# FKGSOFTWARE/TERRA-GAN

Hardware: AMD Instinct MI355X
Metric: DSM tiles/sec train-step (G+D) at 256x256 bs=16 (higher is better)
Workload: dtype f32; 1 GPU; BASELINE configs[1]: 256x256 1-ch DSM tiles, batch 16 per GPU, fp32, PConv-UNet G + PatchGAN D + L1/VGG-perceptual/TV/boundary(0.5) losses + 2x Adam; global_batch=16, tile=256, parallelism=single-gpu, launch=eager, vgg_weights=deterministic stand-in (ImageNet weights not fetchable offline; same FLOPs), vgg_trunk=forward Winograd F(2x2,3x3), dgrads F(4x4,3x3) (DESIGN 2b)

## Files before the change

### include/terragan_hip.h

```cpp
#ifndef TERRAGAN_HIP_H
#define TERRAGAN_HIP_H

#include <stddef.h>
#include <stdint.h>

#ifdef __cplusplus
extern "C" {
#endif

typedef void* tg_stream_t;

enum { TG_OK = 0, TG_ERR_ARG = -1, TG_ERR_LAUNCH = -2, TG_ERR_WS = -3 };
enum { TG_ACT_NONE = 0, TG_ACT_RELU = 1, TG_ACT_LEAKY = 2 };
enum { TG_PREC_F32 = 0, TG_PREC_BF16 = 1, TG_PREC_F32_WINO4 = 2 };

typedef struct TgConv {
    int32_t B, H, W, Cin;
    int32_t Ho, Wo, Cout;
    int32_t k, stride, pad;
    int32_t precision;
} TgConv;

int tg_version(void);
const char* tg_last_error(void);


size_t tg_conv_fwd_ws_bytes(const TgConv* g);
int tg_conv_fwd(const TgConv* g, const float* x, const float* in_mask, const float* w,
                const float* bias, const float* ratio, int act, float slope, float* y,
                float* ws, size_t ws_bytes, tg_stream_t stream);

size_t tg_conv_dgrad_ws_bytes(const TgConv* g);
int tg_conv_dgrad(const TgConv* g, const float* dy, const float* w, const float* in_mask,
                  float* dx, int accumulate, float* ws, size_t ws_bytes, tg_stream_t stream);
int tg_conv_dgrad_gated(const TgConv* g, const float* dy, const float* w, const float* in_mask,
                        const float* x_act, int act, float slope, float* dx, float* ws,
                        size_t ws_bytes, tg_stream_t stream);

enum { TG_WPREP_FWD = 0, TG_WPREP_DGRAD = 1 };
size_t tg_conv_wprep_bytes(const TgConv* g, int mode);
int tg_conv_wprep(const TgConv* g, int mode, const float* w, float* wprep, tg_stream_t stream);
size_t tg_conv_wprep_item_bytes(void);
int tg_conv_wprep_item(const TgConv* g, int mode, const float* w, float* wprep, void* item_out);
int tg_conv_wprep_run(const void* items_dev, int n, tg_stream_t stream);
int tg_conv_fwd_p(const TgConv* g, const float* x, const float* in_mask, const float* w, const float* wprep,
                  const float* bias, const float* ratio, int act, float slope, float* y, float* ws,
                  size_t ws_bytes, tg_stream_t stream);
int tg_conv_fwd_pool(const TgConv* g, const float* x, const float* in_mask, const float* w, const float* wprep,
                     const float* bias, const float* ratio, int act, float slope, float* y, float* pool_y, float* ws,
                     size_t ws_bytes, tg_stream_t stream);
int tg_conv_pool_code_supported(const TgConv* g);
int tg_conv_fwd_pool_code(const TgConv* g, const float* x, const float* w, const float* wprep, const float* bias,
                          float* pool_y, unsigned char* code, float* ws, size_t ws_bytes, tg_stream_t stream);
int tg_maxpool2_bwd_code(const float* dout, const unsigned char* code, int B, int Ho, int Wo, int C, float* dx,
                         tg_stream_t stream);
typedef struct TgSparseMap {
    const uint32_t* bits;
    const int32_t* list;
    const int32_t* count;
    int32_t nb, tiles_y, tiles_x, _pad;
} TgSparseMap;
size_t tg_vgg_sparse_map_bytes(int nb, int H, int W, const char* plan);
int tg_vgg_sparse_map(const float* x, int nb, int H, int W, const char* plan, void* buf, size_t buf_bytes, int* ticket,
                      TgSparseMap* maps, tg_stream_t stream);
int tg_conv_fwd_sparse(const TgConv* g, const float* x, const float* w, const float* wprep, const float* bias, int act,
                       float slope, float* y, float* pool_y, unsigned char* code, const TgSparseMap* sp, float* ws,
                       size_t ws_bytes, tg_stream_t stream);
typedef struct TgBnAct {
    const float *mean, *rstd, *gamma, *beta;
    int32_t act;
    float slope;
} TgBnAct;
int tg_conv_bnin_supported(const TgConv* g, int wgrad);
int tg_conv_fwd_bnin(const TgConv* g, const float* x, const TgBnAct* bn, const float* w, const float* bias, int act,
                     float slope, float* y, float* ws, size_t ws_bytes, tg_stream_t stream);
int tg_conv_wgrad_bnin(const TgConv* g, const float* x, const TgBnAct* bn, const float* dy, float* dw, float* db, float* ws,
                       size_t ws_bytes, tg_stream_t stream);
int tg_conv_dgrad_p(const TgConv* g, const float* dy, const float* w, const float* wprep, const float* in_mask,
                    const float* x_act, int act, float slope, float* dx, int accumulate, float* ws,
                    size_t ws_bytes, tg_stream_t stream);
int tg_relu_gate_pack(const float* a, int64_t rows, int C, uint32_t* bits, tg_stream_t stream);
int tg_conv_dgrad_gbits(const TgConv* g, const float* dy, const float* w, const float* wprep, const float* in_mask,
                        const uint32_t* gate_bits, float* dx, int accumulate, float* ws, size_t ws_bytes, tg_stream_t stream);

int tg_set_cu_reserve(int cus);
int tg_set_work_stealing(int mode);

size_t tg_conv_wgrad_ws_bytes(const TgConv* g);
int tg_conv_wgrad(const TgConv* g, const float* x, const float* in_mask, const float* dy,
                  float* dw, float* db, float* ws, size_t ws_bytes, tg_stream_t stream);

int tg_fold_cin(const float* w3, int cout, int taps, int cin, float* w1, tg_stream_t stream);


int tg_mask_update(const float* mask, int B, int H, int W, int k, int stride, int pad, int Ho,
                   int Wo, float* mask_out, float* ratio, tg_stream_t stream);
int tg_mask_up_merge(const float* up_mask, const float* skip_mask, int B, int h, int w, int H,
                     int W, float* out, tg_stream_t stream);

#define TG_MASK_PYRAMID_MAX 24
typedef struct TgMaskOp {
    int kind, H, W, Ho, Wo, k, stride, pad;
    const float* in;
    const float* in2;
    float* out;
    float* out2;
} TgMaskOp;
typedef struct TgMaskPyramid {
    int nops, _pad;
    TgMaskOp op[TG_MASK_PYRAMID_MAX];
} TgMaskPyramid;
int tg_mask_pyramid(const TgMaskPyramid* pm, int B, tg_stream_t stream);


size_t tg_bn_ws_bytes(int64_t rows, int C);
int tg_bn_stats(const float* y, int64_t rows, int C, float eps, float momentum, float* save_mean,
                float* save_rstd, float* running_mean, float* running_var,
// ... 191 lines not shown
```

### terra-gan_amd/csrc/igemm.hip

```cpp
#include <atomic>
#include <stdlib.h>
#include <string.h>

#include <mutex>
#include <vector>

#include "common.h"

struct ProfRec {
    hipEvent_t a, b;
    int kind;
    double flops, bytes;
    int M, N, K, C, splits, cfg;
    char tag[32];
};
static std::mutex g_prof_mu;
static bool g_prof_on = false;
static std::vector<ProfRec> g_prof;
static thread_local char g_prof_tag[32] = "";

struct ProfScope {
    bool on = false;
    ProfRec r{};
    hipStream_t s;
// ... 948 lines not shown
    p.splits = cdiv(p.nchunks, q.chunks_per_split);
    if (p.bf16) {
        if (n64) *rc = launch_pgemm_cfg<16, 16, 4, 1, 2, 2, 12, true>(p, q, flops, bytes, Mtot, s);
        else *rc = launch_pgemm_cfg<8, 16, 2, 2, 2, 2, 7, true>(p, q, flops, bytes, Mtot, s);
    } else {
        if (n64) *rc = launch_pgemm_cfg<16, 16, 4, 1, 2, 2, 12, false>(p, q, flops, bytes, Mtot, s);
        else *rc = launch_pgemm_cfg<8, 16, 2, 2, 2, 2, 7, false>(p, q, flops, bytes, Mtot, s);
    }
    return true;
}

#include "wino.inc"
#include "wino44.inc"
#include "wino16.inc"

static int launch_wino(IGemmParams& p, size_t ws_floats_avail, hipStream_t s) {
    const WinoPlan pl = wino_plan(p, ws_floats_avail);
    p.splits = pl.splits;
    p.Ktot = 9 * p.C;
    TgWprepItem it = {};
    it.kind = p.bf16 ? 5 : 1; it.N = p.N; it.K = p.C; it.w = p.w_raw; it.out = p.wino_u; it.ww = pl.ww;
    int rc = TG_OK;
    const auto transform = [&]() -> int {
        if (p.bf16) {
            hipLaunchKernelGGL(wino_weights16_kernel, dim3(ew_grid((int64_t)p.N * (p.C / 2), 256)), dim3(256), 0, s, p.w_raw,
                               reinterpret_cast<__bf16*>(p.wino_u), p.N, p.C, pl.ww);
            TG_CHECK_LAUNCH("wino_weights16_kernel");
        } else {
            hipLaunchKernelGGL(wino_weights_kernel, dim3(ew_grid((int64_t)p.N * p.C, 256)), dim3(256), 0, s, p.w_raw, p.wino_u, p.N,
                               p.C, pl.ww);
            TG_CHECK_LAUNCH("wino_weights_kernel");
        }
        return TG_OK;
    };
    if (wino_prep(p, it, transform, &rc)) return rc;
    if (pl.pool) p.pool_done = 1;
    TG_REQUIRE(pl.pool || !(p.pool_code || p.pool_only), "tg_conv_fwd_pool_code: this launch cannot write the pool from its output transform");
    TG_REQUIRE(!p.pool_code || p.act == TG_ACT_RELU, "tg_conv_fwd_pool_code: needs a ReLU output");
    if (pl.gbits) p.gate_bits_done = 1;
    WinoProf pf = {p.bf16 ? 3 : 0, p.bf16 ? 4016 : 4064, p.M, 2.0 * p.M * (double)p.N * p.Ktot * g_alg_scale, 0.0};
    pf.bytes = 4.0 * ((double)p.B * p.IH * p.IW * p.C + (double)p.M + (double)p.N * p.Ktot + (double)p.M * p.N +
                      (p.amask ? (double)p.B * p.IH * p.IW : 0.0) + (pl.pool ? 0.25 * (double)p.M * p.N : 0.0)) -
               (p.pool_only ? (4.0 - 0.25) * (double)p.M * p.N : 0.0);
    if (p.bf16) {
        typedef void (*W16Kern)(const IGemmParams, const WinoGeom, const __bf16*);
        static const W16Kern kerns[8] = {wino16_kernel<false, false>, wino16_kernel<false, true>, wino16_kernel<true, false>,
                                         wino16_kernel<true, true>, wino16_pipe_kernel<false>, wino16_pipe_kernel<true>,
                                         wino16_pipe_kernel<false, true>, wino16_pipe_kernel<true, false, true>};
        static LdsOptIn opts[8];
        const int ki = pl.kernel(false);
        return wino_launch(kerns[ki], opts[ki], pl.pipe ? W16_PIPE_LDS_BYTES : W16_LDS_BYTES, "wino16_kernel", p, pl.q, pf, true, s);
    }
    typedef void (*WinoKern)(const IGemmParams, const WinoGeom, const float*);
    static const WinoKern kerns[18] = {wino_kernel<false, false, false>, wino_kernel<false, true, false>, wino_kernel<true, false, false>,
                                       wino_kernel<true, true, false>, wino_pipe_kernel<false, false>, wino_pipe_kernel<true, false>,
                                       wino_pipe_kernel<false, false, true>, wino_pipe_kernel<true, false, false, true>,
                                       wino_kernel<false, false, true>, wino_kernel<false, true, true>, wino_kernel<true, false, true>,
                                       wino_kernel<true, true, true>, wino_pipe_kernel<false, true>, wino_pipe_kernel<true, true>,
                                       wino_pipe_kernel<false, true, true>, wino_pipe_kernel<true, true, false, true>,
                                       wino_pipe_kernel<false, false, false, false, true>, wino_pipe_kernel<false, false, true, false, true>};
    static LdsOptIn opts[18];
    WinoGeom q = pl.q;
    q.qctr = wino_queue_block(s, p.splits, q.total_work);
    if (pl.sparse && !q.qctr) {
        const TgSparseMap* sm = p.sparse;
        q.sp_bits = sm->bits; q.sp_list = sm->list; q.sp_count = sm->count;
        q.sp_nb = sm->nb; q.sp_tiles = sm->nb * q.tiles_y * q.tiles_x;
    }
    const int ki = pl.kernel(q.qctr != nullptr);
    return wino_launch(kerns[ki], opts[ki], (size_t)WINO_LDS_FLOATS * sizeof(float), "wino_kernel", p, q, pf, true, s);
}

static int pick_bn(int N) { return N >= 128 && N % 128 == 0 ? 128 : (N > 32 ? 64 : 32); }

static void plan_splits(IGemmParams& p, size_t ws_floats_avail) {
    const int bn = pick_bn(p.N);
    const long tiles = (long)cdiv(p.M, 128) * cdiv(p.N, bn);
    int splits = 1;
    if (p.T >= 8) {
        int smax = p.T / 4 < 64 ? p.T / 4 : 64;
        while (smax > 1 && (size_t)smax * p.M * p.N > ws_floats_avail) --smax;
        splits = choose_splits(tiles, smax, 512);
    }
    p.steps_per_split = cdiv(p.T > 0 ? p.T : 1, splits);
    p.splits = p.T > 0 ? cdiv(p.T, p.steps_per_split) : 1;
}

static int launch_igemm(IGemmParams& p, hipStream_t s, size_t ws_floats_avail = 0) {
    if (p.M <= 0 || p.N <= 0) return TG_OK;
    TG_REQUIRE(!p.pool_only, "tg_conv_fwd_pool_code: this launch cannot write the pool from its output transform");
    if (smallconv_fwd_applies(p)) {
        p.splits = 1;
        p.Ktot = p.TH * p.TW * p.C;
        const double by = 4.0 * ((double)p.B * p.IH * p.IW * p.C + (double)p.M * p.N + (double)p.N * p.Ktot);
        ProfScope ps(s, 2, 2.0 * p.M * (double)p.N * p.Ktot, by, p.M, p.N, p.Ktot, p.C, 1, 2000);
        return smallconv_fwd_launch(p, s);
    }
    {
        int rc = TG_OK;
        if (try_pgemm(&p, 1, ws_floats_avail, s, &rc)) return rc;
    }
    const bool scalar = (p.C % 4) != 0;
    p.Ktot = p.TH * p.TW * p.C;
    p.nchunks = cdiv(p.C, 32);
    p.T = scalar ? cdiv(p.Ktot, 32) : p.TH * p.TW * p.nchunks;
    const int bn = pick_bn(p.N);
    if (scalar) {
        if (bn == 128) return launch_igemm_cfg<2, 2, 2, 2, true>(p, s);
        if (bn == 64) return launch_igemm_cfg<2, 2, 2, 1, true>(p, s);
        return launch_igemm_cfg<4, 1, 1, 1, true>(p, s);
    }
    if (p.bf16) {
        if (bn == 128) return launch_igemm_cfg<2, 2, 2, 2, false, true>(p, s);
        if (bn == 64) return launch_igemm_cfg<2, 2, 2, 1, false, true>(p, s);
    }
    if (bn == 128) return launch_igemm_cfg<2, 2, 2, 2, false>(p, s);
    if (bn == 64) return launch_igemm_cfg<2, 2, 2, 1, false>(p, s);
    return launch_igemm_cfg<4, 1, 1, 1, false>(p, s);
}

template <int WAVES_M, int WAVES_N, int WM, int WN, bool BF16>
static int launch_igemm_multi_cfg(const IGemmMulti& pm, int ncls, hipStream_t s) {
// ... 424 lines not shown
        return smallconv_wgrad_applies(p) && smallconv_bnin_wgrad_ok(p) ? 1 : 0;
    }
    return smallconv_bnin_fwd_ok(conv_fwd_params(g)) ? 1 : 0;
}
extern "C" int tg_conv_fwd_bnin(const TgConv* g, const float* x, const TgBnAct* bn, const float* w, const float* bias, int act,
                                float slope, float* y, float* ws, size_t ws_bytes, tg_stream_t stream) {
    TG_REQUIRE(bn && bn->mean && bn->rstd && bn->gamma && bn->beta, "tg_conv_fwd_bnin: null pointer");
    TG_REQUIRE(tg_conv_bnin_supported(g, 0), "tg_conv_fwd_bnin: geometry not supported (ask tg_conv_bnin_supported first)");
    const BnIn b = bnin_of(bn);
    FwdExtras e;
    e.in_bn = &b;
    return conv_fwd_impl(g, x, nullptr, w, nullptr, 0, bias, nullptr, act, slope, y, ws, ws_bytes, stream, nullptr, &e);
}
extern "C" int tg_conv_fwd(const TgConv* g, const float* x, const float* in_mask, const float* w, const float* bias,
                           const float* ratio, int act, float slope, float* y, float* ws, size_t ws_bytes,
                           tg_stream_t stream) {
    return conv_fwd_impl(g, x, in_mask, w, nullptr, 0, bias, ratio, act, slope, y, ws, ws_bytes, stream);
}
extern "C" int tg_conv_fwd_p(const TgConv* g, const float* x, const float* in_mask, const float* w, const float* wprep,
                             const float* bias, const float* ratio, int act, float slope, float* y, float* ws, size_t ws_bytes,
                             tg_stream_t stream) {
    return conv_fwd_impl(g, x, in_mask, w, const_cast<float*>(wprep), wprep ? 1 : 0, bias, ratio, act, slope, y, ws, ws_bytes,
                         stream);
}

__global__ __launch_bounds__(256) void transpose_w_kernel(const float* __restrict__ w, float* __restrict__ wt,
                                                          int cout, int taps, int cin) {
    const size_t total = (size_t)cout * taps * cin;
    for (size_t idx = (size_t)blockIdx.x * 256 + threadIdx.x; idx < total; idx += (size_t)gridDim.x * 256) {
        int co = (int)(idx % cout);
        size_t r = idx / cout;
        int t = (int)(r % taps);
        int ci = (int)(r / taps);
        wt[idx] = w[((size_t)co * taps + t) * cin + ci];
    }
}

static size_t dgrad_wt_floats(const TgConv* g) {
    size_t wt = align_up((size_t)g->Cout * g->k * g->k * g->Cin, 64);
    size_t uf = conv_wino_floats(g);
    return wt > uf ? wt : uf;
}
extern "C" size_t tg_conv_dgrad_ws_bytes(const TgConv* g) {
    if (!g) return 0;
    if (s2d_ok(g)) {
        const TgConv g2 = s2d_geom(g);
        return (s2d_x_floats(g) + s2d_w_floats(g)) * sizeof(float) + tg_conv_dgrad_ws_bytes(&g2);
    }
    return (dgrad_wt_floats(g) + splitk_room_floats((size_t)g->B * g->H * g->W * g->Cin)) * sizeof(float);
}

static int conv_dgrad_impl(const TgConv* g, const float* dy, const float* w, float* wprep, int prep, const float* in_mask, float* dx,
                           int accumulate, const float* gate, int gate_act, float gate_slope, float* ws, size_t ws_bytes,
                           tg_stream_t stream, const uint32_t* gate_bits = nullptr, int* gate_bits_done = nullptr);
extern "C" int tg_conv_dgrad(const TgConv* g, const float* dy, const float* w, const float* in_mask, float* dx,
                             int accumulate, float* ws, size_t ws_bytes, tg_stream_t stream) {
    return conv_dgrad_impl(g, dy, w, nullptr, 0, in_mask, dx, accumulate, nullptr, 0, 0.f, ws, ws_bytes, stream);
}
extern "C" int tg_conv_dgrad_gated(const TgConv* g, const float* dy, const float* w, const float* in_mask, const float* x_act,
                                   int act, float slope, float* dx, float* ws, size_t ws_bytes, tg_stream_t stream) {
    TG_REQUIRE(x_act != nullptr && (act == TG_ACT_RELU || act == TG_ACT_LEAKY), "tg_conv_dgrad_gated: needs x_act and a ReLU/LeakyReLU");
    return conv_dgrad_impl(g, dy, w, nullptr, 0, in_mask, dx, 0, x_act, act, slope, ws, ws_bytes, stream);
}
extern "C" int tg_conv_dgrad_p(const TgConv* g, const float* dy, const float* w, const float* wprep, const float* in_mask,
                               const float* x_act, int act, float slope, float* dx, int accumulate, float* ws, size_t ws_bytes,
                               tg_stream_t stream) {
    TG_REQUIRE(x_act == nullptr || ((act == TG_ACT_RELU || act == TG_ACT_LEAKY) && !accumulate),
               "tg_conv_dgrad_p: a gated dgrad needs a ReLU/LeakyReLU and accumulate == 0");
    const bool usable = wprep != nullptr && !(x_act != nullptr && g && s2d_ok(g));
    return conv_dgrad_impl(g, dy, w, usable ? const_cast<float*>(wprep) : nullptr, usable ? 1 : 0, in_mask, dx, accumulate, x_act,
                           act, slope, ws, ws_bytes, stream);
}
extern "C" int tg_conv_dgrad_gbits(const TgConv* g, const float* dy, const float* w, const float* wprep, const float* in_mask,
                                   const uint32_t* gate_bits, float* dx, int accumulate, float* ws, size_t ws_bytes, tg_stream_t stream) {
    int rc = check_conv(g, "tg_conv_dgrad_gbits");
    if (rc) return rc;
    TG_REQUIRE(dy && w && gate_bits && dx && ws, "tg_conv_dgrad_gbits: null pointer");
    TG_REQUIRE(!accumulate, "tg_conv_dgrad_gbits: a gated dgrad does not accumulate");
    TG_REQUIRE(g->Cin % 32 == 0, "tg_conv_dgrad_gbits: needs Cin %% 32 == 0 (one gate word per 32 channels), got %d", g->Cin);
    TG_REQUIRE((reinterpret_cast<uintptr_t>(gate_bits) & 15) == 0, "tg_conv_dgrad_gbits: pointers must be 16-byte aligned");
    const bool usable = wprep != nullptr && !s2d_ok(g);
    int done = 0;
    rc = conv_dgrad_impl(g, dy, w, usable ? const_cast<float*>(wprep) : nullptr, usable ? 1 : 0, in_mask, dx, 0, nullptr, TG_ACT_NONE, 0.f,
                         ws, ws_bytes, stream, gate_bits, &done);
    if (rc || done) return rc;
    return gate_bits_apply_launch(dx, gate_bits, (int64_t)g->B * g->H * g->W, g->Cin, (hipStream_t)stream);
}
extern "C" int tg_conv_wprep(const TgConv* g, int mode, const float* w, float* wprep, tg_stream_t stream) {
    TG_REQUIRE(g && w && wprep, "tg_conv_wprep: null pointer");
    TG_REQUIRE(mode == TG_WPREP_FWD || mode == TG_WPREP_DGRAD, "tg_conv_wprep: bad mode %d", mode);
    TG_REQUIRE(tg_conv_wprep_bytes(g, mode) > 0, "tg_conv_wprep: this (geometry, mode) runs on the raw weights");
    if (mode == TG_WPREP_FWD)
        return conv_fwd_impl(g, nullptr, nullptr, w, wprep, -1, nullptr, nullptr, 0, 0.f, nullptr, nullptr, 0, stream);
    return conv_dgrad_impl(g, nullptr, w, wprep, -1, nullptr, nullptr, 0, nullptr, 0, 0.f, nullptr, 0, stream);
}
extern "C" size_t tg_conv_wprep_item_bytes(void) { return sizeof(TgWprepItem); }
extern "C" int tg_conv_wprep_item(const TgConv* g, int mode, const float* w, float* wprep, void* item_out) {
    if (!g || !w || !wprep || !item_out || (mode != TG_WPREP_FWD && mode != TG_WPREP_DGRAD)) return 0;
    if (tg_conv_wprep_bytes(g, mode) == 0) return 0;
    TgWprepItem it = {};
    g_wprep_capture = &it;
    g_wprep_captured = 0;
    int rc = mode == TG_WPREP_FWD ? conv_fwd_impl(g, nullptr, nullptr, w, wprep, -1, nullptr, nullptr, 0, 0.f, nullptr, nullptr, 0, nullptr)
                                  : conv_dgrad_impl(g, nullptr, w, wprep, -1, nullptr, nullptr, 0, nullptr, 0, 0.f, nullptr, 0, nullptr);
    g_wprep_capture = nullptr;
    if (rc != TG_OK || g_wprep_captured != 1) return 0;
    memcpy(item_out, &it, sizeof(it));
    return 1;
}
extern "C" int tg_conv_wprep_run(const void* items_dev, int n, tg_stream_t stream) {
    TG_REQUIRE(items_dev && n > 0, "tg_conv_wprep_run: bad arguments");
    hipLaunchKernelGGL(wprep_multi_kernel, dim3(2048, n), dim3(256), 0, (hipStream_t)stream, static_cast<const TgWprepItem*>(items_dev));
    TG_CHECK_LAUNCH("wprep_multi_kernel");
    return TG_OK;
}
static int conv_dgrad_impl(const TgConv* g, const float* dy, const float* w, float* wprep, int prep, const float* in_mask, float* dx,
                           int accumulate, const float* gate, int gate_act, float gate_slope, float* ws, size_t ws_bytes,
                           tg_stream_t stream, const uint32_t* gate_bits, int* gate_bits_done) {
    int rc = check_conv(g, "tg_conv_dgrad");
    if (rc) return rc;
    TG_REQUIRE(w && (prep < 0 || (dy && dx && ws)), "tg_conv_dgrad: null pointer");
    TG_REQUIRE(aligned16(dy) && aligned16(w) && aligned16(dx) && aligned16(ws) && aligned16(wprep),
               "tg_conv_dgrad: pointers must be 16-byte aligned");
    TG_REQUIRE(prep == 0 || wprep != nullptr, "tg_conv_dgrad: prepared weights expected");
    if (s2d_ok(g) && gate == nullptr && gate_bits == nullptr && (prep < 0 || ws_bytes >= tg_conv_dgrad_ws_bytes(g))) {
        hipStream_t s2 = (hipStream_t)stream;
        const TgConv g2 = s2d_geom(g);
        float* dx2 = ws;
        float* w2 = prep ? wprep : ws + s2d_x_floats(g);
        float* wsr = ws ? ws + s2d_x_floats(g) + s2d_w_floats(g) : nullptr;
        if (prep < 0 && g_wprep_capture) {
            const int rc2 = conv_dgrad_impl(&g2, nullptr, w2, wprep + s2d_w_floats(g), -1, nullptr, nullptr, 0, nullptr, 0, 0.f, nullptr, 0, stream);
            if (rc2 == TG_OK && g_wprep_captured == 1 && g_wprep_capture->kind == 1) {
                g_wprep_capture->kind = 4; g_wprep_capture->w = w; g_wprep_capture->taps = g->Cin;
            } else {
                g_wprep_captured = -1;
            }
            return rc2;
        }
        if (prep <= 0) {
            hipLaunchKernelGGL(w5x5_s2d_kernel, dim3(ew_grid((int64_t)g->Cout * 36 * g->Cin, 256)), dim3(256), 0, s2, w, w2, g->Cout, g->Cin, 1);
            TG_CHECK_LAUNCH("w5x5_s2d_kernel");
        }
        {
            AlgScale sc(25.0 / 36.0);
            rc = conv_dgrad_impl(&g2, dy, w2, prep ? wprep + s2d_w_floats(g) : nullptr, prep, nullptr, dx2, 0, nullptr, 0, 0.f, wsr,
                                 ws ? ws_bytes - (s2d_x_floats(g) + s2d_w_floats(g)) * sizeof(float) : 0, stream);
        }
        if (rc || prep < 0) return rc;
        hipLaunchKernelGGL(d2s_kernel, dim3(ew_grid((int64_t)g->B * g->H * g->W * (g->Cin / 4), 256)), dim3(256), 0, s2, dx2, in_mask, dx,
                           g->B, g->H, g->W, g->Cin, accumulate);
        TG_CHECK_LAUNCH("d2s_kernel");
        return TG_OK;
    }
    TG_REQUIRE(!(s2d_ok(g) && gate == nullptr && gate_bits == nullptr && prep > 0),
               "tg_conv_dgrad: workspace too small for the prepared 5x5 stride-2 path");
    const int taps = g->k * g->k;
    const size_t wt_floats = prep ? 0 : dgrad_wt_floats(g);
    TG_REQUIRE(prep < 0 || ws_bytes >= wt_floats * sizeof(float), "tg_conv_dgrad: workspace too small (%zu < %zu)", ws_bytes,
               wt_floats * sizeof(float));
    hipStream_t s = (hipStream_t)stream;
    float* wt = prep ? wprep : ws;
    float* ws2 = ws ? ws + wt_floats : nullptr;
    const size_t ws2_avail = ws ? ws_bytes / sizeof(float) - wt_floats : 0;
    const size_t room = splitk_room_floats((size_t)g->B * g->H * g->W * g->Cin);
    const size_t ws2_floats = min_floats(ws2_avail, room);
    if (wino_dgrad_geom_ok(g)) {
        IGemmParams p = conv_dgrad_s1_params(g);
        p.src = dy; p.rowscale = in_mask; p.dst = dx; p.ws = ws2;
        p.act = TG_ACT_NONE; p.accumulate = accumulate;
        p.gate = gate; p.gate_act = gate_act; p.gate_slope = gate_slope;
        p.w_raw = w; p.w_sn = 1; p.w_sk = (long)taps * g->Cin; p.w_stap = g->Cin;
        p.wino_u = wt;
        p.wino_ready = prep;
        p.gate_bits = gate_bits;
        rc = launch_wino_s1(p, ws, dgrad_wt_floats(g), ws2_avail, room, s, "tg_conv_dgrad");
        if (gate_bits_done) *gate_bits_done = p.gate_bits_done;
        return rc;
    }
    if (wino22_dgrad_geom_ok(g)) {
        IGemmParams p = {};
        p.src = dy; p.rowscale = in_mask; p.dst = dx; p.ws = ws2;
        p.act = TG_ACT_NONE; p.accumulate = accumulate;
        p.gate = gate; p.gate_act = gate_act; p.gate_slope = gate_slope;
        p.w_raw = w;
        p.wino_u = wt;
        p.wino_ready = prep;
        return launch_wino22(g, p, 1, ws2_floats, s);
    }
    if (prep < 0 && g_wprep_capture) {
        TgWprepItem it = {};
        it.kind = 2; it.N = g->Cout; it.K = g->Cin; it.taps = taps; it.w = w; it.out = wt;
        *g_wprep_capture = it;
        g_wprep_captured = 1;
        return TG_OK;
    }
    if (prep <= 0) {
        hipLaunchKernelGGL(transpose_w_kernel, dim3(ew_grid((int64_t)g->Cout * taps * g->Cin, 256)), dim3(256), 0, s, w, wt,
                           g->Cout, taps, g->Cin);
        TG_CHECK_LAUNCH("transpose_w_kernel");
    }
    if (prep < 0) return TG_OK;

    const int st = g->stride;
    IGemmParams cls[4];
    int ncls = 0;
    const bool mergeable = st * st <= 4;
    for (int py = 0; py < st; ++py) {
        for (int px = 0; px < st; ++px) {
            IGemmParams p = {};
            p.src = dy; p.amask = nullptr; p.wmat = wt; p.bias = nullptr; p.rowscale = in_mask; p.dst = dx; p.ws = ws2;
            p.B = g->B; p.IH = g->Ho; p.IW = g->Wo; p.C = g->Cout;
            p.OH = (g->H - py + st - 1) / st; p.OW = (g->W - px + st - 1) / st;
            if (p.OH <= 0 || p.OW <= 0) continue;
            p.N = g->Cin; p.M = g->B * p.OH * p.OW;
            p.DH = g->H; p.DW = g->W; p.ds = st; p.dy0 = py; p.dx0 = px;
            p.ky0 = (py + g->pad) % st; p.kx0 = (px + g->pad) % st;
            p.TH = p.ky0 < g->k ? (g->k - p.ky0 + st - 1) / st : 0;
            p.TW = p.kx0 < g->k ? (g->k - p.kx0 + st - 1) / st : 0;
            p.ss = 1; p.tstep = -1;
            p.sy0 = (py + g->pad - p.ky0) / st; p.sx0 = (px + g->pad - p.kx0) / st;
            p.KW = g->k; p.kstep = st;
            p.Kfull = taps * g->Cout;
            p.act = TG_ACT_NONE; p.slope = 0.f; p.accumulate = accumulate;
            p.gate = gate; p.gate_act = gate_act; p.gate_slope = gate_slope;
            p.bf16 = g->precision == TG_PREC_BF16;
            p.Ktot = p.TH * p.TW * p.C; p.nchunks = cdiv(p.C, 32);
            p.T = (p.C % 4) ? cdiv(p.Ktot, 32) : p.TH * p.TW * p.nchunks;
// ... 702 lines not shown
```

### terra-gan_amd/csrc/pointwise.hip

```cpp
#include <math.h>
#include <string.h>

#include "common.h"

static thread_local char g_err[512] = "";
void tg_set_error(const char* fmt, ...) {
    va_list ap;
    va_start(ap, fmt);
    vsnprintf(g_err, sizeof(g_err), fmt, ap);
    va_end(ap);
}
extern "C" const char* tg_last_error(void) { return g_err; }
extern "C" int tg_version(void) { return 100; }

static size_t align_up(size_t v, size_t a) { return (v + a - 1) / a * a; }
static inline hipStream_t S(tg_stream_t s) { return (hipStream_t)s; }

constexpr int CR_MAXPASS = 4;

struct ColGeom {
    int cpp;
    int rlanes;
    int npass;
    int grid;
// ... 262 lines not shown
    } else {
        for (int ky = 0; ky < k; ++ky) {
            const int iy = oy * stride - pad + ky;
            if (iy < 0 || iy >= H) continue;
            for (int kx = 0; kx < k; ++kx) {
                const int ix = ox * stride - pad + kx;
                if (ix < 0 || ix >= W) continue;
                s += mask[((int64_t)b * H + iy) * W + ix];
            }
        }
    }
    const float on = s > 0.f ? 1.f : 0.f;
    const int64_t o = ((int64_t)b * Ho + oy) * Wo + ox;
    mask_out[o] = on;
    ratio[o] = (1.0f / (s + 1e-8f)) * (float)(k * k) * on;
}
__global__ __launch_bounds__(1024) void mask_pyramid_kernel(const TgMaskPyramid pm) {
    const int b = blockIdx.x;
    for (int i = 0; i < pm.nops; ++i) {
        const TgMaskOp op = pm.op[i];
        if (op.kind == 0) {
            for (int idx = threadIdx.x; idx < op.Ho * op.Wo; idx += 1024)
                mask_update_one(op.in, op.H, op.W, op.k, op.stride, op.pad, op.Ho, op.Wo, b, idx, op.out, op.out2);
        } else {
            const int offy = floordiv2(op.Ho - 2 * op.H), offx = floordiv2(op.Wo - 2 * op.W);
            for (int idx = threadIdx.x; idx < op.Ho * op.Wo; idx += 1024) {
                const int X = idx % op.Wo, Y = idx / op.Wo;
                const int yu = Y - offy, xu = X - offx;
                float v = 0.f;
                if (yu >= 0 && yu < 2 * op.H && xu >= 0 && xu < 2 * op.W) v = op.in[((int64_t)b * op.H + (yu >> 1)) * op.W + (xu >> 1)];
                const int64_t o = ((int64_t)b * op.Ho + Y) * op.Wo + X;
                op.out[o] = fmaxf(v, op.in2[o]);
            }
        }
        __syncthreads();
    }
}
extern "C" int tg_mask_pyramid(const TgMaskPyramid* pm, int B, tg_stream_t stream) {
    TG_REQUIRE(pm && B > 0 && pm->nops >= 1 && pm->nops <= TG_MASK_PYRAMID_MAX, "tg_mask_pyramid: bad arguments");
    for (int i = 0; i < pm->nops; ++i) {
        const TgMaskOp& op = pm->op[i];
        TG_REQUIRE(op.in && op.out && (op.kind == 0 ? op.out2 != nullptr : op.in2 != nullptr), "tg_mask_pyramid: op %d: null pointer", i);
        TG_REQUIRE(op.H > 0 && op.W > 0 && op.Ho > 0 && op.Wo > 0, "tg_mask_pyramid: op %d: bad dims", i);
        if (op.kind == 0)
            TG_REQUIRE(op.k > 0 && op.stride > 0 && op.pad >= 0 && op.Ho == (op.H + 2 * op.pad - op.k) / op.stride + 1 &&
                       op.Wo == (op.W + 2 * op.pad - op.k) / op.stride + 1, "tg_mask_pyramid: op %d: Ho/Wo inconsistent", i);
    }
    hipLaunchKernelGGL(mask_pyramid_kernel, dim3(B), dim3(1024), 0, S(stream), *pm);
    TG_CHECK_LAUNCH("mask_pyramid_kernel");
    return TG_OK;
}

constexpr int VSM_MAX_OPS = 24, VSM_MAX_CONV = 16, VSM_LDS_WORDS = 4096;
struct VggMapArgs {
    const uint32_t* x;
    int nb, H, W, nops, nconv;
    char ops[VSM_MAX_OPS];
    int tiles_y[VSM_MAX_CONV], tiles_x[VSM_MAX_CONV];
    int32_t* count[VSM_MAX_CONV];
    uint32_t* bits[VSM_MAX_CONV];
    int32_t* list[VSM_MAX_CONV];
    unsigned char* flags[VSM_MAX_CONV];
    uint64_t* d0;
    int rows_per_slice;
    int* ticket;
};
__device__ __forceinline__ uint32_t vsm_even_bits(uint64_t v) {
    v &= 0x5555555555555555ull;
    v = (v | (v >> 1)) & 0x3333333333333333ull;
    v = (v | (v >> 2)) & 0x0f0f0f0f0f0f0f0full;
    v = (v | (v >> 4)) & 0x00ff00ff00ff00ffull;
    v = (v | (v >> 8)) & 0x0000ffff0000ffffull;
    v = (v | (v >> 16)) & 0x00000000ffffffffull;
    return (uint32_t)v;
}
__device__ __forceinline__ uint64_t vsm_row_mask(int W, int w, int WW) {
    return (w == WW - 1 && (W & 63)) ? (1ull << (W & 63)) - 1 : ~0ull;
}
__device__ __forceinline__ bool vsm_last_arrival(int* ctr, int n, int* s_last) {
    __builtin_amdgcn_s_waitcnt(0);
    __syncthreads();
    if (threadIdx.x == 0) {
        __threadfence();
        const bool last = atomicAdd(ctr, 1) == n - 1;
        if (last) __threadfence();
        *s_last = last;
    }
    __syncthreads();
    return *s_last;
}
__global__ __launch_bounds__(1024) void vgg_sparse_map_kernel(const VggMapArgs a) {
    extern __shared__ uint64_t vsm[];
    __shared__ int scan[1024];
    __shared__ int s_last;
    const int tid = threadIdx.x, lane = tid & 63, wave = tid >> 6, b = blockIdx.y;
    int H = a.H, W = a.W, WW = (W + 63) >> 6;
    uint64_t* cur = vsm;
    uint64_t* nxt = vsm + H * WW;
    uint64_t* d0 = a.d0 + (size_t)b * H * WW;
    {
        const uint32_t* xp = a.x + (size_t)b * H * W;
        const uint32_t* tp = a.x + ((size_t)a.nb + b) * H * W;
        const int ubeg = blockIdx.x * a.rows_per_slice * WW, uend = min(H, (blockIdx.x + 1) * a.rows_per_slice) * WW;
        for (int u0 = ubeg + wave; u0 < uend; u0 += 16 * 8) {
            uint32_t pv[8], tv[8];
#pragma unroll
            for (int k = 0; k < 8; ++k) {
                const int u = u0 + 16 * k, y = u / WW, px = (u - y * WW) * 64 + lane;
                pv[k] = tv[k] = 0;
                if (u < uend && px < W) { pv[k] = xp[(size_t)y * W + px]; tv[k] = tp[(size_t)y * W + px]; }
            }
#pragma unroll
            for (int k = 0; k < 8; ++k) {
                const uint64_t m = __ballot(pv[k] != tv[k]);
                if (lane == 0 && u0 + 16 * k < uend) d0[u0 + 16 * k] = m;
            }
        }
    }
    if (!vsm_last_arrival(a.ticket + b, (int)gridDim.x, &s_last)) return;
    for (int u = tid; u < H * WW; u += 1024) cur[u] = d0[u];
    if (tid == 0) __hip_atomic_store(a.ticket + b, 0, __ATOMIC_RELAXED, __HIP_MEMORY_SCOPE_AGENT);
    __syncthreads();
    int ci = 0;
    for (int o = 0; o < a.nops; ++o) {
        if (a.ops[o] == 'C') {
            for (int u = tid; u < H * WW; u += 1024) {
                const int y = u / WW, w = u - y * WW;
                uint64_t r = 0;
                for (int dy = -1; dy <= 1; ++dy) {
                    const int yy = y + dy;
                    if (yy < 0 || yy >= H) continue;
                    const uint64_t* row = cur + yy * WW;
                    const uint64_t v = row[w];
                    r |= v | (v << 1) | (v >> 1);
                    if (w > 0) r |= row[w - 1] >> 63;
                    if (w + 1 < WW) r |= row[w + 1] << 63;
                }
                nxt[u] = r & vsm_row_mask(W, w, WW);
            }
            __syncthreads();
            uint64_t* t = cur; cur = nxt; nxt = t;
            const int ty_n = a.tiles_y[ci], tx_n = a.tiles_x[ci], tiles = ty_n * tx_n;
            for (int t2 = tid; t2 < tiles; t2 += 1024) {
                const int ty = t2 / tx_n, tx = t2 - ty * tx_n;
                const int w = (16 * tx) >> 6, sh = (16 * tx) & 63;
                uint64_t any = 0;
                for (int y = 16 * ty; y < min(16 * ty + 16, H); ++y) any |= (cur[y * WW + w] >> sh) & 0xffffull;
                a.flags[ci][(size_t)b * tiles + t2] = any ? 1 : 0;
            }
            ++ci;
        } else {
            const int H2 = H >> 1, W2 = W >> 1, WW2 = (W2 + 63) >> 6;
            for (int u = tid; u < H2 * WW2; u += 1024) {
                const int y = u / WW2, w = u - y * WW2;
                const uint64_t* r0 = cur + (2 * y) * WW;
                const uint64_t* r1 = r0 + WW;
                const uint64_t s0 = r0[2 * w] | r1[2 * w];
                const uint64_t s1 = 2 * w + 1 < WW ? r0[2 * w + 1] | r1[2 * w + 1] : 0;
                const uint64_t v = (uint64_t)vsm_even_bits(s0 | (s0 >> 1)) | ((uint64_t)vsm_even_bits(s1 | (s1 >> 1)) << 32);
                nxt[u] = v & vsm_row_mask(W2, w, WW2);
            }
            H = H2; W = W2; WW = WW2;
            __syncthreads();
            uint64_t* t = cur; cur = nxt; nxt = t;
        }
        __syncthreads();
    }
    if (!vsm_last_arrival(a.ticket + a.nb, a.nb, &s_last)) return;
    for (int c = 0; c < a.nconv; ++c) {
        const int n = a.nb * a.tiles_y[c] * a.tiles_x[c], nw = (n + 31) >> 5;
        int carry = 0;
        for (int w0 = 0; w0 < nw; w0 += 1024) {
            const int w = w0 + tid;
            uint32_t word = 0;
            if (w < nw) {
                const uint4* fp = reinterpret_cast<const uint4*>(a.flags[c] + 32 * (size_t)w);
                const uint4 f0 = fp[0], f1 = fp[1];
                const uint32_t fw[8] = {f0.x, f0.y, f0.z, f0.w, f1.x, f1.y, f1.z, f1.w};
#pragma unroll
                for (int i = 0; i < 8; ++i)
#pragma unroll
                    for (int j = 0; j < 4; ++j) word |= ((fw[i] >> (8 * j)) & 1u) << (4 * i + j);
                if (32 * w + 32 > n) word &= (1u << (n - 32 * w)) - 1u;
                a.bits[c][w] = word;
            }
            const int pc = __popc(word);
            scan[tid] = pc;
            __syncthreads();
            for (int d = 1; d < 1024; d <<= 1) {
                const int v = tid >= d ? scan[tid - d] : 0;
                __syncthreads();
                scan[tid] += v;
                __syncthreads();
            }
            int pos = carry + scan[tid] - pc;
            for (uint32_t m = word; m; m &= m - 1) a.list[c][pos++] = 32 * w + __ffs(m) - 1;
            carry += scan[1023];
            __syncthreads();
        }
        if (tid == 0) *a.count[c] = carry;
    }
    if (tid == 0) __hip_atomic_store(a.ticket + a.nb, 0, __ATOMIC_RELAXED, __HIP_MEMORY_SCOPE_AGENT);
}

struct VsmLayout {
    int nconv, nops, H, W;
    size_t d0;
    int tiles_y[VSM_MAX_CONV], tiles_x[VSM_MAX_CONV];
    size_t count[VSM_MAX_CONV], bits[VSM_MAX_CONV], list[VSM_MAX_CONV], flags[VSM_MAX_CONV];
    size_t bytes;
};
static bool vsm_layout(int nb, int H, int W, const char* plan, VsmLayout& L) {
    if (nb <= 0 || H <= 0 || W <= 0 || !plan) return false;
    if ((size_t)H * ((W + 63) / 64) > VSM_LDS_WORDS) return false;
    L = VsmLayout{};
    L.H = H; L.W = W;
    L.d0 = 0;
    size_t off = align_up((size_t)nb * H * ((W + 63) / 64) * sizeof(uint64_t), 16);
    int h = H, w = W;
    for (const char* c = plan; *c; ++c) {
        if (L.nops == VSM_MAX_OPS) return false;
        ++L.nops;
        if (*c == 'M') {
            h >>= 1; w >>= 1;
            if (h <= 0 || w <= 0) return false;
        } else if (*c == 'C') {
            if (L.nconv == VSM_MAX_CONV) return false;
            const int i = L.nconv++;
            L.tiles_y[i] = cdiv(h, 16); L.tiles_x[i] = cdiv(w, 16);
            const size_t n = (size_t)nb * L.tiles_y[i] * L.tiles_x[i];
            if (n > ((size_t)1 << 30)) return false;
            L.count[i] = off; off += 16;
            L.bits[i] = off; off += align_up((n + 31) / 32, 4) * 4;
            L.list[i] = off; off += align_up(n, 4) * 4;
            L.flags[i] = off; off += align_up(n, 32);
        } else {
            return false;
        }
    }
    L.bytes = off;
    return L.nconv > 0;
}
extern "C" size_t tg_vgg_sparse_map_bytes(int nb, int H, int W, const char* plan) {
    VsmLayout L;
    return vsm_layout(nb, H, W, plan, L) ? L.bytes : 0;
}
extern "C" int tg_vgg_sparse_map(const float* x, int nb, int H, int W, const char* plan, void* buf, size_t buf_bytes, int* ticket,
                                 TgSparseMap* maps, tg_stream_t stream) {
    VsmLayout L;
    TG_REQUIRE(x && buf && ticket && maps, "tg_vgg_sparse_map: null pointer");
    TG_REQUIRE(vsm_layout(nb, H, W, plan, L), "tg_vgg_sparse_map: geometry not supported (tg_vgg_sparse_map_bytes is 0)");
    TG_REQUIRE(buf_bytes >= L.bytes && (reinterpret_cast<uintptr_t>(buf) & 15) == 0, "tg_vgg_sparse_map: buffer too small or unaligned");
    VggMapArgs a = {};
    a.x = reinterpret_cast<const uint32_t*>(x);
    a.nb = nb; a.H = H; a.W = W; a.nops = L.nops; a.nconv = L.nconv; a.ticket = ticket;
    for (int i = 0; i < L.nops; ++i) a.ops[i] = plan[i];
    char* base = static_cast<char*>(buf);
    a.d0 = reinterpret_cast<uint64_t*>(base + L.d0);
    const int slices = cdiv(H, 8) < cdiv(256, nb) ? cdiv(H, 8) : cdiv(256, nb);
    a.rows_per_slice = cdiv(H, slices);
    for (int i = 0; i < L.nconv; ++i) {
        a.tiles_y[i] = L.tiles_y[i]; a.tiles_x[i] = L.tiles_x[i];
        a.count[i] = reinterpret_cast<int32_t*>(base + L.count[i]);
        a.bits[i] = reinterpret_cast<uint32_t*>(base + L.bits[i]);
        a.list[i] = reinterpret_cast<int32_t*>(base + L.list[i]);
        a.flags[i] = reinterpret_cast<unsigned char*>(base + L.flags[i]);
        maps[i] = TgSparseMap{a.bits[i], a.list[i], a.count[i], nb, L.tiles_y[i], L.tiles_x[i], 0};
    }
    const size_t lds = 2 * (size_t)H * ((W + 63) / 64) * sizeof(uint64_t);
    static bool opted[64] = {};
    int dev = 0;
    (void)hipGetDevice(&dev);
    if (dev < 0 || dev >= 64 || !opted[dev]) {
        if (hipFuncSetAttribute(reinterpret_cast<const void*>(vgg_sparse_map_kernel), hipFuncAttributeMaxDynamicSharedMemorySize,
                                (int)(2 * VSM_LDS_WORDS * sizeof(uint64_t))) != hipSuccess) {
            tg_set_error("tg_vgg_sparse_map: LDS opt-in failed");
            return TG_ERR_LAUNCH;
        }
        if (dev >= 0 && dev < 64) opted[dev] = true;
    }
    hipLaunchKernelGGL(vgg_sparse_map_kernel, dim3(cdiv(H, a.rows_per_slice), nb), dim3(1024), lds, S(stream), a);
    TG_CHECK_LAUNCH("vgg_sparse_map_kernel");
    return TG_OK;
}

struct BnStatF {
    const float* y;
    int C;
    __device__ BnStatF group(int g, int64_t rows_g) const { return BnStatF{y + (size_t)g * rows_g * C, C}; }
    __device__ void operator()(int64_t r, int c, float (&q)[2]) const {
        float d = y[r * C + c] - y[c];
        q[0] += d;
        q[1] += d * d;
    }
    __device__ void quad(int64_t r, int c0, float (&q)[2][4]) const {
        const f32x4 v = *reinterpret_cast<const f32x4*>(y + r * C + c0);
        const f32x4 sh = *reinterpret_cast<const f32x4*>(y + c0);
#pragma unroll
        for (int e = 0; e < 4; ++e) {
            float d = v[e] - sh[e];
            q[0][e] += d;
            q[1][e] += d * d;
        }
    }
};
__global__ __launch_bounds__(256) void bn_finalize_kernel(const float* __restrict__ partial, int nblocks, int C,
                                                          const float* __restrict__ y, int64_t rows, float eps,
                                                          float momentum, float* __restrict__ mean_out,
                                                          float* __restrict__ rstd_out, float* __restrict__ rm,
                                                          float* __restrict__ rv, int64_t* __restrict__ nbt) {
    if (blockIdx.x == 0 && threadIdx.x == 0 && nbt) *nbt += 1;
    double q[2];
    int c;
    if (!final_reduce<2>(partial, nblocks, C, q, &c)) return;
    const double n = (double)rows;
    const double md = q[0] / n;
    double var = q[1] / n - md * md;
    if (var < 0.0) var = 0.0;
    const double mean = (double)y[c] + md;
    mean_out[c] = (float)mean;
    rstd_out[c] = (float)(1.0 / sqrt(var + (double)eps));
    if (rm) rm[c] = (float)((1.0 - (double)momentum) * (double)rm[c] + (double)momentum * mean);
    if (rv) rv[c] = (float)((1.0 - (double)momentum) * (double)rv[c] + (double)momentum * var * (n / (n - 1.0)));
}
extern "C" size_t tg_bn_ws_bytes(int64_t rows, int C) {
    if (rows <= 0 || C <= 0) return 0;
    ColGeom g = col_geom(rows, C);
    int grid = g.grid;
    if (C % 4 == 0) {
        ColGeom4 g4 = col_geom4(rows, C);
        if (g4.grid > grid) grid = g4.grid;
    }
    return align_up((size_t)grid * 5 * C, 64) * sizeof(float);
}
extern "C" int tg_bn_stats(const float* y, int64_t rows, int C, float eps, float momentum, float* save_mean,
                           float* save_rstd, float* running_mean, float* running_var, int64_t* num_batches_tracked,
// ... 1796 lines not shown
```

### terra-gan_amd/csrc/wino.inc

```
#pragma once
#include <utility>

struct WinoGeom {
    int tiles_x, tiles_y, total_work, chunks_per_split, nt;
    int sy_min, sx_min;
    int interleave;
    int* qctr;
    const uint32_t* sp_bits;
    const int* sp_list;
    const int* sp_count;
    int sp_tiles, sp_nb;
};
struct WinoWeights {
    long sn, sk, stap;
    int kyu[3], kxv[3];
    int k_fast;
};
typedef unsigned int u32x4 __attribute__((ext_vector_type(4)));
constexpr int WINO_BN = 64;
constexpr int WINO_V = 16 * 64 * 8;
constexpr int WINO_U = 16 * WINO_BN * 8;
constexpr int WINO_PPIX = 18 * 18;
constexpr int WINO_P = WINO_PPIX * 8;
constexpr int WINO_LDS_FLOATS = 2 * WINO_V + 2 * WINO_U + WINO_P;
constexpr int WINO_THREADS = 512;

__device__ __forceinline__ void wino_barrier() { asm volatile("s_waitcnt lgkmcnt(0)\n\ts_barrier" ::: "memory"); }

template <class F, int... T>
__device__ __forceinline__ void wino_static_for(std::integer_sequence<int, T...>, F&& f) {
    (f(std::integral_constant<int, T>{}), ...);
}

__device__ __forceinline__ void wino_distribute(int total, int interleave, int& item, int& item_end, int& step) {
    const int G = gridDim.x;
    if (interleave) {
        const int xcd = blockIdx.x & 7, slot = blockIdx.x >> 3, nslots = (G - xcd + 7) >> 3;
        const int ch_q = total >> 3, ch_r = total & 7;
        const int chunk0 = xcd < ch_r ? xcd * (ch_q + 1) : ch_r * (ch_q + 1) + (xcd - ch_r) * ch_q;
        item = chunk0 + slot;
        item_end = chunk0 + ch_q + (xcd < ch_r ? 1 : 0);
        step = nslots;
    } else {
        const int rblk = xcd_remap(blockIdx.x, G);
        const int per = total / G, rem = total % G;
        item = rblk * per + min(rblk, rem);
        item_end = item + per + (rblk < rem ? 1 : 0);
        step = 1;
    }
}

constexpr int WQ_Z = 16;
constexpr int WQ_INTS = 8 * WQ_Z + 8;
__device__ __forceinline__ int wq_chunk0(int total, int c) { const int q = total >> 3, r = total & 7; return c < r ? c * (q + 1) : r * (q + 1) + (c - r) * q; }
__device__ __forceinline__ int wq_len(int total, int c) { return (total >> 3) + (c < (total & 7) ? 1 : 0); }
template <bool STEAL>
struct WinoWork {
    int item;
    int item_end, step;
    int* home_ctr;
    int home_c0, home_len;

    __device__ __forceinline__ void init(int total, int interleave, int* ctr, int* slot) {
        if constexpr (!STEAL) {
            wino_distribute(total, interleave, item, item_end, step);
            if (item >= item_end) item = -1;
        } else {
            const int home = blockIdx.x & 7, rank = blockIdx.x >> 3;
            const int nwg = (gridDim.x - home + 7) >> 3;
            const int len = wq_len(total, home), c0 = wq_chunk0(total, home);
            home_ctr = ctr + 8 * blockIdx.z + home;
            home_c0 = c0 + nwg;
            home_len = len - nwg;
            item = rank < len ? c0 + rank : -1;
            step = 0; item_end = 0;
            if (threadIdx.x == 0) {
                int nx = -1;
                if (item >= 0 && home_len > 0) {
                    const int i = atomicAdd(home_ctr, 1);
                    if (i < home_len) nx = home_c0 + i;
                }
                slot[0] = nx;
            }
            __syncthreads();
// ... 344 lines not shown
    wino_barrier();
    constexpr bool gated = GATED;
    f32x4 bq = {0.f, 0.f, 0.f, 0.f};
    if (p.bias && p.splits == 1) bq = *reinterpret_cast<const f32x4*>(p.bias + e_n0 + 32 * nw + 4 * (lane & 7));
    float rsq[2][4] = {{1.f, 1.f, 1.f, 1.f}, {1.f, 1.f, 1.f, 1.f}};
    if (p.rowscale && p.splits == 1) {
#pragma unroll
        for (int j = 0; j < 2; ++j)
#pragma unroll
            for (int t4 = 0; t4 < 4; ++t4) {
                const int t = 32 * mw + (lane >> 3) + 8 * t4;
                const int oy = min(e_oy0 + 2 * (t >> 3) + xh, p.OH - 1), ox = min(e_ox0 + 2 * (t & 7) + j, p.OW - 1);
                rsq[j][t4] = p.rowscale[((size_t)e_b * p.DH + (oy * p.ds + p.dy0)) * p.DW + (ox * p.ds + p.dx0)];
            }
    }
#pragma unroll
    for (int j = 0; j < 2; ++j) {
        f32x4 gq[GATED ? 4 : 1];
        if constexpr (gated) {
#pragma unroll
            for (int t4 = 0; t4 < 4; ++t4) {
                const int t = 32 * mw + (lane >> 3) + 8 * t4;
                const int oy = min(e_oy0 + 2 * (t >> 3) + xh, p.OH - 1), ox = min(e_ox0 + 2 * (t & 7) + j, p.OW - 1);
                const size_t pix = ((size_t)e_b * p.DH + (oy * p.ds + p.dy0)) * p.DW + (ox * p.ds + p.dx0);
                gq[t4] = *reinterpret_cast<const f32x4*>(p.gate + pix * p.N + e_n0 + 32 * nw + 4 * (lane & 7));
            }
        }
        const float* xr = X + ((((xh ^ 1) * 2 + nw) * 2 + mw) * 2 + j) * 1024 + lane;
        f32x16 y;
#pragma unroll
        for (int r = 0; r < 16; ++r) y[r] = own[j][r] + xr[r * 64];
        tile_rows4i(scratch, y, lane, [&](int t4, int rr, int cc, f32x4 v4) {
            const int t = 32 * mw + rr;
            const int oy = e_oy0 + 2 * (t >> 3) + xh, ox = e_ox0 + 2 * (t & 7) + j;
            const int nb = e_n0 + 32 * nw + cc;
            if (oy >= p.OH || ox >= p.OW) return;
            if (p.splits > 1) {
                const size_t m = ((size_t)e_b * p.OH + oy) * p.OW + ox;
                *reinterpret_cast<f32x4*>(p.ws + ((size_t)blockIdx.z * p.M + m) * p.N + nb) = v4;
            } else {
                const size_t pix = ((size_t)e_b * p.DH + (oy * p.ds + p.dy0)) * p.DW + (ox * p.ds + p.dx0);
                *reinterpret_cast<f32x4*>(p.dst + pix * p.N + nb) = epilogue4(p, v4, pix, nb, gated ? &gq[gated ? t4 : 0] : nullptr, &rsq[j][t4], &bq);
            }
        });
    }
    wk.publish(wq_pulled, wq_slot);
    if (!more_items) break;
    wino_barrier();
    wk.advance(wq_next);
    }
    wk.done(q.qctr);
}

template <bool GATED, bool STEAL, bool POOL = false, bool GBITS = false, bool SPARSE = false>
__global__ __launch_bounds__(WINO_THREADS) void wino_pipe_kernel(const IGemmParams p, const WinoGeom q, const float* __restrict__ U) {
    extern __shared__ __attribute__((aligned(16))) float smem[];
    float* Vs = smem;
    float* Us = smem + 2 * WINO_V;
    float* Ps = smem + 2 * WINO_V + 2 * WINO_U;

    const int tid = threadIdx.x, lane = tid & 63, wave = tid >> 6;
    const int mw = wave & 1, nw = (wave >> 1) & 1, xh = wave >> 2;
    __shared__ int wq_slot[2];
    WinoWork<STEAL> wk;
    int total = q.total_work;
    if constexpr (SPARSE) {
        const int cnt = __builtin_amdgcn_readfirstlane(*q.sp_count);
        total = (q.sp_tiles + min(max(cnt, 0), q.sp_tiles)) * q.nt;
    }
    wk.init(total, q.interleave, q.qctr, wq_slot);

    struct Item { int nt, n0, oy0, ox0, b, mirror; uint32_t poff[2]; };
    auto decode_item = [&](int it) {
        Item r;
        r.nt = it % q.nt;
        int tile = it / q.nt;
        r.mirror = 0;
        if constexpr (SPARSE) {
            if (tile < q.sp_tiles) {
                r.mirror = (__builtin_amdgcn_readfirstlane(q.sp_bits[tile >> 5]) >> (tile & 31)) & 1 ? 0 : 1;
                tile += q.sp_tiles;
            } else {
                tile = __builtin_amdgcn_readfirstlane(q.sp_list[tile - q.sp_tiles]);
            }
        }
        const int tx = tile % q.tiles_x;
        tile /= q.tiles_x;
        const int ty = tile % q.tiles_y;
        r.b = tile / q.tiles_y;
        r.n0 = r.nt * WINO_BN; r.oy0 = ty * 16; r.ox0 = tx * 16;
        const int py0 = r.oy0 + q.sy_min, px0 = r.ox0 + q.sx_min;
#pragma unroll
        for (int i = 0; i < 2; ++i) {
            const int pp = (tid + WINO_THREADS * i) >> 1, spy = pp / 18, spx = pp - spy * 18;
            const int iy = py0 + spy, ix = px0 + spx;
            r.poff[i] = 0x80000000u;
            if (pp < WINO_PPIX && iy >= 0 && iy < p.IH && ix >= 0 && ix < p.IW)
                r.poff[i] = ((((uint32_t)r.b * p.IH + iy) * p.IW + ix) * (uint32_t)p.C + 4 * (tid & 1)) * 4u;
        }
        return r;
    };
    const auto srsrc = __builtin_amdgcn_make_buffer_rsrc(const_cast<float*>(p.src), 0, (int)((size_t)p.B * p.IH * p.IW * p.C * 4), 0x00020000);
    const auto ursrc = __builtin_amdgcn_make_buffer_rsrc(const_cast<float*>(U), 0, (int)((size_t)16 * p.N * p.C * 4), 0x00020000);
    const uint32_t u_voff = tid * 16;
    const bool p1_ok = ((tid + WINO_THREADS) >> 1) < WINO_PPIX;
    const int c_begin = blockIdx.z * q.chunks_per_split;
    const int c_end = min(p.C >> 3, c_begin + q.chunks_per_split);
    const size_t ustep = (size_t)q.nt * WINO_U;

    f32x4 ru[4], rp[2];
    auto pload1 = [&](uint32_t voff, int c, int i) { rp[i] = __builtin_bit_cast(f32x4, __builtin_amdgcn_raw_buffer_load_b128(srsrc, voff, c * 32, 0)); };
    auto uload1 = [&](int nt, int c, int j) {
        ru[j] = __builtin_bit_cast(f32x4, __builtin_amdgcn_raw_buffer_load_b128(
            ursrc, u_voff, (int)(((size_t)nt * WINO_U + (size_t)c * ustep) * 4) + 16 * WINO_THREADS * j, 0));
    };
    auto pstore1 = [&](int i) { if (i == 0 || p1_ok) *reinterpret_cast<f32x4*>(Ps + 4 * (tid + WINO_THREADS * i)) = rp[i]; };
    auto ustore1 = [&](int buf, int j) { *reinterpret_cast<f32x4*>(Us + buf * WINO_U + 4 * (tid + WINO_THREADS * j)) = ru[j]; };

    const int t_quad = lane & 1, t_tile = (lane >> 1) + 32 * (wave & 1), t_a = wave >> 1;
    const int t_r0 = t_a == 0 ? 0 : (t_a == 2 ? 2 : 1), t_r1 = t_a == 3 ? 3 : (t_a == 2 ? 1 : 2);
    const float t_s1 = t_a == 1 ? 1.f : -1.f;
    const int t_src0 = ((2 * (t_tile >> 3) + t_r0) * 18 + 2 * (t_tile & 7)) * 8 + 4 * t_quad;
    const int t_src1 = ((2 * (t_tile >> 3) + t_r1) * 18 + 2 * (t_tile & 7)) * 8 + 4 * t_quad;
    const int t_dst = (t_a * 4) * 512 + t_tile * 8 + (((t_quad ^ (t_tile >> 4)) & 1) << 2);
    f32x4 td[2][4], tt[4];
    auto t_read1 = [&](int k) { td[k >> 2][k & 3] = *reinterpret_cast<const f32x4*>(Ps + ((k >> 2) ? t_src1 : t_src0) + (k & 3) * 8); };
    auto t_row1 = [&](int j) { tt[j] = td[0][j] + td[1][j] * t_s1; };
    auto t_col1 = [&](int buf, int k) {
        const f32x4 v = k == 0 ? tt[0] - tt[2] : k == 1 ? tt[1] + tt[2] : k == 2 ? tt[2] - tt[1] : tt[1] - tt[3];
        *reinterpret_cast<f32x4*>(Vs + buf * WINO_V + t_dst + k * 512) = v;
    };

// ... 38 lines not shown
        fa[0] = *reinterpret_cast<const f32x4*>(Vs + cur * WINO_V + a_off);
        fb[0] = *reinterpret_cast<const f32x4*>(Us + cur * WINO_U + b_off);
        auto kstep = [&](uint32_t pv0, uint32_t pv1, int unt, int c2) {
            const int nxt = cur ^ 1;
            const float* Vc = Vs + cur * WINO_V + a_off;
            const float* Uc = Us + cur * WINO_U + b_off;
            const float* Vn = Vs + nxt * WINO_V + a_off;
            const float* Un = Us + nxt * WINO_U + b_off;
            wino_static_for(std::make_integer_sequence<int, 32>{}, [&](auto tc) {
                constexpr int t = decltype(tc)::value;
                constexpr int xi = t >> 2, e = t & 3;
                if constexpr (t < 2) pstore1(t);
                if constexpr (t == 2) pload1(pv0, c2, 0);
                if constexpr (t == 3) pload1(pv1, c2, 1);
                if constexpr (t == 4) wino_barrier();
                if constexpr (t >= 5 && t < 9) { t_read1(t - 5); t_read1(4 + t - 5); }
                if constexpr (t >= 8 && t < 12) { t_row1(t - 8); }
                if constexpr (t >= 14 && t < 18) t_col1(nxt, t - 14);
                if constexpr (t >= 18 && t < 22) ustore1(nxt, t - 18);
                if constexpr (t >= 22 && t < 26) uload1(unt, c2, t - 22);
                if constexpr (t == 26) wino_barrier();
                if constexpr (e == 0 && xi < 7) {
                    fa[(xi + 1) & 1] = *reinterpret_cast<const f32x4*>(Vc + (xi + 1) * 512);
                    fb[(xi + 1) & 1] = *reinterpret_cast<const f32x4*>(Uc + (xi + 1) * 512);
                }
                if constexpr (e == 0 && xi == 7) {
                    fa[0] = *reinterpret_cast<const f32x4*>(Vn);
                    fb[0] = *reinterpret_cast<const f32x4*>(Un);
                }
                __builtin_amdgcn_sched_barrier(0);
                acc[xi] = __builtin_amdgcn_mfma_f32_32x32x2f32(fa[xi & 1][e], fb[xi & 1][e], acc[xi], 0, 0, 0);
                __builtin_amdgcn_sched_barrier(0);
            });
            cur = nxt;
        };
        for (int c = c_begin; c < c_end - 2; ++c) kstep(ci.poff[0], ci.poff[1], ci.nt, c + 2);
        kstep(ni.poff[0], ni.poff[1], ni.nt, c_begin);
        kstep(ni.poff[0], ni.poff[1], ni.nt, c_begin + 1);
        const int wq_pulled = wk.request(wk.next(wq_slot));
        const int fr = cur ^ 1;
        float* X = Vs + fr * WINO_V;
        float* scratch = wave < 7 ? Us + fr * WINO_U + wave * (32 * 36) : Ps;
        const int e_wave = __builtin_amdgcn_readfirstlane(wave);
        const int e_mw = e_wave & 1, e_nw = (e_wave >> 1) & 1, e_xh = e_wave >> 2;
        const int e_row0 = ci.oy0 + 8 * e_mw + e_xh;
        const int e_pitch = p.DW * p.ds;
        const int e_pix0 = (ci.b * p.DH + p.dy0) * p.DW + p.dx0 + ci.ox0 * p.ds;
        const int e_nb0 = ci.n0 + 32 * e_nw;
        const uint32_t e_lane_px = 2 * (lane >> 3) * p.ds;
        const bool e_single = p.splits == 1;
        const float act_neg = p.act == TG_ACT_RELU ? 0.f : (p.act == TG_ACT_LEAKY ? p.slope : 1.f);
        const float gate_neg = p.gate_act == TG_ACT_LEAKY ? p.gate_slope : 0.f;
        const auto drsrc = __builtin_amdgcn_make_buffer_rsrc(p.dst, 0, (int)((size_t)p.B * p.DH * p.DW * p.N * 4), 0x00020000);
        const int e_mdelta = SPARSE ? q.sp_nb * p.DH * p.DW * p.N * 4 : 0;
        f32x4 bq = {0.f, 0.f, 0.f, 0.f};
        if (p.bias && e_single) bq = *reinterpret_cast<const f32x4*>(p.bias + e_nb0 + 4 * (lane & 7));
        f32x4 pmx[POOL ? 4 : 1];
        uint32_t jbits = 0;
        if constexpr (POOL) {
#pragma unroll
            for (int t4 = 0; t4 < 4; ++t4) pmx[t4] = f32x4{0.f, 0.f, 0.f, 0.f};
        }
        float rsq[2][4] = {{1.f, 1.f, 1.f, 1.f}, {1.f, 1.f, 1.f, 1.f}};
        if (p.rowscale && e_single) {
            const auto rrsrc = __builtin_amdgcn_make_buffer_rsrc(const_cast<float*>(p.rowscale), 0, (int)((size_t)p.B * p.DH * p.DW * 4), 0x00020000);
#pragma unroll
            for (int j = 0; j < 2; ++j) {
                const uint32_t voff = ci.ox0 + 2 * (lane >> 3) + j < p.OW ? e_lane_px * 4u : 0x80000000u;
#pragma unroll
                for (int t4 = 0; t4 < 4; ++t4) {
                    const int row = min(e_row0 + 2 * t4, p.OH - 1);
                    rsq[j][t4] = __builtin_bit_cast(float, __builtin_amdgcn_raw_buffer_load_b32(
                        rrsrc, voff, (e_pix0 + row * e_pitch + j * p.ds) * 4, 0));
                }
            }
        }
#pragma unroll
        for (int j = 0; j < 2; ++j) {
            f32x16 own;
            {
                float* xs = X + ((xh * 2 + nw) * 2 + mw) * 1024 + lane;
#pragma unroll
                for (int r = 0; r < 16; ++r) {
                    const float s0 = j == 0 ? acc[0][r] + acc[1][r] + acc[2][r] : acc[1][r] - acc[2][r] - acc[3][r];
                    const float s1 = j == 0 ? acc[4][r] + acc[5][r] + acc[6][r] : acc[5][r] - acc[6][r] - acc[7][r];
                    own[r] = xh == 0 ? s0 + s1 : -s0 - s1;
                    xs[r * 64] = xh == 0 ? s1 : s0;
                }
            }
            const uint32_t e_voff = ci.ox0 + 2 * (lane >> 3) + j < p.OW
                                        ? ((e_lane_px + j * p.ds) * (uint32_t)p.N + 4 * (lane & 7)) * 4u : 0x80000000u;
            f32x4 gq[GATED && !GBITS ? 4 : 1];
            uint32_t gw[GBITS ? 4 : 1];
            if constexpr (GBITS) {
                const int nw32 = p.N >> 5;
                const auto brsrc = __builtin_amdgcn_make_buffer_rsrc(const_cast<uint32_t*>(p.gate_bits), 0, (int)((size_t)p.B * p.DH * p.DW * nw32 * 4), 0x00020000);
                const uint32_t b_voff = ci.ox0 + 2 * (lane >> 3) + j < p.OW ? (e_lane_px + j * p.ds) * (uint32_t)nw32 * 4u : 0x80000000u;
#pragma unroll
                for (int t4 = 0; t4 < 4; ++t4) {
                    const int row = min(e_row0 + 2 * t4, p.OH - 1);
                    gw[t4] = __builtin_amdgcn_raw_buffer_load_b32(brsrc, b_voff, ((e_pix0 + row * e_pitch) * nw32 + (e_nb0 >> 5)) * 4, 0)
                             >> (4 * (lane & 7));
                }
            } else if constexpr (GATED) {
                const auto grsrc = __builtin_amdgcn_make_buffer_rsrc(const_cast<float*>(p.gate), 0, (int)((size_t)p.B * p.DH * p.DW * p.N * 4), 0x00020000);
#pragma unroll
                for (int t4 = 0; t4 < 4; ++t4) {
                    const int row = min(e_row0 + 2 * t4, p.OH - 1);
                    gq[t4] = __builtin_bit_cast(f32x4, __builtin_amdgcn_raw_buffer_load_b128(
                        grsrc, e_voff, ((e_pix0 + row * e_pitch) * p.N + e_nb0) * 4, 0));
                }
            }
            wino_barrier();
            const float* xr = X + (((xh ^ 1) * 2 + nw) * 2 + mw) * 1024 + lane;
            f32x16 y;
#pragma unroll
            for (int r = 0; r < 16; ++r) y[r] = own[r] + xr[r * 64];
            tile_rows4i(scratch, y, lane, [&](int t4, int rr, int cc, f32x4 v4) {
                if (e_single) {
                    const int row = e_row0 + 2 * t4;
                    if (row >= p.OH) return;
                    const int soff = ((e_pix0 + row * e_pitch) * p.N + e_nb0) * 4;
                    f32x4 o = (v4 + bq) * rsq[j][t4];
#pragma unroll
                    for (int e = 0; e < 4; ++e) o[e] = o[e] > 0.f ? o[e] : o[e] * act_neg + 0.f;
                    if constexpr (GBITS) {
#pragma unroll
                        for (int e = 0; e < 4; ++e) o[e] *= (gw[t4] >> e) & 1u ? 1.f : 0.f;
                    } else if constexpr (GATED) {
#pragma unroll
                        for (int e = 0; e < 4; ++e) o[e] *= gq[t4][e] > 0.f ? 1.f : gate_neg;
                    }
                    if (p.accumulate) o += __builtin_bit_cast(f32x4, __builtin_amdgcn_raw_buffer_load_b128(drsrc, e_voff, soff, 0));
                    if constexpr (POOL) {
#pragma unroll
                        for (int e = 0; e < 4; ++e) {
                            const bool gt = j == 1 && o[e] > pmx[t4][e];
                            pmx[t4][e] = (j == 0 || gt) ? o[e] : pmx[t4][e];
                            jbits |= (gt ? 1u : 0u) << (4 * t4 + e);
                        }
                        if (p.pool_only) return;
                    }
                    __builtin_amdgcn_raw_buffer_store_b128(__builtin_bit_cast(u32x4, o), drsrc, e_voff + (uint32_t)soff, 0, 0);
                    if constexpr (SPARSE) {
                        if (ci.mirror)
                            __builtin_amdgcn_raw_buffer_store_b128(__builtin_bit_cast(u32x4, o), drsrc, e_voff + (uint32_t)(soff - e_mdelta), 0, 0);
                    }
                } else {
                    const int t = 32 * mw + rr;
                    const int oy = ci.oy0 + 2 * (t >> 3) + xh, ox = ci.ox0 + 2 * (t & 7) + j;
                    if (oy >= p.OH || ox >= p.OW) return;
                    const size_t m = ((size_t)ci.b * p.OH + oy) * p.OW + ox;
                    *reinterpret_cast<f32x4*>(p.ws + ((size_t)blockIdx.z * p.M + m) * p.N + ci.n0 + 32 * nw + cc) = v4;
                }
            });
            if constexpr (POOL) {
                if (j == 1 && e_xh == 1) {
                    float* ps = X + ((0 * 2 + nw) * 2 + mw) * 1024 + lane;
#pragma unroll
                    for (int t4 = 0; t4 < 4; ++t4)
#pragma unroll
                        for (int e = 0; e < 4; ++e) {
                            const float v = pmx[t4][e];
                            ps[(t4 * 4 + e) * 64] = (p.pool_code && ((jbits >> (4 * t4 + e)) & 1u)) ? -v : v;
                        }
                }
            }
            wino_barrier();
        }
        if constexpr (POOL) {
            if (e_xh == 0 && e_single) {
                const float* pr = X + ((0 * 2 + nw) * 2 + mw) * 1024 + lane;
                const int PH = p.OH >> 1, PW = p.OW >> 1;
                const auto prsrc = __builtin_amdgcn_make_buffer_rsrc(p.pool_dst, 0, (int)((size_t)p.B * PH * PW * p.N * 4), 0x00020000);
                const uint32_t p_voff = (ci.ox0 >> 1) + (lane >> 3) < PW ? ((uint32_t)(lane >> 3) * p.N + 4 * (lane & 7)) * 4u : 0x80000000u;
                const auto crsrc = __builtin_amdgcn_make_buffer_rsrc(p.pool_code ? p.pool_code : reinterpret_cast<unsigned char*>(p.pool_dst), 0,
                                                                     (int)((size_t)p.B * PH * PW * p.N), 0x00020000);
                const uint32_t c_voff = (ci.ox0 >> 1) + (lane >> 3) < PW ? (uint32_t)(lane >> 3) * p.N + 4 * (lane & 7) : 0x80000000u;
#pragma unroll
                for (int t4 = 0; t4 < 4; ++t4) {
                    const int prow = (ci.oy0 >> 1) + 4 * e_mw + t4;
                    if (prow >= PH) continue;
                    f32x4 m;
                    uint32_t code = 0;
#pragma unroll
                    for (int e = 0; e < 4; ++e) {
                        const float raw = pr[(t4 * 4 + e) * 64];
                        const float r0 = pmx[t4][e], r1 = p.pool_code ? fabsf(raw) : raw;
                        const bool row1 = r1 > r0;
                        m[e] = row1 ? r1 : r0;
                        const uint32_t j0 = (jbits >> (4 * t4 + e)) & 1u, j1 = __float_as_uint(raw) >> 31;
                        code |= ((row1 ? 2u + j1 : j0) | (m[e] > 0.f ? 4u : 0u)) << (8 * e);
                    }
                    const int pix = (ci.b * PH + prow) * PW + (ci.ox0 >> 1);
                    __builtin_amdgcn_raw_buffer_store_b128(__builtin_bit_cast(u32x4, m), prsrc, p_voff + (uint32_t)((pix * p.N + e_nb0) * 4), 0, 0);
                    if (p.pool_code) __builtin_amdgcn_raw_buffer_store_b32(code, crsrc, c_voff + (uint32_t)(pix * p.N + e_nb0), 0, 0);
                    if constexpr (SPARSE) {
                        if (ci.mirror) {
                            const int mpix = pix - q.sp_nb * PH * PW;
                            __builtin_amdgcn_raw_buffer_store_b128(__builtin_bit_cast(u32x4, m), prsrc, p_voff + (uint32_t)((mpix * p.N + e_nb0) * 4), 0, 0);
                            if (p.pool_code) __builtin_amdgcn_raw_buffer_store_b32(code, crsrc, c_voff + (uint32_t)(mpix * p.N + e_nb0), 0, 0);
                        }
                    }
                }
            }
        }
        wk.publish(wq_pulled, wq_slot);
        const int wq_nxt2 = wk.next(wq_slot);
        if (wq_nxt2 < 0) break;
        ci = ni;
        if constexpr (STEAL) wino_barrier();
        wk.advance(wq_nxt2);
    }
    wk.done(q.qctr);
}


static int wino_kc(const IGemmParams& p) { return p.bf16 ? 16 : 8; }
static bool wino_geom_ok(const IGemmParams& p) {
    static const bool off = getenv("TG_NO_WINO") != nullptr, off16 = getenv("TG_NO_WINO16") != nullptr;
    if (off || (p.bf16 && off16)) return false;
    if (p.TH != 3 || p.TW != 3 || p.ss != 1 || (p.tstep != 1 && p.tstep != -1) || (p.kstep != 1 && p.kstep != -1)) return false;
    return (p.C % wino_kc(p)) == 0 && (p.N % WINO_BN) == 0 && p.OH >= 16 && p.OW >= 16;
}
static size_t wino_u_floats(int N, int C) { return (size_t)16 * N * C; }

static WinoWeights wino_weights_map(const IGemmParams& p, int sy_min, int sx_min) {
    WinoWeights ww = {};
    ww.sn = p.w_sn; ww.sk = p.w_sk; ww.stap = p.w_stap;
    ww.k_fast = p.w_sk == 1;
    for (int t = 0; t < 3; ++t) {
        ww.kyu[p.sy0 + t * p.tstep - sy_min] = p.ky0 + t * p.kstep;
        ww.kxv[p.sx0 + t * p.tstep - sx_min] = p.kx0 + t * p.kstep;
    }
    return ww;
}

struct WinoPlan {
    WinoGeom q;
    WinoWeights ww;
    int splits;
    bool fast, pipe, gated, pool, gbits;
    bool sparse;
    int kernel(bool queued) const {
        if (sparse && !queued) return pool ? 17 : 16;
        return (queued ? 8 : 0) + (gbits ? 7 : pool ? 6 : pipe ? 4 + gated : (fast ? 2 : 0) + gated);
    }
};
static WinoPlan wino_plan(const IGemmParams& p, size_t ws_floats_avail) {
    WinoPlan pl = {};
    WinoGeom& q = pl.q;
    q.tiles_x = cdiv(p.OW, 16);
    q.tiles_y = cdiv(p.OH, 16);
    q.nt = p.N / WINO_BN;
    q.total_work = q.tiles_x * q.tiles_y * p.B * q.nt;
    const size_t u_bytes = wino_u_floats(p.N, p.C) * (p.bf16 ? sizeof(__bf16) : sizeof(float));
    q.interleave = wino_interleave_ok(u_bytes);
    const int sy_b = p.sy0 + 2 * p.tstep, sx_b = p.sx0 + 2 * p.tstep;
    q.sy_min = p.sy0 < sy_b ? p.sy0 : sy_b;
    q.sx_min = p.sx0 < sx_b ? p.sx0 : sx_b;
    pl.ww = wino_weights_map(p, q.sy_min, q.sx_min);
    const int nchunks = p.C / wino_kc(p);
    int splits = 1;
    if (nchunks >= 16) {
        int smax = nchunks / 8 < 16 ? nchunks / 8 : 16;
        while (smax > 1 && (size_t)smax * p.M * p.N > ws_floats_avail) --smax;
        splits = choose_splits(q.total_work, smax, WINO_PLAN_CUS);
    }
    q.chunks_per_split = cdiv(nchunks, splits);
    pl.splits = cdiv(nchunks, q.chunks_per_split);
    const bool one = pl.splits == 1;
    static const bool no_fast = getenv("TG_WINO_NO_FAST") != nullptr;
    pl.fast = !no_fast && p.amask == nullptr && (size_t)p.B * p.IH * p.IW * p.C * 4 < ((size_t)1 << 31) && u_bytes < ((size_t)1 << 31);
    pl.gated = p.gate != nullptr && one;
    static const bool no_pipe = getenv("TG_WINO_NO_PIPE") != nullptr;
    pl.pipe = pl.fast && !no_pipe && nchunks - (pl.splits - 1) * q.chunks_per_split >= 2 && q.chunks_per_split >= 2 &&
              (size_t)p.B * p.DH * p.DW * p.N * 4 < ((size_t)1 << 31);
    const bool plain_dst = p.ds == 1 && p.dy0 == 0 && p.dx0 == 0 && p.DH == p.OH && p.DW == p.OW && !p.accumulate;
    static const bool no_pool = getenv("TG_NO_FUSED_POOL") != nullptr;
    pl.pool = p.pool_dst && !no_pool && pl.pipe && !pl.gated && one && !(p.OH & 1) && !(p.OW & 1) && plain_dst;
    pl.gbits = p.gate_bits != nullptr && pl.pipe && one;
    const TgSparseMap* sm = p.sparse;
    pl.sparse = !p.bf16 && sm && pl.pipe && !pl.gated && !pl.gbits && one && !p.rowscale && plain_dst && (pl.pool || !p.pool_dst) &&
                sm->nb > 0 && p.B == 2 * sm->nb && sm->tiles_y == q.tiles_y && sm->tiles_x == q.tiles_x && sm->bits && sm->list && sm->count;
    return pl;
}

template <class Transform>
static bool wino_prep(const IGemmParams& p, const TgWprepItem& it, Transform transform, int* rc) {
    *rc = TG_OK;
    if (p.wino_ready < 0 && g_wprep_capture) {
        if (it.kind) *g_wprep_capture = it;
        g_wprep_captured = it.kind ? 1 : -1;
        return true;
    }
    if (p.wino_ready <= 0 && (*rc = transform()) != TG_OK) return true;
    return p.wino_ready < 0;
}

struct WinoProf {
    int kind, cfg, M;
    double flops, bytes;
};
template <class Geom, class UT>
static int wino_launch(void (*kern)(const IGemmParams, const Geom, const UT*), LdsOptIn& opt, size_t lds, const char* name,
                       const IGemmParams& p, const Geom& q, const WinoProf& pf, bool reduce, hipStream_t s) {
    if (int rc = lds_opt_in(opt, reinterpret_cast<const void*>(kern), lds, name)) return rc;
    {
        ProfScope ps(s, pf.kind, pf.flops, pf.bytes, pf.M, p.N, p.Ktot, p.C, p.splits, pf.cfg);
        const int grid = q.total_work < wino_cus() ? q.total_work : wino_cus();
        hipLaunchKernelGGL(kern, dim3(grid, 1, p.splits), dim3(WINO_THREADS), lds, s, p, q, reinterpret_cast<const UT*>(p.wino_u));
    }
    TG_CHECK_LAUNCH(name);
    if (reduce && p.splits > 1) {
        hipLaunchKernelGGL(igemm_splitk_epilogue, dim3(ew_grid((int64_t)p.M * p.N, 256)), dim3(256), 0, s, p);
        TG_CHECK_LAUNCH("igemm_splitk_epilogue");
    }
    return TG_OK;
}

struct WinoWgradGeom {
    int strips_x, tiles_y, nstrips, steps_per_split, splits, ntco, ntci;
};

constexpr int WG_PITCH = 72;
constexpr int WG_XR = 4 * 18 * WG_PITCH;
constexpr int WG_DR = 2 * 16 * WG_PITCH;
constexpr int WINO_WG_LDS_FLOATS = 4 * WINO_V + WG_XR + WG_DR;

__global__ __launch_bounds__(WINO_THREADS) void wino_wgrad_kernel(const WgradParams p, const WinoWgradGeom q, float* __restrict__ slabs) {
    extern __shared__ __attribute__((aligned(16))) float smem[];
    float* As = smem;
    float* Bs = smem + 2 * WINO_V;
    float* Xr = smem + 4 * WINO_V;
    float* Dr = Xr + WG_XR;

    const int tid = threadIdx.x, lane = tid & 63, wave = tid >> 6;
// ... 254 lines not shown
```

### terra-gan_amd/csrc/wino44.inc

```
#pragma once

constexpr int W4_PTS = 36;
constexpr int W4_BW = 32, W4_BH = 16;
constexpr int W4_PW = W4_BW + 2, W4_PH = W4_BH + 2;
constexpr int W4_PPIX = W4_PW * W4_PH;
constexpr int W4_V = W4_PTS * 2 * 32 * 4;
constexpr int W4_T = 4 * 6 * 2 * W4_PW * 4;
constexpr int W4_P = 2 * W4_PPIX * 4;
constexpr int W4_LDS_FLOATS = 2 * W4_V + 9216 + W4_P;
constexpr int W4_U_STEP = W4_PTS * 2 * 64 * 4;
static_assert(W4_T <= 9216, "T area");
static_assert(4 * 4 * 3 * 2 * 64 * 4 <= W4_LDS_FLOATS, "exchange area");

struct Wino44Geom {
    int tiles_x, tiles_y, total_work, nt;
    int sy_min, sx_min;
    int interleave;
};

template <int A>
__device__ __forceinline__ f32x4 w44_bt1(const f32x4 (&d)[6]) {
    if constexpr (A == 0) return 4.f * d[0] + (d[4] - 5.f * d[2]);
    else if constexpr (A == 1) return (d[4] - 4.f * d[2]) + (d[3] - 4.f * d[1]);
    else if constexpr (A == 2) return (d[4] - 4.f * d[2]) - (d[3] - 4.f * d[1]);
    else if constexpr (A == 3) return (d[4] - d[2]) + 2.f * (d[3] - d[1]);
    else if constexpr (A == 4) return (d[4] - d[2]) - 2.f * (d[3] - d[1]);
    else return 4.f * d[1] + (d[5] - 5.f * d[3]);
}
template <int h>
__device__ __forceinline__ void w44_at3(float x0, float x1, float x2, float (&o)[4]) {
    if constexpr (h == 0) {
        const float sm = x1 + x2, df = x1 - x2;
        o[0] = x0 + sm; o[1] = df; o[2] = sm; o[3] = df;
    } else {
        const float sm = x0 + x1, df = x0 - x1;
        o[0] = sm; o[1] = 2.f * df; o[2] = 4.f * sm; o[3] = 8.f * df + x2;
    }
}

__device__ __forceinline__ void w44_g(float g0, float g1, float g2, float (&o)[6]) {
    o[0] = 0.25f * g0;
    o[1] = (-1.f / 6.f) * (g0 + g1 + g2);
    o[2] = (-1.f / 6.f) * (g0 - g1 + g2);
    o[3] = (1.f / 24.f) * g0 + (1.f / 12.f) * g1 + (1.f / 6.f) * g2;
    o[4] = (1.f / 24.f) * g0 - (1.f / 12.f) * g1 + (1.f / 6.f) * g2;
    o[5] = g2;
}
__device__ __forceinline__ void wino44_weights_body(const float* __restrict__ w, float* __restrict__ U, int N, int K, const WinoWeights& ww) {
    const int NT = N / 64;
    const size_t total = (size_t)N * K;
    for (size_t idx = (size_t)blockIdx.x * 256 + threadIdx.x; idx < total; idx += (size_t)gridDim.x * 256) {
        const int blk = (int)(idx >> 9), e = (int)(idx & 511);
        const int kc = blk / NT, nt = blk - kc * NT;
        const int nh = e >> 8, lane = (e >> 2) & 63, j = e & 3;
        const int n = nt * 64 + nh * 32 + (lane & 31), k = kc * 8 + 4 * (lane >> 5) + j;
        const float* wp = w + (size_t)n * ww.sn + (size_t)k * ww.sk;
        float tg[6][3];
#pragma unroll
        for (int v = 0; v < 3; ++v) {
            float col[6];
            w44_g(wp[(size_t)(ww.kyu[0] * 3 + ww.kxv[v]) * ww.stap], wp[(size_t)(ww.kyu[1] * 3 + ww.kxv[v]) * ww.stap],
                  wp[(size_t)(ww.kyu[2] * 3 + ww.kxv[v]) * ww.stap], col);
#pragma unroll
            for (int a = 0; a < 6; ++a) tg[a][v] = col[a];
        }
        float* ub = U + (size_t)blk * W4_U_STEP + e;
#pragma unroll
        for (int a = 0; a < 6; ++a) {
            float row[6];
            w44_g(tg[a][0], tg[a][1], tg[a][2], row);
#pragma unroll
            for (int b = 0; b < 6; ++b) ub[(a * 6 + b) * 512] = row[b];
        }
    }
}
__global__ __launch_bounds__(256) void wino44_weights_kernel(const float* __restrict__ w, float* __restrict__ U, int N, int K, WinoWeights ww) {
    wino44_weights_body(w, U, N, K, ww);
}

template <bool GATED, bool GBITS = false>
__global__ __launch_bounds__(WINO_THREADS) void wino44_kernel(const IGemmParams p, const Wino44Geom q, const float* __restrict__ U) {
    extern __shared__ __attribute__((aligned(16))) float smem[];
    float* Vs = smem;
    float* Ts = smem + 2 * W4_V;
    float* Ps = smem + 2 * W4_V + 9216;

    const int tid = threadIdx.x, lane = tid & 63;
    const int wave = __builtin_amdgcn_readfirstlane(tid >> 6);
    const int pg = wave & 3, nh = wave >> 2, ah = pg >> 1, bh = pg & 1;
    int item, item_end, istep;
    wino_distribute(q.total_work, q.interleave, item, item_end, istep);
    if (item >= item_end) return;

    const int nchunks = p.C >> 3;
    const int img_bytes = p.IH * p.IW * p.C * 4;
    auto srsrc = __builtin_amdgcn_make_buffer_rsrc(const_cast<float*>(p.src), 0, img_bytes, 0x00020000);
    const auto ursrc = __builtin_amdgcn_make_buffer_rsrc(const_cast<float*>(U), 0, (int)((size_t)W4_PTS * p.N * p.C * 4), 0x00020000);

    int n0, oy0, ox0, b, i_nt;
    uint32_t poff[3];
    const bool p2_ok = tid + 2 * WINO_THREADS < 2 * W4_PPIX;
    auto decode = [&]() {
        i_nt = item % q.nt;
        int tile = item / q.nt;
        const int tx = tile % q.tiles_x;
        tile /= q.tiles_x;
        const int ty = tile % q.tiles_y;
        b = tile / q.tiles_y;
        n0 = i_nt * 64; oy0 = ty * W4_BH; ox0 = tx * W4_BW;
        srsrc = __builtin_amdgcn_make_buffer_rsrc(const_cast<float*>(p.src) + (size_t)b * p.IH * p.IW * p.C, 0, img_bytes, 0x00020000);
        const int py0 = oy0 + q.sy_min, px0 = ox0 + q.sx_min;
#pragma unroll
        for (int i = 0; i < 3; ++i) {
            const int slot = tid + WINO_THREADS * i, pp = slot >> 1, spy = pp / W4_PW, spx = pp - spy * W4_PW;
            const int iy = py0 + spy, ix = px0 + spx;
            poff[i] = 0x80000000u;
            if (pp < W4_PPIX && iy >= 0 && iy < p.IH && ix >= 0 && ix < p.IW)
                poff[i] = (((uint32_t)iy * p.IW + ix) * (uint32_t)p.C + 4 * (slot & 1)) * 4u;
        }
    };
    f32x4 rp[3];
    auto pload1 = [&](int c, int i) { rp[i] = __builtin_bit_cast(f32x4, __builtin_amdgcn_raw_buffer_load_b128(srsrc, poff[i], c * 32, 0)); };
    auto pstore1 = [&](int i) {
        const int slot = tid + WINO_THREADS * i;
        if (i < 2 || p2_ok) *reinterpret_cast<f32x4*>(Ps + ((slot & 1) * W4_PPIX + (slot >> 1)) * 4) = rp[i];
    };

    const bool t1_on = tid < 2 * 4 * W4_PW;
    const int t1_x = tid % W4_PW, t1_q = (tid / W4_PW) & 1, t1_ty = (tid / W4_PW) >> 1;
    const int t1_src = (t1_q * W4_PPIX + (4 * (t1_on ? t1_ty : 0)) * W4_PW + t1_x) * 4;
    const int t1_dst = ((((t1_on ? t1_ty : 0) * 6) * 2 + t1_q) * W4_PW + t1_x) * 4;
    const bool t2_on = tid < 384;
    const int t2_q = tid & 1, t2_tile = (tid >> 1) & 31, t2_a = t2_on ? tid >> 6 : 0;
    const int t2_src = ((((t2_tile >> 3) * 6 + t2_a) * 2 + t2_q) * W4_PW + 4 * (t2_tile & 7)) * 4;
    const int t2_dst = ((t2_a * 6 * 2 + t2_q) * 32 + t2_tile) * 4;
    f32x4 td[6];
    auto t1_read = [&](int r) { td[r] = *reinterpret_cast<const f32x4*>(Ps + t1_src + r * (W4_PW * 4)); };
    auto t1_write = [&](auto ac) {
        constexpr int a = decltype(ac)::value;
        const f32x4 o = w44_bt1<a>(td);
        if (t1_on) *reinterpret_cast<f32x4*>(Ts + t1_dst + a * (2 * W4_PW * 4)) = o;
    };
    auto t2_read = [&](int j) { td[j] = *reinterpret_cast<const f32x4*>(Ts + t2_src + j * 4); };
    auto t2_write = [&](int buf, auto bc) {
        constexpr int bb = decltype(bc)::value;
        const f32x4 o = w44_bt1<bb>(td);
        if (t2_on) *reinterpret_cast<f32x4*>(Vs + buf * W4_V + t2_dst + bb * (2 * 32 * 4)) = o;
    };

    const int a_off = ((lane >> 5) * 32 + (lane & 31)) * 4;
    auto pt_of = [&](int lp) { return (3 * ah + lp / 3) * 6 + 3 * bh + lp % 3; };
    const uint32_t u_voff = (uint32_t)((nh * 64 + lane) * 16);
    f32x4 fa[3], fb[3];
    auto uload = [&](int c, int lp, int slot) {
        fb[slot] = __builtin_bit_cast(f32x4, __builtin_amdgcn_raw_buffer_load_b128(
            ursrc, u_voff, (int)((((size_t)c * q.nt + i_nt) * W4_U_STEP + (size_t)pt_of(lp) * 512) * 4), 0));
    };
// ... 113 lines not shown
        const int e_nb0 = e_n0 + 32 * nh;
        const int e_pitch = p.DW * p.ds;
        const int e_pix0 = (e_b * p.DH + p.dy0) * p.DW + p.dx0 + (e_ox0 + 2 * bh) * p.ds;
        const uint32_t e_lane = (uint32_t)(4 * (lane >> 3) * p.ds * p.N + 4 * (lane & 7)) * 4u;
        const int e_lane_ox = e_ox0 + 4 * (lane >> 3) + 2 * bh;
        const float act_neg = p.act == TG_ACT_RELU ? 0.f : (p.act == TG_ACT_LEAKY ? p.slope : 1.f);
        const float gate_neg = p.gate_act == TG_ACT_LEAKY ? p.gate_slope : 0.f;
        const auto drsrc = __builtin_amdgcn_make_buffer_rsrc(p.dst, 0, (int)((size_t)p.B * p.DH * p.DW * p.N * 4), 0x00020000);
        f32x4 bq = {0.f, 0.f, 0.f, 0.f};
        if (p.bias) bq = *reinterpret_cast<const f32x4*>(p.bias + e_nb0 + 4 * (lane & 7));
#pragma unroll
        for (int px = 0; px < 4; ++px) {
            const int di = px >> 1, dj = px & 1;
            const uint32_t e_voff = e_lane_ox + dj < p.OW ? e_lane : 0x80000000u;
            const int e_row0 = e_oy0 + 2 * ah + di;
            f32x4 gq[GATED && !GBITS ? 4 : 1];
            uint32_t gw[GBITS ? 4 : 1];
            if constexpr (GBITS) {
                const int nw32 = p.N >> 5;
                const auto brsrc = __builtin_amdgcn_make_buffer_rsrc(const_cast<uint32_t*>(p.gate_bits), 0, (int)((size_t)p.B * p.DH * p.DW * nw32 * 4), 0x00020000);
                const uint32_t b_voff = e_lane_ox + dj < p.OW ? (uint32_t)(4 * (lane >> 3) * p.ds * nw32) * 4u : 0x80000000u;
#pragma unroll
                for (int t4 = 0; t4 < 4; ++t4) {
                    const int row = min(e_row0 + 4 * t4, p.OH - 1);
                    gw[t4] = __builtin_amdgcn_raw_buffer_load_b32(brsrc, b_voff, ((e_pix0 + row * e_pitch + dj * p.ds) * nw32 + (e_nb0 >> 5)) * 4, 0)
                             >> (4 * (lane & 7));
                }
            } else if constexpr (GATED) {
                const auto grsrc = __builtin_amdgcn_make_buffer_rsrc(const_cast<float*>(p.gate), 0, (int)((size_t)p.B * p.DH * p.DW * p.N * 4), 0x00020000);
#pragma unroll
                for (int t4 = 0; t4 < 4; ++t4) {
                    const int row = min(e_row0 + 4 * t4, p.OH - 1);
                    gq[t4] = __builtin_bit_cast(f32x4, __builtin_amdgcn_raw_buffer_load_b128(
                        grsrc, e_voff, ((e_pix0 + row * e_pitch + dj * p.ds) * p.N + e_nb0) * 4, 0));
                }
            }
            f32x16 yv;
#pragma unroll
            for (int r = 0; r < 16; ++r) yv[r] = y[px][r];
            tile_rows4i(scratch, yv, lane, [&](int t4, int rr, int cc, f32x4 v4) {
                const int row = e_row0 + 4 * t4;
                if (row >= p.OH) return;
                const uint32_t soff = (uint32_t)(((e_pix0 + row * e_pitch + dj * p.ds) * p.N + e_nb0) * 4);
                f32x4 o = v4 + bq;
#pragma unroll
                for (int e = 0; e < 4; ++e) o[e] = fmaxf(o[e], 0.f) + act_neg * fminf(o[e], 0.f);
                if constexpr (GBITS) {
#pragma unroll
                    for (int e = 0; e < 4; ++e) o[e] *= (gw[t4] >> e) & 1u ? 1.f : 0.f;
                } else if constexpr (GATED) {
#pragma unroll
                    for (int e = 0; e < 4; ++e) o[e] *= gq[t4][e] > 0.f ? 1.f : gate_neg;
                }
                if (p.accumulate) o += __builtin_bit_cast(f32x4, __builtin_amdgcn_raw_buffer_load_b128(drsrc, e_voff + soff, 0, 0));
                __builtin_amdgcn_raw_buffer_store_b128(__builtin_bit_cast(u32x4, o), drsrc, e_voff + soff, 0, 0);
            });
        }
        if (!more_items) break;
        item += istep;
        wino_barrier();
    }
}

static bool wino44_enabled() {
    static const bool off = getenv("TG_NO_WINO") != nullptr || getenv("TG_NO_WINO44") != nullptr;
    return !off;
}
static bool wino44_geom_ok(const IGemmParams& p) {
    if (!wino44_enabled() || p.wino_u == nullptr || p.bf16 || !p.wino4) return false;
    if (p.TH != 3 || p.TW != 3 || p.ss != 1 || (p.tstep != 1 && p.tstep != -1) || (p.kstep != 1 && p.kstep != -1)) return false;
    if ((p.C % 8) != 0 || (p.N % 64) != 0 || p.OH < 16 || p.OW < 32) return false;
    if ((size_t)p.IH * p.IW * p.C * 4 >= ((size_t)1 << 31) || (size_t)W4_PTS * p.N * p.C * 4 >= ((size_t)1 << 31)) return false;
    return true;
}
static bool wino44_runtime_ok(const IGemmParams& p) {
    return p.amask == nullptr && p.rowscale == nullptr && (size_t)p.B * p.DH * p.DW * p.N * 4 < ((size_t)1 << 31);
}
static bool wino44_ok(const IGemmParams& p) {
    return wino44_geom_ok(p) && (p.wino_ready < 0 || wino44_runtime_ok(p));
}
static bool wino44_prepared_unusable(const IGemmParams& p) { return p.wino_ready > 0 && wino44_geom_ok(p) && !wino44_runtime_ok(p); }
static size_t wino44_u_floats(int N, int C) { return (size_t)W4_PTS * N * C; }

static int launch_wino44(IGemmParams& p, hipStream_t s) {
    Wino44Geom q = {};
    q.tiles_x = cdiv(p.OW, W4_BW);
    q.tiles_y = cdiv(p.OH, W4_BH);
    q.nt = p.N / 64;
    q.total_work = q.tiles_x * q.tiles_y * p.B * q.nt;
    q.interleave = wino_interleave_ok(wino44_u_floats(p.N, p.C) * sizeof(float));
    const int sy_b = p.sy0 + 2 * p.tstep, sx_b = p.sx0 + 2 * p.tstep;
    q.sy_min = p.sy0 < sy_b ? p.sy0 : sy_b;
    q.sx_min = p.sx0 < sx_b ? p.sx0 : sx_b;
    const WinoWeights ww = wino_weights_map(p, q.sy_min, q.sx_min);
    p.splits = 1;
    p.Ktot = 9 * p.C;
    const TgWprepItem it = {};
    int rc = TG_OK;
    const auto transform = [&]() -> int {
        hipLaunchKernelGGL(wino44_weights_kernel, dim3(ew_grid((int64_t)p.N * p.C, 256)), dim3(256), 0, s, p.w_raw, p.wino_u, p.N, p.C, ww);
        TG_CHECK_LAUNCH("wino44_weights_kernel");
        return TG_OK;
    };
    if (wino_prep(p, it, transform, &rc)) return rc;
    const bool gated = p.gate != nullptr;
    const bool gbits = p.gate_bits != nullptr;
    if (gbits) p.gate_bits_done = 1;
    const int ki = gbits ? 2 : gated ? 1 : 0;
    typedef void (*Kern)(const IGemmParams, const Wino44Geom, const float*);
    static const Kern kerns[3] = {wino44_kernel<false>, wino44_kernel<true>, wino44_kernel<true, true>};
    static LdsOptIn opts[3];
    const WinoProf pf = {0, 4044, p.M, 2.0 * p.M * (double)p.N * p.Ktot * g_alg_scale,
                         4.0 * ((double)p.B * p.IH * p.IW * p.C + (double)p.N * p.Ktot + (double)p.M * p.N)};
    return wino_launch(kerns[ki], opts[ki], (size_t)W4_LDS_FLOATS * sizeof(float), "wino44_kernel", p, q, pf, false, s);
}
```

### terra-gan_amd/mvp_gan/src/train.py

```python
import logging
import time
from pathlib import Path
from typing import Dict, Optional

import torch
from torch.utils.data import DataLoader

from tg_hip import engine as E
from tg_hip import ops as O
from tg_hip.gradbuf import grad_buffers

from mvp_gan import ExperimentTracker
from .models._common import as_bhw, require_hip
from .models.discriminator import Discriminator
from .models.generator import PConvUNet
from .utils.dataset import InpaintingDataset, resize_to_tensor
from .utils.raster_dataset import RasterWindowLoader
from .utils.shard_dataset import ShardLoader, is_shard
from .evaluation.metrics import calculate_boundary_quality
from .utils.losses import HumanGuidedLoss, InpaintingLoss, criterion_forward

logger = logging.getLogger(__name__)


# ... 30 lines not shown
                        raise ValueError(f"hip_adam_step: optimizer state {mk} has shape {tuple(t.shape)}, parameter {tuple(p.shape)}")
                    if t.device != p.device or t.dtype != p.dtype or not (O._dense_layouts(t) & O._dense_layouts(p)):
                        new = torch.empty_like(p, memory_format=torch.preserve_format)
                        new.copy_(t)
                        st[mk] = new
                if not torch.is_tensor(st["step"]):
                    st["step"] = torch.tensor(float(st["step"]), dtype=torch.float32)
                layout_ok.add((p.data_ptr(), st["exp_avg"].data_ptr(), st["exp_avg_sq"].data_ptr()))
            st["step"] += 1
            groups.setdefault(hyper[p] + (int(st["step"]),), []).append((p, st))
        for (lr, b1, b2, eps, step), items in groups.items():
            O.adam_multi_([p.data for p, _ in items], [p.grad for p, _ in items], [st["exp_avg"] for _, st in items],
                          [st["exp_avg_sq"] for _, st in items], lr, b1, b2, eps, step, grad_scale)

    if buckets is None:
        _update(list(hyper))
    else:
        for b in buckets:
            b.wait()
            _update(b.params)


def _assign_grads(module, grads):
    for k, p in module.named_parameters():
        g = grads.get(k)
        if g is not None:
            p.grad = g


def train_step(generator, discriminator, criterion, optimizer_G, optimizer_D, real_imgs, masks, grad_sync=None,
               reuse_fake_forward=True):
    try:
        return _train_step(generator, discriminator, criterion, optimizer_G, optimizer_D, real_imgs, masks, grad_sync,
                           reuse_fake_forward)
    except BaseException:
        if grad_sync is not None:
            grad_sync.reset()
        raise


def _train_step(generator, discriminator, criterion, optimizer_G, optimizer_D, real_imgs, masks, grad_sync, reuse_fake_forward):
    require_hip(real_imgs, "train_step")
    GP, DP = generator._tensors(), discriminator._tensors()
    real, mask = as_bhw(real_imgs, "train_step"), as_bhw(masks, "train_step")
    B, H, W = real.shape
    both = torch.empty((2 * B, H, W), dtype=torch.float32, device=real.device)
    masked = O.mul(real, mask, keep=both[B:])

    optimizer_G.zero_grad()
    ckpt = getattr(generator, "activation_checkpointing", False)
    gen, gctx = E.generator_forward(GP, masked, mask, generator.training, checkpoint=ckpt, out=both[:B])
    if grad_sync is not None and grad_sync._inflight != 0:
        raise RuntimeError(f"train_step: {grad_sync._inflight} gradient collectives still in flight at the loss stack")
    g_loss, _parts, dgen = criterion_forward(criterion, gen, real, mask, want_grad=True, both=both, checkpoint=ckpt)
    grouped = reuse_fake_forward and discriminator.training
    if grouped:
        logits2, dctx2 = E.discriminator_forward(DP, both, True, groups=2, update_running=False)
        E.discriminator_replay_running_stats(DP, dctx2, order=(0,))
        fake_logits, real_logits = logits2[:B], logits2[B:]
        dctx_fake = E.discriminator_group(dctx2, 0)
    else:
        fake_logits, dctx_fake = E.discriminator_forward(DP, gen, discriminator.training)
    g_adv, dlogits = O.bce_logits(fake_logits, 1.0)
    g_total = O.lincomb(g_loss, 1.0, g_adv, 1.0)
    _none, dgen_adv = E.discriminator_backward(DP, dctx_fake, dlogits, want_wgrad=False, want_dimg=True)
    O.axpby_(dgen_adv.reshape(B, H, W), 1.0, 1.0, dgen)
    gl = grad_sync.begin(generator, "G") if grad_sync is not None else None
    ggrads, _ = E.generator_backward(GP, gctx, dgen, gbuf=grad_buffers(generator).views,
                                     on_ready=gl.ready if gl is not None else None)
    del gctx
    _assign_grads(generator, ggrads)
    gb = gl.finish() if gl is not None else None
    if grad_sync is None:
        hip_adam_step(optimizer_G)

    optimizer_D.zero_grad()
    if grouped:
        E.discriminator_replay_running_stats(DP, dctx2, order=(1, 0))
    else:
        real_logits, dctx_real = E.discriminator_forward(DP, real, discriminator.training)
        fake_logits, dctx_fake = E.discriminator_forward(DP, gen, discriminator.training)
    dl2 = torch.empty_like(logits2) if grouped else None
    real_loss, dl_real = O.bce_logits(real_logits, 1.0, coef=0.5, dz_out=dl2[B:] if grouped else None)
    fake_loss, dl_fake = O.bce_logits(fake_logits, 0.0, coef=0.5, dz_out=dl2[:B] if grouped else None)
    d_loss = O.lincomb(real_loss, 0.5, fake_loss, 0.5)
    dl_ = grad_sync.begin(discriminator, "D") if grad_sync is not None else None
    if grouped:
        dg_real, _ = E.discriminator_backward(DP, dctx2, dl2, want_wgrad=True,
                                              gbuf=grad_buffers(discriminator).views,
                                              on_ready=dl_.ready if dl_ is not None else None)
    else:
        dg_real, _ = E.discriminator_backward(DP, dctx_real, dl_real, want_wgrad=True,
                                              gbuf=grad_buffers(discriminator).views)
        dg_fake, _ = E.discriminator_backward(DP, dctx_fake, dl_fake, want_wgrad=True)
        for k, g in dg_real.items():
            O.axpby_(dg_fake[k], 1.0, 1.0, g)
    _assign_grads(discriminator, dg_real)
    if grad_sync is not None:
        db = dl_.finish()
        hip_adam_step(optimizer_G, grad_sync.grad_scale, gb)
        hip_adam_step(optimizer_D, grad_sync.grad_scale, db)
    else:
        hip_adam_step(optimizer_D)

    return {"gen": gen.reshape(B, 1, H, W), "g_total": g_total, "g_loss": g_loss, "g_adv": g_adv, "d_loss": d_loss,
            "real_loss": real_loss, "fake_loss": fake_loss}

# ... 157 lines not shown
```

### terra-gan_amd/mvp_gan/src/utils/losses.py

```python
import logging
import os

import torch
import torch.nn as nn

from tg_hip import engine as E
from tg_hip import ops as O

from ..models._common import as_bhw, require_hip

logger = logging.getLogger(__name__)

_VGG16_CFG = [64, 64, "M", 128, 128, "M", 256, 256, 256, "M", 512, 512, 512, "M", 512, 512, 512, "M"]


def _vgg16_features_16(vgg_weights=None, allow_standin=None):
    path = vgg_weights or os.environ.get("TERRAGAN_VGG16_WEIGHTS")
    if allow_standin is None:
        allow_standin = os.environ.get("TERRAGAN_ALLOW_STANDIN_VGG") == "1"
    sd = None
    if path is None:
        try:
            from torchvision.models import VGG16_Weights, vgg16
            return vgg16(weights=VGG16_Weights.IMAGENET1K_V1).features[:16]
# ... 25 lines not shown

    def forward(self, a, b):
        return _L1Fn.apply(a, b)


class _L1Fn(torch.autograd.Function):
    @staticmethod
    def forward(ctx, a, b):
        require_hip(a, "L1")
        ac, bc = a.detach().float().contiguous(), b.detach().float().contiguous()
        out, _ = O.l1_mean(ac, bc, want_grad=False)
        ctx.save_for_backward(ac, bc)
        return out.reshape(())

    @staticmethod
    def backward(ctx, g):
        ac, bc = ctx.saved_tensors
        _, da = O.l1_mean(ac, bc, 1.0, gscale=g.float().contiguous().reshape(1), want_grad=True)
        return da, None


class BoundaryAwareLoss(nn.Module):

    def __init__(self, boundary_width: int = 10, epsilon: float = 1e-6, device=None):
        super().__init__()
        self.boundary_width, self.epsilon = boundary_width, epsilon
        self.device = device if device is not None else torch.device("cuda" if torch.cuda.is_available() else "cpu")

    def forward(self, pred, target, mask):
        return _PixelLossFn.apply(pred, target, mask, None, 0.0, 0.0, 1.0, self.epsilon)


class _PixelLossFn(torch.autograd.Function):

    @staticmethod
    def forward(ctx, pred, target, mask, l1_weight, w_l1, w_tv, w_bnd, eps):
        require_hip(pred, "pixel losses")
        p, t, m = as_bhw(pred, "loss"), as_bhw(target, "loss"), as_bhw(mask, "loss")
        lw = as_bhw(l1_weight, "loss") if l1_weight is not None else None
        out5, _ = O.pixel_losses(p, t, m, w_l1, w_tv, w_bnd, l1_weight=lw, want_grad=False, eps=eps)
        ctx.args = (p, t, m, lw, w_l1, w_tv, w_bnd, eps)
        ctx.shape = pred.shape
        return out5[4].reshape(())

    @staticmethod
    def backward(ctx, g):
        p, t, m, lw, w_l1, w_tv, w_bnd, eps = ctx.args
        _, dp = O.pixel_losses(p, t, m, w_l1, w_tv, w_bnd, l1_weight=lw, gscale=g.float().contiguous().reshape(1),
                               want_grad=True, eps=eps)
        return dp.reshape(ctx.shape), None, None, None, None, None, None, None


def criterion_forward(crit, pred, target, mask, want_grad, gscale=None, l1_weight=None, w_l1=1.0, scale=1.0, both=None,
                      checkpoint=False):
    w_p, w_tv, w_b = crit.perceptual_weight, crit.tv_weight, crit.boundary_weight
    out5, dp = O.pixel_losses(pred, target, mask, w_l1 * scale, max(w_tv, 0.0) * scale, max(w_b, 0.0) * scale,
                              l1_weight=l1_weight, gscale=gscale, want_grad=want_grad, eps=crit.boundary_loss.epsilon)
    total = out5[4:5]
    parts = {"pixel": out5}
    if w_p > 0:
        V = crit._vgg_tensors()
        B = pred.shape[0]
        if both is None:
            both = torch.empty((2 * B,) + tuple(pred.shape[1:]), dtype=pred.dtype, device=pred.device)
            both[:B].copy_(pred)
            both[B:].copy_(target)
        feats, vctx = E.vgg_forward(V, both, keep=("gates" if checkpoint else True) if want_grad else False, nb=B)
        fp, ft = feats[:B], feats[B:]
        perc, dfeat = O.l1_mean(fp, ft, w_p * scale, gscale=gscale, want_grad=want_grad, relu_gate=True)
        parts["perc"] = perc
        total = O.lincomb(total, 1.0, perc, w_p * scale)
        if want_grad:
            dperc = E.vgg_backward(vctx, dfeat, nb=B, gated=True)
            O.axpby_(dperc, 1.0, 1.0, dp)
    return total, parts, dp


class _InpaintingLossFn(torch.autograd.Function):
    @staticmethod
    def forward(ctx, pred, target, mask, crit):
        require_hip(pred, "InpaintingLoss")
        p, t, m = as_bhw(pred, "InpaintingLoss"), as_bhw(target, "InpaintingLoss"), as_bhw(mask, "InpaintingLoss")
        total, _parts, _ = criterion_forward(crit, p, t, m, want_grad=False)
        ctx.args, ctx.crit, ctx.shape = (p, t, m), crit, pred.shape
        return total.reshape(())

    @staticmethod
    def backward(ctx, g):
        p, t, m = ctx.args
        _t, _parts, dp = criterion_forward(ctx.crit, p, t, m, want_grad=True, gscale=g.float().contiguous().reshape(1))
        return dp.reshape(ctx.shape), None, None, None


class InpaintingLoss(nn.Module):
    def __init__(self, perceptual_weight: float = 0.1, tv_weight: float = 0.1, boundary_weight: float = 0.5,
                 device=None, vgg_weights=None, allow_standin_vgg=None):
        super().__init__()
        self.device = device if device is not None else torch.device("cuda" if torch.cuda.is_available() else "cpu")
        self.l1_loss = _L1Mean()
        self.perceptual_weight, self.tv_weight, self.boundary_weight = perceptual_weight, tv_weight, boundary_weight
        self.vgg_layers = _vgg16_features_16(vgg_weights, allow_standin_vgg).eval().to(self.device)
        for p in self.vgg_layers.parameters():
            p.requires_grad = False
        self.boundary_loss = BoundaryAwareLoss(device=self.device).to(self.device)
        self._vgg_cache = None

    def to(self, device):
        self.device = torch.device(device) if not isinstance(device, torch.device) else device
        self.boundary_loss.device = self.device
        self._vgg_cache = None
        return super().to(device)

    def _apply(self, fn, *a, **kw):
        self._vgg_cache = None
        return super()._apply(fn, *a, **kw)

    def _vgg_tensors(self):
        key = tuple((p.data_ptr(), p._version) for p in self.vgg_layers.parameters())
        if self._vgg_cache is None or self._vgg_cache[0] != key:
            V = {k: v.detach() for k, v in self.vgg_layers.state_dict().items()}
# ... 33 lines not shown
```

### terra-gan_amd/tg_hip/engine.py

```python
import os
from types import SimpleNamespace as NS

import torch

from . import ops as O

G_ENC = [("enc1", 1, 64, 7, 2, 3), ("enc2", 64, 128, 5, 2, 2), ("enc3", 128, 256, 5, 2, 2),
         ("enc4", 256, 512, 3, 2, 1), ("enc5", 512, 512, 3, 2, 1), ("enc6", 512, 512, 3, 2, 1),
         ("enc7", 512, 512, 3, 2, 1)]
G_DEC = [("dec7", 1024, 512, 3, 1, 1), ("dec6", 1024, 512, 3, 1, 1), ("dec5", 1024, 512, 3, 1, 1),
         ("dec4", 768, 256, 3, 1, 1), ("dec3", 384, 128, 3, 1, 1), ("dec2", 192, 64, 3, 1, 1),
         ("dec1", 64, 64, 3, 1, 1)]
D_LAYERS = [(0, None, None, 64, 4, 2, 1, True), (2, 3, 64, 128, 4, 2, 1, True), (5, 6, 128, 256, 4, 2, 1, True),
            (8, 9, 256, 512, 4, 2, 1, True), (11, None, 512, 1, 4, 1, 1, False)]
VGG_TRUNK = [0, 2, "M", 5, 7, "M", 10, 12, 14]


VGG_WINO4 = os.environ.get("TG_VGG_WINO4", "1") != "0"
VGG_WINO4_FWD = os.environ.get("TG_VGG_WINO4_FWD", "0") == "1"
VGG_WINO4_MINCH = int(os.environ.get("TG_VGG_WINO4_MINCH", "128"))
VGG_SPARSE = os.environ.get("TG_VGG_SPARSE", "1") != "0"
POOL_CODE = os.environ.get("TG_NO_POOL_CODE") is None


def _vgg_wino4(w, B, H, W, cout, mode=None, default=True):
    if mode is False or (mode is None and not default):
        return False
    wide = max(w.shape[0], w.shape[1]) >= VGG_WINO4_MINCH
    if mode is True:
        return wide
    items = B * ((H + 15) // 16) * ((W + 31) // 32) * (cout // 64)
    return wide and items >= 256
_side = {}
SIDE_WGRAD = os.environ.get("TG_SIDE_STREAM") == "1"
PROBE = None


def _side_stream():
    dev = torch.cuda.current_device()
    st = _side.get(dev)
    if st is None:
        st = _side[dev] = torch.cuda.Stream(device=dev)
    return st


def _wgrad(gbuf, inputs, fn):
    if gbuf is None or not SIDE_WGRAD:
        return fn()
    main, side = torch.cuda.current_stream(), _side_stream()
    side.wait_stream(main)
    with torch.cuda.stream(side):
        out = fn()
    for t in inputs:
        if t is not None:
            t.record_stream(side)
    return out


def join_side():
    if SIDE_WGRAD and torch.cuda.current_device() in _side:
        torch.cuda.current_stream().wait_stream(_side_stream())


def _pconv_fwd(P, name, k, s, p, x, in_mask, ratio, training, premasked=False, defer_act=False):
    O.tag(f"{name}.fwd")
    y = O.conv_fwd(x, P[f"{name}.input_conv.weight"], P[f"{name}.input_conv.bias"].detach(), k, s, p,
                   in_mask=None if premasked else in_mask, ratio=ratio)
    if training:
        mean, rstd, a = O.bn_fwd(y, P[f"{name}.bn.weight"], P[f"{name}.bn.bias"], O.ACT_RELU, 0.0, P[f"{name}.bn.running_mean"],
                                 P[f"{name}.bn.running_var"], P[f"{name}.bn.num_batches_tracked"], apply=not defer_act)
    else:
        mean, rstd = O.bn_eval_stats(P[f"{name}.bn.running_mean"], P[f"{name}.bn.running_var"])
        a = None if defer_act else O.bn_act_fwd(y, mean, rstd, P[f"{name}.bn.weight"], P[f"{name}.bn.bias"], O.ACT_RELU)
    if PROBE is not None:
# ... 239 lines not shown
                Bg = da.shape[0] // G_
                dy = da
                for gi in range(G_):
                    sl = slice(gi * Bg, (gi + 1) * Bg)
                    _d, g1, b1, db1 = O.bn_act_bwd(da[sl], c.y[sl], c.means[gi], c.rstds[gi], P[f"model.{c.bi}.weight"],
                                                   P[f"model.{c.bi}.bias"], O.ACT_LEAKY, 0.2, want_dbias=want_wgrad,
                                                   outs=outs if gi == 0 else None)
                    if gi == 0:
                        dgamma, dbeta, db = g1, b1, db1
                    elif want_wgrad:
                        O.axpby_(g1, 1.0, 1.0, dgamma), O.axpby_(b1, 1.0, 1.0, dbeta), O.axpby_(db1, 1.0, 1.0, db)
            if want_wgrad:
                grads[f"model.{c.bi}.weight"], grads[f"model.{c.bi}.bias"] = dgamma, dbeta
        gated = False
        O.tag(f"d{c.ci}.dgrad")
        if li > 0 or want_dimg:
            below = ctx.layers[li - 1] if li > 0 else None
            if below is not None and below.bi is None and below.act != O.ACT_NONE:
                da = O.conv_dgrad(dy, w, tuple(c.x.shape), c.k, c.s, c.p, gate=below.a, gate_act=below.act, gate_slope=0.2)
                gated = True
            else:
                da = O.conv_dgrad(dy, w, tuple(c.x.shape), c.k, c.s, c.p)
        else:
            da = None
        O.tag(f"d{c.ci}.wgrad")
        if want_wgrad:
            dw, db2 = _wgrad(gbuf, (c.x, dy), lambda c=c, dy=dy, w=w, db=db: O.conv_wgrad(
                c.x, dy, w, c.k, c.s, c.p, want_bias=db is None,
                dw_out=gbuf[f"model.{c.ci}.weight"] if gbuf is not None else None,
                db_out=gbuf[f"model.{c.ci}.bias"] if (gbuf is not None and db is None) else None))
            grads[f"model.{c.ci}.weight"], grads[f"model.{c.ci}.bias"] = dw, (db if db is not None else db2)
            if c.bi is not None:
                _notify(on_ready, grads, (f"model.{c.bi}.bias", f"model.{c.bi}.weight"))
            _notify(on_ready, grads, (f"model.{c.ci}.bias", f"model.{c.ci}.weight"))
    join_side()
    return grads, da


def discriminator_replay_running_stats(P, ctx, order=(0,)):
    G_ = getattr(ctx, "groups", 1)
    for c in ctx.layers:
        if c.bi is not None:
            rows = c.y.numel() // c.y.shape[-1] // G_
            if hasattr(c, "mean2"):
                O.bn_running_update_multi(c.mean2, c.rstd2, rows, list(order), P[f"model.{c.bi}.running_mean"],
                                          P[f"model.{c.bi}.running_var"], P[f"model.{c.bi}.num_batches_tracked"])
                continue
            for gi in order:
                mean, rstd = (c.means[gi], c.rstds[gi]) if hasattr(c, "means") else (c.mean, c.rstd)
                O.bn_running_update(mean, rstd, rows, P[f"model.{c.bi}.running_mean"], P[f"model.{c.bi}.running_var"],
                                    P[f"model.{c.bi}.num_batches_tracked"])


def vgg_forward(V, img, keep=True, wino4=None, nb=None):
    gates = keep == "gates"
    assert keep in (True, False) or gates, keep
    h = img.reshape(*img.shape, 1)
    steps = []
    pooled = code = None
    smaps = None
    if VGG_SPARSE and nb is not None and 2 * nb == img.shape[0]:
        smaps = O.vgg_sparse_map(img, nb, "".join("M" if it == "M" else "C" for it in VGG_TRUNK))
    ci = -1
    for i, item in enumerate(VGG_TRUNK):
        if item == "M":
            o = pooled if pooled is not None else O.maxpool2_fwd(h)
            if keep:
                steps.append(NS(kind="M", x=h if (code is None or not gates) else None, code=code))
            pooled = code = None
        else:
            w = V["0.folded"] if item == 0 else V[f"{item}.weight"]
            ci += 1
            sp = smaps.maps[ci] if smaps is not None else None
            O.tag(f"vgg{item}.fwd")
            pool = i + 1 < len(VGG_TRUNK) and VGG_TRUNK[i + 1] == "M" and h.shape[1] % 2 == 0 and h.shape[2] % 2 == 0
            w4 = _vgg_wino4(w, h.shape[0], h.shape[1], h.shape[2], w.shape[0], wino4, VGG_WINO4_FWD)
            if pool and POOL_CODE and not w4 and O.conv_pool_code_supported(tuple(h.shape), w.shape[0]):
                pooled, code = O.conv_fwd_pool_code(h, w, V[f"{item}.bias"], sparse=sp)
                o = None
            else:
                o = O.conv_fwd(h, w, V[f"{item}.bias"], 3, 1, 1, act=O.ACT_RELU, pool=pool, wino4=w4, sparse=sp)
                if pool:
                    o, pooled = o
            if gates:
                feeds = i + 1 < len(VGG_TRUNK) and VGG_TRUNK[i + 1] != "M"
                steps.append(NS(kind="C", w=w, x_shape=tuple(h.shape), a=None, bits=O.relu_gate_pack(o, nb) if feeds else None))
            elif keep:
                steps.append(NS(kind="C", w=w, x_shape=tuple(h.shape), a=o))
        h = o
    return h, NS(steps=steps)


def vgg_backward(ctx, dfeat, nb=None, wino4=None, gated=False):
    da = dfeat
    steps = ctx.steps
    w4 = wino4
    for i in range(len(steps) - 1, -1, -1):
        st = steps[i]
        if st.kind == "M":
            if getattr(st, "code", None) is not None:
                da = O.maxpool2_bwd_code(da, st.code)
            else:
                x = st.x if nb is None else st.x[:nb]
                da = O.maxpool2_bwd(da, x, relu_gate=True)
            gated = True
        else:
            a = None if st.a is None else (st.a if nb is None else st.a[:nb])
            if not gated and a is None:
                raise ValueError("vgg_backward: this context keeps no activation of the trunk's output: pass gated=True")
            dy = da if gated else O.act_bwd(da, a, O.ACT_RELU)
            shp = st.x_shape if nb is None else (nb,) + tuple(st.x_shape[1:])
            below = steps[i - 1] if i > 0 else None
            O.tag(f"vgg{VGG_TRUNK[i]}.dgrad")
            if below is not None and below.kind == "C" and getattr(below, "bits", None) is not None:
                assert below.bits.shape[0] == shp[0], "vgg_backward: the gate bits were packed for another number of images"
                da = O.conv_dgrad(dy, st.w, shp, 3, 1, 1, gate_bits=below.bits,
                                  wino4=_vgg_wino4(st.w, shp[0], shp[1], shp[2], shp[3], w4, VGG_WINO4))
                gated = True
            elif below is not None and below.kind == "C":
                ga = below.a if nb is None else below.a[:nb]
                da = O.conv_dgrad(dy, st.w, shp, 3, 1, 1, gate=ga, gate_act=O.ACT_RELU,
                                  wino4=_vgg_wino4(st.w, shp[0], shp[1], shp[2], shp[3], w4, VGG_WINO4))
                gated = True
            else:
                da = O.conv_dgrad(dy, st.w, shp, 3, 1, 1, wino4=_vgg_wino4(st.w, shp[0], shp[1], shp[2], shp[3], w4, VGG_WINO4))
                gated = False
    return da.reshape(da.shape[0], da.shape[1], da.shape[2])
```

### terra-gan_amd/tg_hip/lib.py

```python
import ctypes as C
import os

import torch

_HERE = os.path.dirname(os.path.abspath(__file__))
LIB_PATH = os.environ.get("TG_HIP_LIB") or os.path.join(os.path.dirname(_HERE), "lib", "libterragan_hip.so")


class TgConv(C.Structure):
    _fields_ = [(n, C.c_int32) for n in ("B", "H", "W", "Cin", "Ho", "Wo", "Cout", "k", "stride", "pad", "precision")]


TG_MASK_PYRAMID_MAX = 24


class TgMaskOp(C.Structure):
    _fields_ = [(n, C.c_int32) for n in ("kind", "H", "W", "Ho", "Wo", "k", "stride", "pad")] + \
               [(n, C.c_void_p) for n in ("in_", "in2", "out", "out2")]


class TgMaskPyramid(C.Structure):
    _fields_ = [("nops", C.c_int32), ("_pad", C.c_int32), ("op", TgMaskOp * TG_MASK_PYRAMID_MAX)]


class TgBnAct(C.Structure):
    _fields_ = [(n, C.c_void_p) for n in ("mean", "rstd", "gamma", "beta")] + [("act", C.c_int32), ("slope", C.c_float)]


class TgSparseMap(C.Structure):
    _fields_ = [(n, C.c_void_p) for n in ("bits", "list", "count")] + [(n, C.c_int32) for n in ("nb", "tiles_y", "tiles_x", "_pad")]


class TgRasterPlan(C.Structure):
    _fields_ = [(n, C.c_int32) for n in ("H", "W", "wh", "ww", "overlap", "ny", "nx")]


TG_EVAL_MAX_CLASSES = 8


class TgAreaClasses(C.Structure):
    _fields_ = [("n_edges", C.c_int32), ("_pad", C.c_int32), ("px", C.c_int64 * (TG_EVAL_MAX_CLASSES - 1))]


class TgError(RuntimeError):
    pass


P, I, I64, F, SZ, D = C.c_void_p, C.c_int, C.c_int64, C.c_float, C.c_size_t, C.c_double
CP = C.POINTER(TgConv)
RP = C.POINTER(TgRasterPlan)

SIGNATURES = {
    "tg_version": (I, []),
    "tg_last_error": (C.c_char_p, []),
    "tg_conv_fwd_ws_bytes": (SZ, [CP]),
    "tg_conv_fwd": (I, [CP, P, P, P, P, P, I, F, P, P, SZ, P]),
    "tg_conv_dgrad_ws_bytes": (SZ, [CP]),
    "tg_conv_dgrad": (I, [CP, P, P, P, P, I, P, SZ, P]),
    "tg_conv_dgrad_gated": (I, [CP, P, P, P, P, I, F, P, P, SZ, P]),
    "tg_set_cu_reserve": (I, [I]),
    "tg_set_work_stealing": (I, [I]),
    "tg_conv_wprep_bytes": (SZ, [CP, I]),
    "tg_conv_wprep": (I, [CP, I, P, P, P]),
    "tg_conv_wprep_item_bytes": (SZ, []),
    "tg_conv_wprep_item": (I, [CP, I, P, P, P]),
    "tg_conv_wprep_run": (I, [P, I, P]),
    "tg_conv_fwd_p": (I, [CP, P, P, P, P, P, P, I, F, P, P, SZ, P]),
    "tg_conv_fwd_pool": (I, [CP, P, P, P, P, P, P, I, F, P, P, P, SZ, P]),
    "tg_conv_pool_code_supported": (I, [CP]),
    "tg_conv_fwd_pool_code": (I, [CP, P, P, P, P, P, P, P, SZ, P]),
    "tg_maxpool2_bwd_code": (I, [P, P, I, I, I, I, P, P]),
    "tg_vgg_sparse_map_bytes": (SZ, [I, I, I, C.c_char_p]),
    "tg_vgg_sparse_map": (I, [P, I, I, I, C.c_char_p, P, SZ, P, C.POINTER(TgSparseMap), P]),
    "tg_conv_fwd_sparse": (I, [CP, P, P, P, P, I, F, P, P, P, C.POINTER(TgSparseMap), P, SZ, P]),
    "tg_conv_bnin_supported": (I, [CP, I]),
    "tg_conv_fwd_bnin": (I, [CP, P, C.POINTER(TgBnAct), P, P, I, F, P, P, SZ, P]),
    "tg_conv_wgrad_bnin": (I, [CP, P, C.POINTER(TgBnAct), P, P, P, P, SZ, P]),
    "tg_conv_dgrad_p": (I, [CP, P, P, P, P, P, I, F, P, I, P, SZ, P]),
    "tg_relu_gate_pack": (I, [P, I64, I, P, P]),
    "tg_conv_dgrad_gbits": (I, [CP, P, P, P, P, P, P, I, P, SZ, P]),
    "tg_conv_wgrad_ws_bytes": (SZ, [CP]),
    "tg_conv_wgrad": (I, [CP, P, P, P, P, P, P, SZ, P]),
    "tg_fold_cin": (I, [P, I, I, I, P, P]),
    "tg_mask_update": (I, [P, I, I, I, I, I, I, I, I, P, P, P]),
    "tg_mask_up_merge": (I, [P, P, I, I, I, I, I, P, P]),
    "tg_mask_pyramid": (I, [C.POINTER(TgMaskPyramid), I, P]),
    "tg_bn_ws_bytes": (SZ, [I64, I]),
    "tg_bn_stats": (I, [P, I64, I, F, F, P, P, P, P, P, P, SZ, P]),
    "tg_bn_eval_stats": (I, [P, P, I, F, P, P, P]),
    "tg_bn_act_fwd": (I, [P, I64, I, P, P, P, P, I, F, P, P]),
    "tg_bn_fwd": (I, [P, I64, I, F, F, P, P, I, F, P, P, P, P, P, P, P, SZ, P]),
    "tg_bn_act_bwd": (I, [P, P, I64, I, P, P, P, P, I, F, P, P, P, P, P, P, SZ, P]),
    "tg_bn_bwd_conv1_supported": (I, [I64, I]),
    "tg_bn_conv1_ws_bytes": (SZ, [I64, I]),
    "tg_bn_act_bwd_conv1": (I, [P, P, I, I, I, P, I, P, P, P, P, I, F, P, P, P, P, P, P, SZ, P]),
    "tg_act_bwd": (I, [P, P, I64, I, I, F, P, P, P]),
    "tg_upcat_fwd": (I, [P, P, P, I, I, I, I, I, I, I, P, P]),
    "tg_upcat_bn_supported": (I, [I, I, I, I, I, I, I]),
    "tg_upcat_fwd_bn": (I, [P, C.POINTER(TgBnAct), P, P, I, I, I, I, I, I, I, P, P]),
    "tg_upcat_bwd": (I, [P, I, I, I, I, I, I, I, P, P, P]),
    "tg_sigmoid_composite_fwd": (I, [P, P, P, I64, P, P]),
    "tg_sigmoid_composite_bwd": (I, [P, P, P, I64, P, P, P]),
    "tg_maxpool2_fwd": (I, [P, I, I, I, I, P, P]),
    "tg_maxpool2_bwd": (I, [P, P, I, I, I, I, I, P, P]),
    "tg_pixel_loss_ws_bytes": (SZ, [I, I, I]),
    "tg_pixel_losses": (I, [P, P, P, P, I, I, I, F, F, F, F, P, P, P, I, P, SZ, P]),
    "tg_reduce_ws_bytes": (SZ, [I64]),
    "tg_l1_mean": (I, [P, P, I64, F, P, P, P, P, SZ, P]),
    "tg_l1_mean_relu": (I, [P, P, I64, F, P, P, P, P, SZ, P]),
    "tg_bce_logits": (I, [P, I64, F, F, P, P, P, P, SZ, P]),
    "tg_adam": (I, [P, P, P, P, I64, D, D, D, D, I, F, P]),
    "tg_adam_multi": (I, [P, P, I, I, D, D, D, D, I, F, P]),
    "tg_adam_scalars": (I, [D, D, D, I, P]),
    "tg_write_floats": (I, [P, I, P, P]),
    "tg_adam_multi_s": (I, [P, P, I, I, D, D, D, P, F, P]),
    "tg_axpby": (I, [P, F, F, P, I64, P]),
    "tg_lincomb": (I, [P, F, P, F, P, I64, P]),
    "tg_mul": (I, [P, P, P, I64, P]),
    "tg_mul_keep": (I, [P, P, P, P, I64, P]),
    "tg_bn_running_update": (I, [P, P, I64, I, F, F, P, P, P, P]),
    "tg_bn_grouped_ws_bytes": (SZ, [I64, I, I]),
    "tg_bn_fwd_grouped": (I, [P, I64, I, I, F, P, P, I, F, P, P, P, P, SZ, P]),
    "tg_bn_act_bwd_grouped": (I, [P, P, I64, I, I, P, P, P, P, I, F, P, P, P, P, P, SZ, P]),
    "tg_bn_running_update_multi": (I, [P, P, I64, I, F, F, C.POINTER(C.c_int), I, P, P, P, P]),
    "tg_quality_metrics_ws_bytes": (SZ, [I64, I, I]),
    "tg_quality_metrics": (I, [P, P, P, I64, I, I, P, P, SZ, P]),
# ... 52 lines not shown
```

### terra-gan_amd/tg_hip/ops.py

```python
import ctypes as C

import torch

from . import lib as L

ACT_NONE, ACT_RELU, ACT_LEAKY = 0, 1, 2
PREC_F32, PREC_BF16, PREC_F32_WINO4 = 0, 1, 2
_precision = PREC_F32


def set_precision(name):
    global _precision
    _precision = {"f32": PREC_F32, "fp32": PREC_F32, "bf16": PREC_BF16}[name]


def get_precision():
    return "bf16" if _precision == PREC_BF16 else "f32"
BN_EPS, BN_MOMENTUM = 1e-5, 0.1
PROF_TAGS = False


def tag(name):
    if PROF_TAGS:
        _lib().tg_prof_tag(name.encode())
# ... 109 lines not shown
def graph_replayed(weight_ptrs, refreshed_keys):
    for ptr in weight_ptrs:
        _wstamp[ptr] = _wstamp.get(ptr, 0) + 1
    for key in refreshed_keys:
        e = _wprep.get(key)
        if e is not None:
            w = e[0]()
            if w is not None:
                e[1] = (w._version, _wstamp.get(key[0], 0))


def _prepared(w, wv, g, mode):
    if not WPREP_CACHE:
        return None
    import weakref
    ptr = wv.data_ptr()
    key = (ptr, mode, g.H, g.W, g.Cin, g.Cout, g.k, g.stride, g.pad, g.precision)
    stamp = (w._version, _wstamp.get(ptr, 0))
    ent = _wprep.get(key)
    if ent is not None and ent[0]() is w and ent[1] == stamp:
        ent[4] = True
        if WPREP_VERIFY and ent[2] is not None:
            fresh = torch.empty_like(ent[2])
            L.check(_lib().tg_conv_wprep(C.byref(g), mode, _p(wv), _p(fresh), _stream()), "tg_conv_wprep")
            if not torch.equal(fresh.view(torch.int32), ent[2].view(torch.int32)):
                raise L.TgError("prepared weights are stale: a parameter was rewritten without tg_hip.ops.weights_updated()")
        return ent[2]
    lib = _lib()
    if ent is None or ent[0]() is not w:
        nb = lib.tg_conv_wprep_bytes(C.byref(g), mode)
        buf = torch.empty((nb + 3) // 4, dtype=torch.float32, device=wv.device) if nb else None
        if len(_wprep) > 512:
            for k_ in [k_ for k_, e in _wprep.items() if e[0]() is None]:
                del _wprep[k_]
        item = False
        if buf is not None:
            raw = C.create_string_buffer(lib.tg_conv_wprep_item_bytes())
            if lib.tg_conv_wprep_item(C.byref(g), mode, _p(wv), _p(buf), raw):
                item = raw.raw
        ent = [weakref.ref(w), None, buf, item, True]
        _wprep[key] = ent
    if ent[2] is not None:
        L.check(lib.tg_conv_wprep(C.byref(g), mode, _p(wv), _p(ent[2]), _stream()), "tg_conv_wprep")
    ent[1] = stamp
    ent[4] = True
    return ent[2]


_sparse_tickets = {}


class SparseMaps:

    def __init__(self, buf, maps):
        self.buf, self.maps = buf, maps


def vgg_sparse_map(x, nb, plan):
    _chk(x, "x")
    H, W = x.shape[1], x.shape[2]
    assert x.shape[0] == 2 * nb and x.numel() == 2 * nb * H * W, (tuple(x.shape), nb)
    lib = _lib()
    pb = plan.encode()
    nbytes = lib.tg_vgg_sparse_map_bytes(nb, H, W, pb)
    if nbytes == 0:
        return None
    dev = x.device.index if x.device.index is not None else torch.cuda.current_device()
    ticket = _sparse_tickets.get(dev)
    if ticket is None or ticket.numel() < nb + 1:
        if torch.cuda.is_current_stream_capturing():
            return None
        ticket = _sparse_tickets[dev] = torch.zeros(max(nb + 1, 64), dtype=torch.int32, device=x.device)
    buf = torch.empty(nbytes, dtype=torch.uint8, device=x.device)
    nconv = plan.count("C")
    maps = (L.TgSparseMap * nconv)()
    L.check(lib.tg_vgg_sparse_map(_p(x), nb, H, W, pb, _p(buf), nbytes, _p(ticket), maps, _stream()), "tg_vgg_sparse_map")
    return SparseMaps(buf, maps)


def conv_fwd(x, w, bias, k, stride, pad, in_mask=None, ratio=None, act=ACT_NONE, slope=0.0, wino4=False, pool=False, sparse=None):
    _chk(x, "x"); _chk(bias, "bias"); _chk(in_mask, "in_mask"); _chk(ratio, "ratio")
    if sparse is not None:
        assert in_mask is None and ratio is None
        wv = weight_view(w)
        _chk(wv, "weight")
        g = conv_geom(x, wv.shape[0], k, stride, pad, wino4)
        y = empty(g.B, g.Ho, g.Wo, g.Cout, like=x)
        yp = empty(g.B, g.Ho // 2, g.Wo // 2, g.Cout, like=x) if pool else None
        lib = _lib()
        ws = workspace(lib.tg_conv_fwd_ws_bytes(C.byref(g)))
        L.check(lib.tg_conv_fwd_sparse(C.byref(g), _p(x), _p(wv), _p(_prepared(w, wv, g, WPREP_FWD)), _p(bias), act, slope, _p(y),
                                       _p(yp), None, C.byref(sparse), _p(ws), ws.numel() * 4, _stream()), "tg_conv_fwd_sparse")
        return (y, yp) if pool else y
    wv = weight_view(w)
    _chk(wv, "weight")
    g = conv_geom(x, wv.shape[0], k, stride, pad, wino4)
    assert wv.shape == (g.Cout, k, k, g.Cin), (tuple(wv.shape), g.Cout, k, g.Cin)
    y = empty(g.B, g.Ho, g.Wo, g.Cout, like=x)
    lib = _lib()
    nb = lib.tg_conv_fwd_ws_bytes(C.byref(g))
    ws = workspace(nb)
    if pool:
        yp = empty(g.B, g.Ho // 2, g.Wo // 2, g.Cout, like=x)
        L.check(lib.tg_conv_fwd_pool(C.byref(g), _p(x), _p(in_mask), _p(wv), _p(_prepared(w, wv, g, WPREP_FWD)), _p(bias), _p(ratio),
                                     act, slope, _p(y), _p(yp), _p(ws), ws.numel() * 4, _stream()), "tg_conv_fwd_pool")
        return y, yp
    L.check(lib.tg_conv_fwd_p(C.byref(g), _p(x), _p(in_mask), _p(wv), _p(_prepared(w, wv, g, WPREP_FWD)), _p(bias), _p(ratio),
                              act, slope, _p(y), _p(ws), ws.numel() * 4, _stream()), "tg_conv_fwd")
    return y


def _bn_act(in_bn):
    mean, rstd, gamma, beta = in_bn[:4]
    for t in (mean, rstd, gamma, beta):
        _chk(t, "in_bn")
    act = in_bn[4] if len(in_bn) > 4 else ACT_RELU
    slope = in_bn[5] if len(in_bn) > 5 else 0.0
    return L.TgBnAct(mean.data_ptr(), rstd.data_ptr(), gamma.detach().data_ptr(), beta.detach().data_ptr(), act, slope)


def conv_bnin_supported(x_shape, cout, k, stride, pad, wgrad=False):
    B, H, W, Cin = x_shape
    Ho, Wo = (H + 2 * pad - k) // stride + 1, (W + 2 * pad - k) // stride + 1
    g = L.TgConv(B, H, W, Cin, Ho, Wo, cout, k, stride, pad, _precision)
    return bool(_lib().tg_conv_bnin_supported(C.byref(g), 1 if wgrad else 0))


def conv_fwd_bnin(x, in_bn, w, bias, k, stride, pad, act=ACT_NONE, slope=0.0):
# ... 5 lines not shown
    lib = _lib()
    ws = workspace(lib.tg_conv_fwd_ws_bytes(C.byref(g)))
    bn = _bn_act(in_bn)
    L.check(lib.tg_conv_fwd_bnin(C.byref(g), _p(x), C.byref(bn), _p(wv), _p(bias), act, slope, _p(y), _p(ws), ws.numel() * 4, _stream()),
            "tg_conv_fwd_bnin")
    return y


def conv_pool_code_supported(x_shape, cout):
    B, H, W, Cin = x_shape
    g = L.TgConv(B, H, W, Cin, H, W, cout, 3, 1, 1, _precision)
    return bool(_lib().tg_conv_pool_code_supported(C.byref(g)))


def conv_fwd_pool_code(x, w, bias, sparse=None):
    _chk(x, "x"); _chk(bias, "bias")
    wv = weight_view(w)
    _chk(wv, "weight")
    g = conv_geom(x, wv.shape[0], 3, 1, 1)
    yp = empty(g.B, g.Ho // 2, g.Wo // 2, g.Cout, like=x)
    code = torch.empty((g.B, g.Ho // 2, g.Wo // 2, g.Cout), dtype=torch.uint8, device=x.device)
    lib = _lib()
    ws = workspace(lib.tg_conv_fwd_ws_bytes(C.byref(g)))
    if sparse is not None:
        L.check(lib.tg_conv_fwd_sparse(C.byref(g), _p(x), _p(wv), _p(_prepared(w, wv, g, WPREP_FWD)), _p(bias), ACT_RELU, 0.0, None,
                                       _p(yp), C.c_void_p(code.data_ptr()), C.byref(sparse), _p(ws), ws.numel() * 4, _stream()),
                "tg_conv_fwd_sparse")
        return yp, code
    L.check(lib.tg_conv_fwd_pool_code(C.byref(g), _p(x), _p(wv), _p(_prepared(w, wv, g, WPREP_FWD)), _p(bias), _p(yp),
                                      C.c_void_p(code.data_ptr()), _p(ws), ws.numel() * 4, _stream()), "tg_conv_fwd_pool_code")
    return yp, code


def maxpool2_bwd_code(dout, code):
    _chk(dout, "dout")
    B, Ho, Wo, Cc = dout.shape
    assert code.dtype == torch.uint8 and code.is_contiguous() and tuple(code.shape[1:]) == (Ho, Wo, Cc) and code.shape[0] >= B
    dx = empty(B, 2 * Ho, 2 * Wo, Cc, like=dout)
    L.check(_lib().tg_maxpool2_bwd_code(_p(dout), C.c_void_p(code.data_ptr()), B, Ho, Wo, Cc, _p(dx), _stream()), "tg_maxpool2_bwd_code")
    return dx


def relu_gate_pack(a, nb=None):
    _chk(a, "a")
    B, H, W, Cc = a.shape
    nb = B if nb is None else nb
    assert 0 < nb <= B, (nb, B)
    bits = torch.empty((nb, H, W, Cc // 32), dtype=torch.uint32, device=a.device)
    L.check(_lib().tg_relu_gate_pack(_p(a), nb * H * W, Cc, C.c_void_p(bits.data_ptr()), _stream()), "tg_relu_gate_pack")
    return bits


def conv_dgrad(dy, w, x_shape, k, stride, pad, in_mask=None, out=None, gate=None, gate_act=ACT_RELU, gate_slope=0.0, wino4=False,
               gate_bits=None):
    _chk(dy, "dy"); _chk(in_mask, "in_mask"); _chk(out, "out"); _chk(gate, "gate")
    wv = weight_view(w)
    B, H, W, Cin = x_shape
    g = L.TgConv(B, H, W, Cin, dy.shape[1], dy.shape[2], dy.shape[3], k, stride, pad, _prec(wino4))
    acc = 1 if out is not None else 0
    dx = out if out is not None else empty(B, H, W, Cin, like=dy)
    lib = _lib()
    ws = workspace(lib.tg_conv_dgrad_ws_bytes(C.byref(g)))
    if gate_bits is not None:
        assert gate is None and out is None, "conv_dgrad: gate_bits is exclusive with gate and does not accumulate"
        assert gate_bits.dtype == torch.uint32 and gate_bits.is_contiguous() and tuple(gate_bits.shape) == (B, H, W, Cin // 32), \
            (gate_bits.dtype, tuple(gate_bits.shape), tuple(x_shape))
        L.check(lib.tg_conv_dgrad_gbits(C.byref(g), _p(dy), _p(wv), _p(_prepared(w, wv, g, WPREP_DGRAD)), _p(in_mask),
                                        C.c_void_p(gate_bits.data_ptr()), _p(dx), 0, _p(ws), ws.numel() * 4, _stream()),
                "tg_conv_dgrad_gbits")
        return dx
    if gate is not None:
        assert out is None and tuple(gate.shape) == tuple(x_shape)
    L.check(lib.tg_conv_dgrad_p(C.byref(g), _p(dy), _p(wv), _p(_prepared(w, wv, g, WPREP_DGRAD)), _p(in_mask), _p(gate),
                                gate_act if gate is not None else ACT_NONE, gate_slope, _p(dx), acc, _p(ws), ws.numel() * 4,
                                _stream()), "tg_conv_dgrad")
    return dx


def conv_wgrad(x, dy, w, k, stride, pad, in_mask=None, want_bias=True, dw_out=None, db_out=None, in_bn=None):
    _chk(x, "x"); _chk(dy, "dy"); _chk(in_mask, "in_mask")
    wv = weight_view(w)
    B, H, W, Cin = x.shape
    g = L.TgConv(B, H, W, Cin, dy.shape[1], dy.shape[2], dy.shape[3], k, stride, pad, _precision)
    if dw_out is not None:
        dwv = dw_out.permute(0, 2, 3, 1)
        assert dwv.is_contiguous() and dwv.shape == wv.shape
    else:
        dwv = torch.empty_like(wv)
    db = (db_out if db_out is not None else empty(g.Cout, like=x)) if want_bias else None
    lib = _lib()
    ws = workspace(lib.tg_conv_wgrad_ws_bytes(C.byref(g)))
    if in_bn is not None:
        assert in_mask is None
        bn = _bn_act(in_bn)
        L.check(lib.tg_conv_wgrad_bnin(C.byref(g), _p(x), C.byref(bn), _p(dy), _p(dwv), _p(db), _p(ws), ws.numel() * 4, _stream()),
                "tg_conv_wgrad_bnin")
        return dwv.permute(0, 3, 1, 2), db
    L.check(lib.tg_conv_wgrad(C.byref(g), _p(x), _p(in_mask), _p(dy), _p(dwv), _p(db), _p(ws), ws.numel() * 4, _stream()),
            "tg_conv_wgrad")
    return dwv.permute(0, 3, 1, 2), db


def fold_cin(w):
    wv = weight_view(w)
    co, kh, kw, ci = wv.shape
    out = empty(co, kh, kw, 1, like=wv)
    L.check(_lib().tg_fold_cin(_p(wv), co, kh * kw, ci, _p(out), _stream()), "tg_fold_cin")
    return out.permute(0, 3, 1, 2)


def mask_update(mask, k, stride, pad):
    _chk(mask, "mask")
    B, H, W = mask.shape
    Ho, Wo = (H + 2 * pad - k) // stride + 1, (W + 2 * pad - k) // stride + 1
    mo, ratio = empty(B, Ho, Wo, like=mask), empty(B, Ho, Wo, like=mask)
# ... 814 lines not shown
```

Measured before the change: 1042 tiles/s.

## Skip VGG dgrad tiles outside the perceptual-loss gradient support

Extends the VGG sparse tile map with a 'need' mask so the backward data-gradient convolutions of the perceptual trunk run only over tiles where the gradient can be nonzero. Dilated support maps per layer are built in the same map kernel, with a second compacted list for paired tiles. New Winograd kernel variants consume the dgrad map. This removes dgrad work over regions where pred and target match and the loss does not need gradients, at the cost of a more complex map kernel and added risk of wrong gradients at tile borders.

```diff
diff --git a/include/terragan_hip.h b/include/terragan_hip.h
--- a/include/terragan_hip.h
+++ b/include/terragan_hip.h
@@ -58,11 +58,19 @@
     const uint32_t* bits;
     const int32_t* list;
     const int32_t* count;
-    int32_t nb, tiles_y, tiles_x, _pad;
+    int32_t nb, tiles_y, tiles_x;
+    int32_t dgrad;
+    const int32_t* list2;
+    const int32_t* count2;
 } TgSparseMap;
 size_t tg_vgg_sparse_map_bytes(int nb, int H, int W, const char* plan);
 int tg_vgg_sparse_map(const float* x, int nb, int H, int W, const char* plan, void* buf, size_t buf_bytes, int* ticket,
                       TgSparseMap* maps, tg_stream_t stream);
+int tg_vgg_sparse_map_need(const float* x, const float* need, int nb, int H, int W, const char* plan, void* buf, size_t buf_bytes,
+                           int* ticket, TgSparseMap* maps, TgSparseMap* dmaps, tg_stream_t stream);
+int tg_conv_dgrad_sparse(const TgConv* g, const float* dy, const float* w, const float* wprep, const float* x_act, int act,
+                         float slope, const uint32_t* gate_bits, float* dx, const TgSparseMap* sp, float* ws, size_t ws_bytes,
+                         tg_stream_t stream);
 int tg_conv_fwd_sparse(const TgConv* g, const float* x, const float* w, const float* wprep, const float* bias, int act,
                        float slope, float* y, float* pool_y, unsigned char* code, const TgSparseMap* sp, float* ws,
                        size_t ws_bytes, tg_stream_t stream);
diff --git a/terra-gan_amd/csrc/igemm.hip b/terra-gan_amd/csrc/igemm.hip
--- a/terra-gan_amd/csrc/igemm.hip
+++ b/terra-gan_amd/csrc/igemm.hip
@@ -1024,14 +1024,16 @@
         return wino_launch(kerns[ki], opts[ki], pl.pipe ? W16_PIPE_LDS_BYTES : W16_LDS_BYTES, "wino16_kernel", p, pl.q, pf, true, s);
     }
     typedef void (*WinoKern)(const IGemmParams, const WinoGeom, const float*);
-    static const WinoKern kerns[18] = {wino_kernel<false, false, false>, wino_kernel<false, true, false>, wino_kernel<true, false, false>,
+    static const WinoKern kerns[21] = {wino_kernel<false, false, false>, wino_kernel<false, true, false>, wino_kernel<true, false, false>,
                                        wino_kernel<true, true, false>, wino_pipe_kernel<false, false>, wino_pipe_kernel<true, false>,
                                        wino_pipe_kernel<false, false, true>, wino_pipe_kernel<true, false, false, true>,
                                        wino_kernel<false, false, true>, wino_kernel<false, true, true>, wino_kernel<true, false, true>,
                                        wino_kernel<true, true, true>, wino_pipe_kernel<false, true>, wino_pipe_kernel<true, true>,
                                        wino_pipe_kernel<false, true, true>, wino_pipe_kernel<true, true, false, true>,
-                                       wino_pipe_kernel<false, false, false, false, true>, wino_pipe_kernel<false, false, true, false, true>};
-    static LdsOptIn opts[18];
+                                       wino_pipe_kernel<false, false, false, false, 1>, wino_pipe_kernel<false, false, true, false, 1>,
+                                       wino_pipe_kernel<true, false, false, false, 2>, wino_pipe_kernel<true, false, false, true, 2>,
+                                       wino_pipe_kernel<false, false, false, false, 2>};
+    static LdsOptIn opts[21];
     WinoGeom q = pl.q;
     q.qctr = wino_queue_block(s, p.splits, q.total_work);
     if (pl.sparse && !q.qctr) {
@@ -1039,7 +1041,7 @@
         q.sp_bits = sm->bits; q.sp_list = sm->list; q.sp_count = sm->count;
         q.sp_nb = sm->nb; q.sp_tiles = sm->nb * q.tiles_y * q.tiles_x;
     }
-    const int ki = pl.kernel(q.qctr != nullptr);
+    const int ki = pl.kernel(q.qctr != nullptr, p.sparse && p.sparse->dgrad);
     return wino_launch(kerns[ki], opts[ki], (size_t)WINO_LDS_FLOATS * sizeof(float), "wino_kernel", p, q, pf, true, s);
 }
 
@@ -1570,7 +1572,8 @@
 
 static int conv_dgrad_impl(const TgConv* g, const float* dy, const float* w, float* wprep, int prep, const float* in_mask, float* dx,
                            int accumulate, const float* gate, int gate_act, float gate_slope, float* ws, size_t ws_bytes,
-                           tg_stream_t stream, const uint32_t* gate_bits = nullptr, int* gate_bits_done = nullptr);
+                           tg_stream_t stream, const uint32_t* gate_bits = nullptr, int* gate_bits_done = nullptr,
+                           const TgSparseMap* sparse = nullptr);
 extern "C" int tg_conv_dgrad(const TgConv* g, const float* dy, const float* w, const float* in_mask, float* dx,
                              int accumulate, float* ws, size_t ws_bytes, tg_stream_t stream) {
     return conv_dgrad_impl(g, dy, w, nullptr, 0, in_mask, dx, accumulate, nullptr, 0, 0.f, ws, ws_bytes, stream);
@@ -1604,6 +1607,27 @@
     if (rc || done) return rc;
     return gate_bits_apply_launch(dx, gate_bits, (int64_t)g->B * g->H * g->W, g->Cin, (hipStream_t)stream);
 }
+extern "C" int tg_conv_dgrad_sparse(const TgConv* g, const float* dy, const float* w, const float* wprep, const float* x_act, int act,
+                                    float slope, const uint32_t* gate_bits, float* dx, const TgSparseMap* sp, float* ws, size_t ws_bytes,
+                                    tg_stream_t stream) {
+    int rc = check_conv(g, "tg_conv_dgrad_sparse");
+    if (rc) return rc;
+    TG_REQUIRE(dy && w && dx && ws, "tg_conv_dgrad_sparse: null pointer");
+    TG_REQUIRE(!(x_act && gate_bits), "tg_conv_dgrad_sparse: x_act and gate_bits are exclusive");
+    TG_REQUIRE(x_act == nullptr || act == TG_ACT_RELU || act == TG_ACT_LEAKY, "tg_conv_dgrad_sparse: a gated dgrad needs a ReLU/LeakyReLU");
+    TG_REQUIRE(sp == nullptr || (sp->dgrad == 1 && sp->nb == g->B && sp->tiles_y == cdiv(g->H, 16) && sp->tiles_x == cdiv(g->W, 16)),
+               "tg_conv_dgrad_sparse: the map is not a dgrad map of this input grid");
+    if (gate_bits) {
+        TG_REQUIRE(g->Cin % 32 == 0, "tg_conv_dgrad_sparse: gate bits need Cin %% 32 == 0, got %d", g->Cin);
+        TG_REQUIRE((reinterpret_cast<uintptr_t>(gate_bits) & 15) == 0, "tg_conv_dgrad_sparse: pointers must be 16-byte aligned");
+    }
+    const bool usable = wprep != nullptr && !((x_act || gate_bits) && s2d_ok(g));
+    int done = 0;
+    rc = conv_dgrad_impl(g, dy, w, usable ? const_cast<float*>(wprep) : nullptr, usable ? 1 : 0, nullptr, dx, 0, x_act,
+                         x_act ? act : TG_ACT_NONE, slope, ws, ws_bytes, stream, gate_bits, &done, sp);
+    if (rc || done || !gate_bits) return rc;
+    return gate_bits_apply_launch(dx, gate_bits, (int64_t)g->B * g->H * g->W, g->Cin, (hipStream_t)stream);
+}
 extern "C" int tg_conv_wprep(const TgConv* g, int mode, const float* w, float* wprep, tg_stream_t stream) {
     TG_REQUIRE(g && w && wprep, "tg_conv_wprep: null pointer");
     TG_REQUIRE(mode == TG_WPREP_FWD || mode == TG_WPREP_DGRAD, "tg_conv_wprep: bad mode %d", mode);
@@ -1634,7 +1658,7 @@
 }
 static int conv_dgrad_impl(const TgConv* g, const float* dy, const float* w, float* wprep, int prep, const float* in_mask, float* dx,
                            int accumulate, const float* gate, int gate_act, float gate_slope, float* ws, size_t ws_bytes,
-                           tg_stream_t stream, const uint32_t* gate_bits, int* gate_bits_done) {
+                           tg_stream_t stream, const uint32_t* gate_bits, int* gate_bits_done, const TgSparseMap* sparse) {
     int rc = check_conv(g, "tg_conv_dgrad");
     if (rc) return rc;
     TG_REQUIRE(w && (prep < 0 || (dy && dx && ws)), "tg_conv_dgrad: null pointer");
@@ -1692,6 +1716,7 @@
         p.wino_u = wt;
         p.wino_ready = prep;
         p.gate_bits = gate_bits;
+        p.sparse = sparse;
         rc = launch_wino_s1(p, ws, dgrad_wt_floats(g), ws2_avail, room, s, "tg_conv_dgrad");
         if (gate_bits_done) *gate_bits_done = p.gate_bits_done;
         return rc;
diff --git a/terra-gan_amd/csrc/pointwise.hip b/terra-gan_amd/csrc/pointwise.hip
--- a/terra-gan_amd/csrc/pointwise.hip
+++ b/terra-gan_amd/csrc/pointwise.hip
@@ -338,15 +338,20 @@
 }
 
 constexpr int VSM_MAX_OPS = 24, VSM_MAX_CONV = 16, VSM_LDS_WORDS = 4096;
+constexpr int VSM_MAX_SLOTS = 2 * VSM_MAX_CONV;
 struct VggMapArgs {
     const uint32_t* x;
-    int nb, H, W, nops, nconv;
+    const float* need;
+    int nb, H, W, nops, nconv, nslots;
     char ops[VSM_MAX_OPS];
-    int tiles_y[VSM_MAX_CONV], tiles_x[VSM_MAX_CONV];
-    int32_t* count[VSM_MAX_CONV];
-    uint32_t* bits[VSM_MAX_CONV];
-    int32_t* list[VSM_MAX_CONV];
-    unsigned char* flags[VSM_MAX_CONV];
+    signed char slot_after[VSM_MAX_OPS];
+    int slot_seed;
+    int tiles_y[VSM_MAX_SLOTS], tiles_x[VSM_MAX_SLOTS];
+    int32_t* count[VSM_MAX_SLOTS];
+    uint32_t* bits[VSM_MAX_SLOTS];
+    int32_t* list[VSM_MAX_SLOTS];
+    int32_t* list2[VSM_MAX_SLOTS];
+    unsigned char* flags[VSM_MAX_SLOTS];
     uint64_t* d0;
     int rows_per_slice;
     int* ticket;
@@ -377,7 +382,7 @@
 }
 __global__ __launch_bounds__(1024) void vgg_sparse_map_kernel(const VggMapArgs a) {
     extern __shared__ uint64_t vsm[];
-    __shared__ int scan[1024];
+    __shared__ unsigned long long scan[1024];
     __shared__ int s_last;
     const int tid = threadIdx.x, lane = tid & 63, wave = tid >> 6, b = blockIdx.y;
     int H = a.H, W = a.W, WW = (W + 63) >> 6;
@@ -387,18 +392,24 @@
     {
         const uint32_t* xp = a.x + (size_t)b * H * W;
         const uint32_t* tp = a.x + ((size_t)a.nb + b) * H * W;
+        const float* np_ = a.need ? a.need + (size_t)b * H * W : nullptr;
         const int ubeg = blockIdx.x * a.rows_per_slice * WW, uend = min(H, (blockIdx.x + 1) * a.rows_per_slice) * WW;
         for (int u0 = ubeg + wave; u0 < uend; u0 += 16 * 8) {
             uint32_t pv[8], tv[8];
+            float nv[8];
 #pragma unroll
             for (int k = 0; k < 8; ++k) {
                 const int u = u0 + 16 * k, y = u / WW, px = (u - y * WW) * 64 + lane;
                 pv[k] = tv[k] = 0;
-                if (u < uend && px < W) { pv[k] = xp[(size_t)y * W + px]; tv[k] = tp[(size_t)y * W + px]; }
+                nv[k] = 1.f;
+                if (u < uend && px < W) {
+                    pv[k] = xp[(size_t)y * W + px]; tv[k] = tp[(size_t)y * W + px];
+                    if (np_) nv[k] = np_[(size_t)y * W + px];
+                }
             }
 #pragma unroll
             for (int k = 0; k < 8; ++k) {
-                const uint64_t m = __ballot(pv[k] != tv[k]);
+                const uint64_t m = __ballot(pv[k] != tv[k] || nv[k] != 1.f);
                 if (lane == 0 && u0 + 16 * k < uend) d0[u0 + 16 * k] = m;
             }
         }
@@ -407,7 +418,17 @@
     for (int u = tid; u < H * WW; u += 1024) cur[u] = d0[u];
     if (tid == 0) __hip_atomic_store(a.ticket + b, 0, __ATOMIC_RELAXED, __HIP_MEMORY_SCOPE_AGENT);
     __syncthreads();
-    int ci = 0;
+    auto flag_tiles = [&](int sl, const uint64_t* img, int h, int ww) {
+        const int tx_n = a.tiles_x[sl], tiles = a.tiles_y[sl] * tx_n;
+        for (int t2 = tid; t2 < tiles; t2 += 1024) {
+            const int ty = t2 / tx_n, tx = t2 - ty * tx_n;
+            const int w = (16 * tx) >> 6, sh = (16 * tx) & 63;
+            uint64_t any = 0;
+            for (int y = 16 * ty; y < min(16 * ty + 16, h); ++y) any |= (img[y * ww + w] >> sh) & 0xffffull;
+            a.flags[sl][(size_t)b * tiles + t2] = any ? 1 : 0;
+        }
+    };
+    if (a.slot_seed >= 0) flag_tiles(a.slot_seed, cur, H, WW);
     for (int o = 0; o < a.nops; ++o) {
         if (a.ops[o] == 'C') {
             for (int u = tid; u < H * WW; u += 1024) {
@@ -426,15 +447,7 @@
             }
             __syncthreads();
             uint64_t* t = cur; cur = nxt; nxt = t;
-            const int ty_n = a.tiles_y[ci], tx_n = a.tiles_x[ci], tiles = ty_n * tx_n;
-            for (int t2 = tid; t2 < tiles; t2 += 1024) {
-                const int ty = t2 / tx_n, tx = t2 - ty * tx_n;
-                const int w = (16 * tx) >> 6, sh = (16 * tx) & 63;
-                uint64_t any = 0;
-                for (int y = 16 * ty; y < min(16 * ty + 16, H); ++y) any |= (cur[y * WW + w] >> sh) & 0xffffull;
-                a.flags[ci][(size_t)b * tiles + t2] = any ? 1 : 0;
-            }
-            ++ci;
+            flag_tiles(a.slot_after[o], cur, H, WW);
         } else {
             const int H2 = H >> 1, W2 = W >> 1, WW2 = (W2 + 63) >> 6;
             for (int u = tid; u < H2 * WW2; u += 1024) {
@@ -449,13 +462,15 @@
             H = H2; W = W2; WW = WW2;
             __syncthreads();
             uint64_t* t = cur; cur = nxt; nxt = t;
+            if (a.slot_after[o] >= 0) flag_tiles(a.slot_after[o], cur, H, WW);
         }
         __syncthreads();
     }
     if (!vsm_last_arrival(a.ticket + a.nb, a.nb, &s_last)) return;
-    for (int c = 0; c < a.nconv; ++c) {
+    for (int c = 0; c < a.nslots; ++c) {
         const int n = a.nb * a.tiles_y[c] * a.tiles_x[c], nw = (n + 31) >> 5;
-        int carry = 0;
+        int carry = 0, carry2 = 0;
+        int32_t* const l2 = a.list2[c];
         for (int w0 = 0; w0 < nw; w0 += 1024) {
             const int w = w0 + tid;
             uint32_t word = 0;
@@ -470,30 +485,36 @@
                 if (32 * w + 32 > n) word &= (1u << (n - 32 * w)) - 1u;
                 a.bits[c][w] = word;
             }
-            const int pc = __popc(word);
-            scan[tid] = pc;
+            const uint32_t pword = l2 ? (word | (word >> 1)) & 0x55555555u : 0u;
+            const int pc = __popc(word), pc2 = __popc(pword);
+            scan[tid] = (unsigned long long)pc | ((unsigned long long)pc2 << 32);
             __syncthreads();
             for (int d = 1; d < 1024; d <<= 1) {
-                const int v = tid >= d ? scan[tid - d] : 0;
+                const unsigned long long v = tid >= d ? scan[tid - d] : 0ull;
                 __syncthreads();
                 scan[tid] += v;
                 __syncthreads();
             }
-            int pos = carry + scan[tid] - pc;
+            int pos = carry + (int)(uint32_t)scan[tid] - pc;
             for (uint32_t m = word; m; m &= m - 1) a.list[c][pos++] = 32 * w + __ffs(m) - 1;
-            carry += scan[1023];
+            int pos2 = carry2 + (int)(scan[tid] >> 32) - pc2;
+            for (uint32_t m = pword; m; m &= m - 1) l2[pos2++] = 32 * w + __ffs(m) - 1;
+            carry += (int)(uint32_t)scan[1023];
+            carry2 += (int)(scan[1023] >> 32);
             __syncthreads();
         }
-        if (tid == 0) *a.count[c] = carry;
+        if (tid == 0) { a.count[c][0] = carry; a.count[c][1] = carry2; }
     }
     if (tid == 0) __hip_atomic_store(a.ticket + a.nb, 0, __ATOMIC_RELAXED, __HIP_MEMORY_SCOPE_AGENT);
 }
 
 struct VsmLayout {
-    int nconv, nops, H, W;
+    int nconv, nops, nslots, H, W;
     size_t d0;
-    int tiles_y[VSM_MAX_CONV], tiles_x[VSM_MAX_CONV];
-    size_t count[VSM_MAX_CONV], bits[VSM_MAX_CONV], list[VSM_MAX_CONV], flags[VSM_MAX_CONV];
+    int tiles_y[VSM_MAX_SLOTS], tiles_x[VSM_MAX_SLOTS];
+    size_t count[VSM_MAX_SLOTS], bits[VSM_MAX_SLOTS], list[VSM_MAX_SLOTS], list2[VSM_MAX_SLOTS], flags[VSM_MAX_SLOTS];
+    int slot_seed, slot_after[VSM_MAX_OPS];
+    int in_slot[VSM_MAX_CONV];
     size_t bytes;
 };
 static bool vsm_layout(int nb, int H, int W, const char* plan, VsmLayout& L) {
@@ -503,55 +524,83 @@
     L.H = H; L.W = W;
     L.d0 = 0;
     size_t off = align_up((size_t)nb * H * ((W + 63) / 64) * sizeof(uint64_t), 16);
-    int h = H, w = W;
     for (const char* c = plan; *c; ++c) {
-        if (L.nops == VSM_MAX_OPS) return false;
-        ++L.nops;
-        if (*c == 'M') {
+        if (*c == 'C') ++L.nconv;
+        else if (*c != 'M') return false;
+        if (++L.nops > VSM_MAX_OPS) return false;
+    }
+    if (L.nconv == 0 || L.nconv > VSM_MAX_CONV) return false;
+    L.nslots = L.nconv;
+    const auto place = [&](int i, int h, int w) -> bool {
+        L.tiles_y[i] = cdiv(h, 16); L.tiles_x[i] = cdiv(w, 16);
+        const size_t n = (size_t)nb * L.tiles_y[i] * L.tiles_x[i];
+        if (n > ((size_t)1 << 30)) return false;
+        L.count[i] = off; off += 16;
+        L.bits[i] = off; off += align_up((n + 31) / 32, 4) * 4;
+        L.list[i] = off; off += align_up(n, 4) * 4;
+        L.list2[i] = off; off += align_up((n + 1) / 2, 4) * 4;
+        L.flags[i] = off; off += align_up(n, 32);
+        return true;
+    };
+    int h = H, w = W, ci = 0, cur_slot = L.nslots++;
+    L.slot_seed = cur_slot;
+    if (!place(cur_slot, h, w)) return false;
+    for (int o = 0; o < L.nops; ++o) {
+        if (plan[o] == 'M') {
             h >>= 1; w >>= 1;
             if (h <= 0 || w <= 0) return false;
-        } else if (*c == 'C') {
-            if (L.nconv == VSM_MAX_CONV) return false;
-            const int i = L.nconv++;
-            L.tiles_y[i] = cdiv(h, 16); L.tiles_x[i] = cdiv(w, 16);
-            const size_t n = (size_t)nb * L.tiles_y[i] * L.tiles_x[i];
-            if (n > ((size_t)1 << 30)) return false;
-            L.count[i] = off; off += 16;
-            L.bits[i] = off; off += align_up((n + 31) / 32, 4) * 4;
-            L.list[i] = off; off += align_up(n, 4) * 4;
-            L.flags[i] = off; off += align_up(n, 32);
+            cur_slot = L.nslots++;
+            if (!place(cur_slot, h, w)) return false;
         } else {
-            return false;
-        }
+            L.in_slot[ci] = cur_slot;
+            cur_slot = ci++;
+            if (!place(cur_slot, h, w)) return false;
+        }
+        L.slot_after[o] = cur_slot;
     }
     L.bytes = off;
-    return L.nconv > 0;
+    return true;
 }
 extern "C" size_t tg_vgg_sparse_map_bytes(int nb, int H, int W, const char* plan) {
     VsmLayout L;
     return vsm_layout(nb, H, W, plan, L) ? L.bytes : 0;
 }
-extern "C" int tg_vgg_sparse_map(const float* x, int nb, int H, int W, const char* plan, void* buf, size_t buf_bytes, int* ticket,
-                                 TgSparseMap* maps, tg_stream_t stream) {
+extern "C" int tg_vgg_sparse_map_need(const float* x, const float* need, int nb, int H, int W, const char* plan, void* buf, size_t buf_bytes,
+                                      int* ticket, TgSparseMap* maps, TgSparseMap* dmaps, tg_stream_t stream) {
     VsmLayout L;
     TG_REQUIRE(x && buf && ticket && maps, "tg_vgg_sparse_map: null pointer");
+    TG_REQUIRE((need != nullptr) == (dmaps != nullptr), "tg_vgg_sparse_map_need: `need` and `dmaps` come together");
     TG_REQUIRE(vsm_layout(nb, H, W, plan, L), "tg_vgg_sparse_map: geometry not supported (tg_vgg_sparse_map_bytes is 0)");
     TG_REQUIRE(buf_bytes >= L.bytes && (reinterpret_cast<uintptr_t>(buf) & 15) == 0, "tg_vgg_sparse_map: buffer too small or unaligned");
     VggMapArgs a = {};
     a.x = reinterpret_cast<const uint32_t*>(x);
+    a.need = need;
     a.nb = nb; a.H = H; a.W = W; a.nops = L.nops; a.nconv = L.nconv; a.ticket = ticket;
-    for (int i = 0; i < L.nops; ++i) a.ops[i] = plan[i];
+    a.nslots = need ? L.nslots : L.nconv;
+    a.slot_seed = need ? L.slot_seed : -1;
+    for (int i = 0; i < L.nops; ++i) {
+        a.ops[i] = plan[i];
+        a.slot_after[i] = (signed char)(plan[i] == 'C' || need ? L.slot_after[i] : -1);
+    }
     char* base = static_cast<char*>(buf);
     a.d0 = reinterpret_cast<uint64_t*>(base + L.d0);
     const int slices = cdiv(H, 8) < cdiv(256, nb) ? cdiv(H, 8) : cdiv(256, nb);
     a.rows_per_slice = cdiv(H, slices);
-    for (int i = 0; i < L.nconv; ++i) {
+    const auto map_of = [&](int i, int dgrad) {
+        TgSparseMap m = {a.bits[i], a.list[i], a.count[i], nb, L.tiles_y[i], L.tiles_x[i], dgrad, a.list2[i], a.list2[i] ? a.count[i] + 1 : nullptr};
+        return m;
+    };
+    for (int i = 0; i < a.nslots; ++i) {
         a.tiles_y[i] = L.tiles_y[i]; a.tiles_x[i] = L.tiles_x[i];
         a.count[i] = reinterpret_cast<int32_t*>(base + L.count[i]);
         a.bits[i] = reinterpret_cast<uint32_t*>(base + L.bits[i]);
         a.list[i] = reinterpret_cast<int32_t*>(base + L.list[i]);
+        a.list2[i] = need && !(L.tiles_x[i] & 1) ? reinterpret_cast<int32_t*>(base + L.list2[i]) : nullptr;
         a.flags[i] = reinterpret_cast<unsigned char*>(base + L.flags[i]);
-        maps[i] = TgSparseMap{a.bits[i], a.list[i], a.count[i], nb, L.tiles_y[i], L.tiles_x[i], 0};
+    }
+    for (int i = 0; i < L.nconv; ++i) {
+        maps[i] = map_of(i, 0);
+        if (dmaps) dmaps[i] = map_of(L.in_slot[i], 1);
     }
     const size_t lds = 2 * (size_t)H * ((W + 63) / 64) * sizeof(uint64_t);
     static bool opted[64] = {};
@@ -568,6 +617,10 @@
     hipLaunchKernelGGL(vgg_sparse_map_kernel, dim3(cdiv(H, a.rows_per_slice), nb), dim3(1024), lds, S(stream), a);
     TG_CHECK_LAUNCH("vgg_sparse_map_kernel");
     return TG_OK;
+}
+extern "C" int tg_vgg_sparse_map(const float* x, int nb, int H, int W, const char* plan, void* buf, size_t buf_bytes, int* ticket,
+                                 TgSparseMap* maps, tg_stream_t stream) {
+    return tg_vgg_sparse_map_need(x, nullptr, nb, H, W, plan, buf, buf_bytes, ticket, maps, nullptr, stream);
 }
 
 struct BnStatF {
diff --git a/terra-gan_amd/csrc/wino.inc b/terra-gan_amd/csrc/wino.inc
--- a/terra-gan_amd/csrc/wino.inc
+++ b/terra-gan_amd/csrc/wino.inc
@@ -30,6 +30,23 @@
 template <class F, int... T>
 __device__ __forceinline__ void wino_static_for(std::integer_sequence<int, T...>, F&& f) {
     (f(std::integral_constant<int, T>{}), ...);
+}
+
+template <int PAIR>
+__device__ __forceinline__ void wino_sparse_zero_fill(const IGemmParams& p, const uint32_t* __restrict__ bits, int tiles_x, int tiles_y, int nb) {
+    const int ux = tiles_x / PAIR, units = nb * tiles_y * ux;
+    for (int u = blockIdx.x; u < units; u += gridDim.x) {
+        const int t = u * PAIR;
+        if ((__builtin_amdgcn_readfirstlane(bits[t >> 5]) >> (t & 31)) & (PAIR == 2 ? 3u : 1u)) continue;
+        const int ix = u % ux, r = u / ux, ty = r % tiles_y, b = r / tiles_y;
+        const int oy0 = 16 * ty, ox0 = 16 * PAIR * ix;
+        const int rows = min(16, p.OH - oy0), rowq = min(16 * PAIR, p.OW - ox0) * (p.N >> 2);
+        float* base = p.dst + (((size_t)b * p.OH + oy0) * p.OW + ox0) * p.N;
+        for (int y = 0; y < rows; ++y) {
+            f32x4* row = reinterpret_cast<f32x4*>(base + (size_t)y * p.OW * p.N);
+            for (int i = threadIdx.x; i < rowq; i += WINO_THREADS) row[i] = f32x4{0.f, 0.f, 0.f, 0.f};
+        }
+    }
 }
 
 __device__ __forceinline__ void wino_distribute(int total, int interleave, int& item, int& item_end, int& step) {
@@ -480,7 +497,7 @@
     wk.done(q.qctr);
 }
 
-template <bool GATED, bool STEAL, bool POOL = false, bool GBITS = false, bool SPARSE = false>
+template <bool GATED, bool STEAL, bool POOL = false, bool GBITS = false, int SPARSE = 0>
 __global__ __launch_bounds__(WINO_THREADS) void wino_pipe_kernel(const IGemmParams p, const WinoGeom q, const float* __restrict__ U) {
     extern __shared__ __attribute__((aligned(16))) float smem[];
     float* Vs = smem;
@@ -494,7 +511,8 @@
     int total = q.total_work;
     if constexpr (SPARSE) {
         const int cnt = __builtin_amdgcn_readfirstlane(*q.sp_count);
-        total = (q.sp_tiles + min(max(cnt, 0), q.sp_tiles)) * q.nt;
+        total = ((SPARSE == 2 ? 0 : q.sp_tiles) + min(max(cnt, 0), q.sp_tiles)) * q.nt;
+        if constexpr (SPARSE == 2) wino_sparse_zero_fill<1>(p, q.sp_bits, q.tiles_x, q.tiles_y, q.sp_nb);
     }
     wk.init(total, q.interleave, q.qctr, wq_slot);
 
@@ -505,7 +523,9 @@
         int tile = it / q.nt;
         r.mirror = 0;
         if constexpr (SPARSE) {
-            if (tile < q.sp_tiles) {
+            if constexpr (SPARSE == 2) {
+                tile = __builtin_amdgcn_readfirstlane(q.sp_list[tile]);
+            } else if (tile < q.sp_tiles) {
                 r.mirror = (__builtin_amdgcn_readfirstlane(q.sp_bits[tile >> 5]) >> (tile & 31)) & 1 ? 0 : 1;
                 tile += q.sp_tiles;
             } else {
@@ -650,7 +670,7 @@
         const float act_neg = p.act == TG_ACT_RELU ? 0.f : (p.act == TG_ACT_LEAKY ? p.slope : 1.f);
         const float gate_neg = p.gate_act == TG_ACT_LEAKY ? p.gate_slope : 0.f;
         const auto drsrc = __builtin_amdgcn_make_buffer_rsrc(p.dst, 0, (int)((size_t)p.B * p.DH * p.DW * p.N * 4), 0x00020000);
-        const int e_mdelta = SPARSE ? q.sp_nb * p.DH * p.DW * p.N * 4 : 0;
+        const int e_mdelta = SPARSE == 1 ? q.sp_nb * p.DH * p.DW * p.N * 4 : 0;
         f32x4 bq = {0.f, 0.f, 0.f, 0.f};
         if (p.bias && e_single) bq = *reinterpret_cast<const f32x4*>(p.bias + e_nb0 + 4 * (lane & 7));
         f32x4 pmx[POOL ? 4 : 1];
@@ -740,7 +760,7 @@
                         if (p.pool_only) return;
                     }
                     __builtin_amdgcn_raw_buffer_store_b128(__builtin_bit_cast(u32x4, o), drsrc, e_voff + (uint32_t)soff, 0, 0);
-                    if constexpr (SPARSE) {
+                    if constexpr (SPARSE == 1) {
                         if (ci.mirror)
                             __builtin_amdgcn_raw_buffer_store_b128(__builtin_bit_cast(u32x4, o), drsrc, e_voff + (uint32_t)(soff - e_mdelta), 0, 0);
                     }
@@ -793,7 +813,7 @@
                     const int pix = (ci.b * PH + prow) * PW + (ci.ox0 >> 1);
                     __builtin_amdgcn_raw_buffer_store_b128(__builtin_bit_cast(u32x4, m), prsrc, p_voff + (uint32_t)((pix * p.N + e_nb0) * 4), 0, 0);
                     if (p.pool_code) __builtin_amdgcn_raw_buffer_store_b32(code, crsrc, c_voff + (uint32_t)(pix * p.N + e_nb0), 0, 0);
-                    if constexpr (SPARSE) {
+                    if constexpr (SPARSE == 1) {
                         if (ci.mirror) {
                             const int mpix = pix - q.sp_nb * PH * PW;
                             __builtin_amdgcn_raw_buffer_store_b128(__builtin_bit_cast(u32x4, m), prsrc, p_voff + (uint32_t)((mpix * p.N + e_nb0) * 4), 0, 0);
@@ -840,8 +860,8 @@
     int splits;
     bool fast, pipe, gated, pool, gbits;
     bool sparse;
-    int kernel(bool queued) const {
-        if (sparse && !queued) return pool ? 17 : 16;
+    int kernel(bool queued, bool dgrad_map = false) const {
+        if (sparse && !queued) return dgrad_map ? (gbits ? 19 : gated ? 18 : 20) : pool ? 17 : 16;
         return (queued ? 8 : 0) + (gbits ? 7 : pool ? 6 : pipe ? 4 + gated : (fast ? 2 : 0) + gated);
     }
 };
@@ -879,8 +899,10 @@
     pl.pool = p.pool_dst && !no_pool && pl.pipe && !pl.gated && one && !(p.OH & 1) && !(p.OW & 1) && plain_dst;
     pl.gbits = p.gate_bits != nullptr && pl.pipe && one;
     const TgSparseMap* sm = p.sparse;
-    pl.sparse = !p.bf16 && sm && pl.pipe && !pl.gated && !pl.gbits && one && !p.rowscale && plain_dst && (pl.pool || !p.pool_dst) &&
-                sm->nb > 0 && p.B == 2 * sm->nb && sm->tiles_y == q.tiles_y && sm->tiles_x == q.tiles_x && sm->bits && sm->list && sm->count;
+    const bool sp_any = !p.bf16 && sm && pl.pipe && one && !p.rowscale && plain_dst && sm->nb > 0 && sm->tiles_y == q.tiles_y &&
+                        sm->tiles_x == q.tiles_x && sm->bits && sm->list && sm->count;
+    pl.sparse = sp_any && (sm->dgrad ? p.B == sm->nb && !p.pool_dst && (p.gate == nullptr || pl.gated) && !(p.OH & 15) && !(p.OW & 15)
+                                     : !pl.gated && !pl.gbits && p.gate == nullptr && (pl.pool || !p.pool_dst) && p.B == 2 * sm->nb);
     return pl;
 }
 
diff --git a/terra-gan_amd/csrc/wino44.inc b/terra-gan_amd/csrc/wino44.inc
--- a/terra-gan_amd/csrc/wino44.inc
+++ b/terra-gan_amd/csrc/wino44.inc
@@ -16,6 +16,10 @@
     int tiles_x, tiles_y, total_work, nt;
     int sy_min, sx_min;
     int interleave;
+    const uint32_t* sp_bits;
+    const int* sp_list;
+    const int* sp_count;
+    int sp_units, sp_nb;
 };
 
 template <int A>
@@ -78,7 +82,7 @@
     wino44_weights_body(w, U, N, K, ww);
 }
 
-template <bool GATED, bool GBITS = false>
+template <bool GATED, bool GBITS = false, bool SPARSE = false>
 __global__ __launch_bounds__(WINO_THREADS) void wino44_kernel(const IGemmParams p, const Wino44Geom q, const float* __restrict__ U) {
     extern __shared__ __attribute__((aligned(16))) float smem[];
     float* Vs = smem;
@@ -89,7 +93,13 @@
     const int wave = __builtin_amdgcn_readfirstlane(tid >> 6);
     const int pg = wave & 3, nh = wave >> 2, ah = pg >> 1, bh = pg & 1;
     int item, item_end, istep;
-    wino_distribute(q.total_work, q.interleave, item, item_end, istep);
+    int total = q.total_work;
+    if constexpr (SPARSE) {
+        const int cnt = __builtin_amdgcn_readfirstlane(*q.sp_count);
+        total = min(max(cnt, 0), q.sp_units) * q.nt;
+        wino_sparse_zero_fill<2>(p, q.sp_bits, 2 * q.tiles_x, q.tiles_y, q.sp_nb);
+    }
+    wino_distribute(total, q.interleave, item, item_end, istep);
     if (item >= item_end) return;
 
     const int nchunks = p.C >> 3;
@@ -98,11 +108,17 @@
     const auto ursrc = __builtin_amdgcn_make_buffer_rsrc(const_cast<float*>(U), 0, (int)((size_t)W4_PTS * p.N * p.C * 4), 0x00020000);
 
     int n0, oy0, ox0, b, i_nt;
+    int sp_pair = 3;
     uint32_t poff[3];
     const bool p2_ok = tid + 2 * WINO_THREADS < 2 * W4_PPIX;
     auto decode = [&]() {
         i_nt = item % q.nt;
         int tile = item / q.nt;
+        if constexpr (SPARSE) {
+            const int t16 = __builtin_amdgcn_readfirstlane(q.sp_list[tile]);
+            sp_pair = (__builtin_amdgcn_readfirstlane(q.sp_bits[t16 >> 5]) >> (t16 & 31)) & 3;
+            tile = t16 >> 1;
+        }
         const int tx = tile % q.tiles_x;
         tile /= q.tiles_x;
         const int ty = tile % q.tiles_y;
@@ -322,6 +338,11 @@
 #pragma unroll
                     for (int e = 0; e < 4; ++e) o[e] *= gq[t4][e] > 0.f ? 1.f : gate_neg;
                 }
+                if constexpr (SPARSE) {
+                    const bool listed = (sp_pair >> (lane >> 5)) & 1;
+#pragma unroll
+                    for (int e = 0; e < 4; ++e) o[e] = listed ? o[e] : 0.f;
+                }
                 if (p.accumulate) o += __builtin_bit_cast(f32x4, __builtin_amdgcn_raw_buffer_load_b128(drsrc, e_voff + soff, 0, 0));
                 __builtin_amdgcn_raw_buffer_store_b128(__builtin_bit_cast(u32x4, o), drsrc, e_voff + soff, 0, 0);
             });
@@ -376,10 +397,19 @@
     const bool gated = p.gate != nullptr;
     const bool gbits = p.gate_bits != nullptr;
     if (gbits) p.gate_bits_done = 1;
-    const int ki = gbits ? 2 : gated ? 1 : 0;
+    const TgSparseMap* sm = p.sparse;
+    const bool sparse = sm && sm->dgrad && sm->bits && sm->list2 && sm->count2 && sm->nb > 0 && p.B == sm->nb && sm->tiles_y == q.tiles_y &&
+                        sm->tiles_x == 2 * q.tiles_x && p.ds == 1 && p.dy0 == 0 && p.dx0 == 0 && p.DH == p.OH && p.DW == p.OW &&
+                        !p.accumulate && !p.pool_dst && !(p.OH & 15) && !(p.OW & 15);
+    if (sparse) {
+        q.sp_bits = sm->bits; q.sp_list = sm->list2; q.sp_count = sm->count2;
+        q.sp_nb = sm->nb; q.sp_units = sm->nb * q.tiles_y * q.tiles_x;
+    }
+    const int ki = (sparse ? 3 : 0) + (gbits ? 2 : gated ? 1 : 0);
     typedef void (*Kern)(const IGemmParams, const Wino44Geom, const float*);
-    static const Kern kerns[3] = {wino44_kernel<false>, wino44_kernel<true>, wino44_kernel<true, true>};
-    static LdsOptIn opts[3];
+    static const Kern kerns[6] = {wino44_kernel<false>, wino44_kernel<true>, wino44_kernel<true, true>,
+                                  wino44_kernel<false, false, true>, wino44_kernel<true, false, true>, wino44_kernel<true, true, true>};
+    static LdsOptIn opts[6];
     const WinoProf pf = {0, 4044, p.M, 2.0 * p.M * (double)p.N * p.Ktot * g_alg_scale,
                          4.0 * ((double)p.B * p.IH * p.IW * p.C + (double)p.N * p.Ktot + (double)p.M * p.N)};
     return wino_launch(kerns[ki], opts[ki], (size_t)W4_LDS_FLOATS * sizeof(float), "wino44_kernel", p, q, pf, false, s);
diff --git a/terra-gan_amd/mvp_gan/src/train.py b/terra-gan_amd/mvp_gan/src/train.py
--- a/terra-gan_amd/mvp_gan/src/train.py
+++ b/terra-gan_amd/mvp_gan/src/train.py
@@ -106,7 +106,8 @@
     gen, gctx = E.generator_forward(GP, masked, mask, generator.training, checkpoint=ckpt, out=both[:B])
     if grad_sync is not None and grad_sync._inflight != 0:
         raise RuntimeError(f"train_step: {grad_sync._inflight} gradient collectives still in flight at the loss stack")
-    g_loss, _parts, dgen = criterion_forward(criterion, gen, real, mask, want_grad=True, both=both, checkpoint=ckpt)
+    g_loss, _parts, dgen = criterion_forward(criterion, gen, real, mask, want_grad=True, both=both, checkpoint=ckpt,
+                                             grad_needed=mask)
     grouped = reuse_fake_forward and discriminator.training
     if grouped:
         logits2, dctx2 = E.discriminator_forward(DP, both, True, groups=2, update_running=False)
diff --git a/terra-gan_amd/mvp_gan/src/utils/losses.py b/terra-gan_amd/mvp_gan/src/utils/losses.py
--- a/terra-gan_amd/mvp_gan/src/utils/losses.py
+++ b/terra-gan_amd/mvp_gan/src/utils/losses.py
@@ -101,7 +101,7 @@
 
 
 def criterion_forward(crit, pred, target, mask, want_grad, gscale=None, l1_weight=None, w_l1=1.0, scale=1.0, both=None,
-                      checkpoint=False):
+                      checkpoint=False, grad_needed=None):
     w_p, w_tv, w_b = crit.perceptual_weight, crit.tv_weight, crit.boundary_weight
     out5, dp = O.pixel_losses(pred, target, mask, w_l1 * scale, max(w_tv, 0.0) * scale, max(w_b, 0.0) * scale,
                               l1_weight=l1_weight, gscale=gscale, want_grad=want_grad, eps=crit.boundary_loss.epsilon)
@@ -114,7 +114,8 @@
             both = torch.empty((2 * B,) + tuple(pred.shape[1:]), dtype=pred.dtype, device=pred.device)
             both[:B].copy_(pred)
             both[B:].copy_(target)
-        feats, vctx = E.vgg_forward(V, both, keep=("gates" if checkpoint else True) if want_grad else False, nb=B)
+        feats, vctx = E.vgg_forward(V, both, keep=("gates" if checkpoint else True) if want_grad else False, nb=B,
+                                    need=grad_needed if want_grad else None)
         fp, ft = feats[:B], feats[B:]
         perc, dfeat = O.l1_mean(fp, ft, w_p * scale, gscale=gscale, want_grad=want_grad, relu_gate=True)
         parts["perc"] = perc
diff --git a/terra-gan_amd/tg_hip/engine.py b/terra-gan_amd/tg_hip/engine.py
--- a/terra-gan_amd/tg_hip/engine.py
+++ b/terra-gan_amd/tg_hip/engine.py
@@ -20,6 +20,7 @@
 VGG_WINO4_FWD = os.environ.get("TG_VGG_WINO4_FWD", "0") == "1"
 VGG_WINO4_MINCH = int(os.environ.get("TG_VGG_WINO4_MINCH", "128"))
 VGG_SPARSE = os.environ.get("TG_VGG_SPARSE", "1") != "0"
+VGG_SPARSE_DGRAD = os.environ.get("TG_VGG_SPARSE_DGRAD", "1") != "0"
 POOL_CODE = os.environ.get("TG_NO_POOL_CODE") is None
 
 
@@ -365,7 +366,7 @@
                                     P[f"model.{c.bi}.num_batches_tracked"])
 
 
-def vgg_forward(V, img, keep=True, wino4=None, nb=None):
+def vgg_forward(V, img, keep=True, wino4=None, nb=None, need=None):
     gates = keep == "gates"
     assert keep in (True, False) or gates, keep
     h = img.reshape(*img.shape, 1)
@@ -373,7 +374,10 @@
     pooled = code = None
     smaps = None
     if VGG_SPARSE and nb is not None and 2 * nb == img.shape[0]:
-        smaps = O.vgg_sparse_map(img, nb, "".join("M" if it == "M" else "C" for it in VGG_TRUNK))
+        if not (VGG_SPARSE_DGRAD and keep and PROBE is None):
+            need = None
+        smaps = O.vgg_sparse_map(img, nb, "".join("M" if it == "M" else "C" for it in VGG_TRUNK), need=need)
+    dmaps = smaps.dmaps if smaps is not None else None
     ci = -1
     for i, item in enumerate(VGG_TRUNK):
         if item == "M":
@@ -397,11 +401,12 @@
                     o, pooled = o
             if gates:
                 feeds = i + 1 < len(VGG_TRUNK) and VGG_TRUNK[i + 1] != "M"
-                steps.append(NS(kind="C", w=w, x_shape=tuple(h.shape), a=None, bits=O.relu_gate_pack(o, nb) if feeds else None))
+                steps.append(NS(kind="C", w=w, x_shape=tuple(h.shape), a=None, bits=O.relu_gate_pack(o, nb) if feeds else None,
+                                dmap=dmaps[ci] if dmaps is not None else None))
             elif keep:
-                steps.append(NS(kind="C", w=w, x_shape=tuple(h.shape), a=o))
+                steps.append(NS(kind="C", w=w, x_shape=tuple(h.shape), a=o, dmap=dmaps[ci] if dmaps is not None else None))
         h = o
-    return h, NS(steps=steps)
+    return h, NS(steps=steps, smaps=smaps if dmaps is not None else None)
 
 
 def vgg_backward(ctx, dfeat, nb=None, wino4=None, gated=False):
@@ -424,18 +429,18 @@
             dy = da if gated else O.act_bwd(da, a, O.ACT_RELU)
             shp = st.x_shape if nb is None else (nb,) + tuple(st.x_shape[1:])
             below = steps[i - 1] if i > 0 else None
+            use4 = _vgg_wino4(st.w, shp[0], shp[1], shp[2], shp[3], w4, VGG_WINO4)
+            sp = getattr(st, "dmap", None) if nb is not None and shp[3] > 1 and not use4 else None
             O.tag(f"vgg{VGG_TRUNK[i]}.dgrad")
             if below is not None and below.kind == "C" and getattr(below, "bits", None) is not None:
                 assert below.bits.shape[0] == shp[0], "vgg_backward: the gate bits were packed for another number of images"
-                da = O.conv_dgrad(dy, st.w, shp, 3, 1, 1, gate_bits=below.bits,
-                                  wino4=_vgg_wino4(st.w, shp[0], shp[1], shp[2], shp[3], w4, VGG_WINO4))
+                da = O.conv_dgrad(dy, st.w, shp, 3, 1, 1, gate_bits=below.bits, sparse=sp, wino4=use4)
                 gated = True
             elif below is not None and below.kind == "C":
                 ga = below.a if nb is None else below.a[:nb]
-                da = O.conv_dgrad(dy, st.w, shp, 3, 1, 1, gate=ga, gate_act=O.ACT_RELU,
-                                  wino4=_vgg_wino4(st.w, shp[0], shp[1], shp[2], shp[3], w4, VGG_WINO4))
+                da = O.conv_dgrad(dy, st.w, shp, 3, 1, 1, gate=ga, gate_act=O.ACT_RELU, sparse=sp, wino4=use4)
                 gated = True
             else:
-                da = O.conv_dgrad(dy, st.w, shp, 3, 1, 1, wino4=_vgg_wino4(st.w, shp[0], shp[1], shp[2], shp[3], w4, VGG_WINO4))
+                da = O.conv_dgrad(dy, st.w, shp, 3, 1, 1, sparse=sp, wino4=use4)
                 gated = False
     return da.reshape(da.shape[0], da.shape[1], da.shape[2])
diff --git a/terra-gan_amd/tg_hip/lib.py b/terra-gan_amd/tg_hip/lib.py
--- a/terra-gan_amd/tg_hip/lib.py
+++ b/terra-gan_amd/tg_hip/lib.py
@@ -28,7 +28,8 @@
 
 
 class TgSparseMap(C.Structure):
-    _fields_ = [(n, C.c_void_p) for n in ("bits", "list", "count")] + [(n, C.c_int32) for n in ("nb", "tiles_y", "tiles_x", "_pad")]
+    _fields_ = [(n, C.c_void_p) for n in ("bits", "list", "count")] + [(n, C.c_int32) for n in ("nb", "tiles_y", "tiles_x", "dgrad")] + \
+        [(n, C.c_void_p) for n in ("list2", "count2")]
 
 
 class TgRasterPlan(C.Structure):
@@ -72,6 +73,8 @@
     "tg_maxpool2_bwd_code": (I, [P, P, I, I, I, I, P, P]),
     "tg_vgg_sparse_map_bytes": (SZ, [I, I, I, C.c_char_p]),
     "tg_vgg_sparse_map": (I, [P, I, I, I, C.c_char_p, P, SZ, P, C.POINTER(TgSparseMap), P]),
+    "tg_vgg_sparse_map_need": (I, [P, P, I, I, I, C.c_char_p, P, SZ, P, C.POINTER(TgSparseMap), C.POINTER(TgSparseMap), P]),
+    "tg_conv_dgrad_sparse": (I, [CP, P, P, P, P, I, F, P, P, C.POINTER(TgSparseMap), P, SZ, P]),
     "tg_conv_fwd_sparse": (I, [CP, P, P, P, P, I, F, P, P, P, C.POINTER(TgSparseMap), P, SZ, P]),
     "tg_conv_bnin_supported": (I, [CP, I]),
     "tg_conv_fwd_bnin": (I, [CP, P, C.POINTER(TgBnAct), P, P, I, F, P, P, SZ, P]),
diff --git a/terra-gan_amd/tg_hip/ops.py b/terra-gan_amd/tg_hip/ops.py
--- a/terra-gan_amd/tg_hip/ops.py
+++ b/terra-gan_amd/tg_hip/ops.py
@@ -185,12 +185,12 @@
 
 class SparseMaps:
 
-    def __init__(self, buf, maps):
-        self.buf, self.maps = buf, maps
-
-
-def vgg_sparse_map(x, nb, plan):
-    _chk(x, "x")
+    def __init__(self, buf, maps, dmaps=None):
+        self.buf, self.maps, self.dmaps = buf, maps, dmaps
+
+
+def vgg_sparse_map(x, nb, plan, need=None):
+    _chk(x, "x"); _chk(need, "need")
     H, W = x.shape[1], x.shape[2]
     assert x.shape[0] == 2 * nb and x.numel() == 2 * nb * H * W, (tuple(x.shape), nb)
     lib = _lib()
@@ -207,6 +207,12 @@
     buf = torch.empty(nbytes, dtype=torch.uint8, device=x.device)
     nconv = plan.count("C")
     maps = (L.TgSparseMap * nconv)()
+    if need is not None:
+        assert need.numel() == nb * H * W and need.shape[0] == nb, (tuple(need.shape), nb, H, W)
+        dmaps = (L.TgSparseMap * nconv)()
+        L.check(lib.tg_vgg_sparse_map_need(_p(x), _p(need), nb, H, W, pb, _p(buf), nbytes, _p(ticket), maps, dmaps, _stream()),
+                "tg_vgg_sparse_map_need")
+        return SparseMaps(buf, maps, dmaps)
     L.check(lib.tg_vgg_sparse_map(_p(x), nb, H, W, pb, _p(buf), nbytes, _p(ticket), maps, _stream()), "tg_vgg_sparse_map")
     return SparseMaps(buf, maps)
 
@@ -318,7 +324,7 @@
 
 
 def conv_dgrad(dy, w, x_shape, k, stride, pad, in_mask=None, out=None, gate=None, gate_act=ACT_RELU, gate_slope=0.0, wino4=False,
-               gate_bits=None):
+               gate_bits=None, sparse=None):
     _chk(dy, "dy"); _chk(in_mask, "in_mask"); _chk(out, "out"); _chk(gate, "gate")
     wv = weight_view(w)
     B, H, W, Cin = x_shape
@@ -327,6 +333,18 @@
     dx = out if out is not None else empty(B, H, W, Cin, like=dy)
     lib = _lib()
     ws = workspace(lib.tg_conv_dgrad_ws_bytes(C.byref(g)))
+    if sparse is not None:
+        assert in_mask is None and out is None and not (gate is not None and gate_bits is not None)
+        if gate_bits is not None:
+            assert gate_bits.dtype == torch.uint32 and gate_bits.is_contiguous() and tuple(gate_bits.shape) == (B, H, W, Cin // 32), \
+                (gate_bits.dtype, tuple(gate_bits.shape), tuple(x_shape))
+        if gate is not None:
+            assert tuple(gate.shape) == tuple(x_shape)
+        L.check(lib.tg_conv_dgrad_sparse(C.byref(g), _p(dy), _p(wv), _p(_prepared(w, wv, g, WPREP_DGRAD)), _p(gate),
+                                         gate_act if gate is not None else ACT_NONE, gate_slope,
+                                         C.c_void_p(gate_bits.data_ptr()) if gate_bits is not None else None, _p(dx),
+                                         C.byref(sparse), _p(ws), ws.numel() * 4, _stream()), "tg_conv_dgrad_sparse")
+        return dx
     if gate_bits is not None:
         assert gate is None and out is None, "conv_dgrad: gate_bits is exclusive with gate and does not accumulate"
         assert gate_bits.dtype == torch.uint32 and gate_bits.is_contiguous() and tuple(gate_bits.shape) == (B, H, W, Cin // 32), \
```

Result: faster. 1057 tiles/s (median of 6 runs) (+1.4%).
